# nadult/Snail

Measured on AMD Instinct MI355X. Metric: Mrays/sec (primary), higher is better.
Workload: dtype f32; 1 GPU; BASELINE config 1: atrium (263124 tris, sponza.obj stand-in) 1920x1080 primary rays, hit records (t,u,v,triId); reflections=False, arith=host_sse, arith_tables=host CPU, packets=16x16 px = 1 wavefront, bvh_nodes=161677, bvh_depth=21, frames_in_flight=16, frames_per_launch=4, launches_in_flight=4, settle_frames=356, order_refresh=16, ranks=1, packet_order=heaviest first (node visits of an earlier frame), parallelism=single-gpu

## Files before the change

### include/snail_hip_debug.h

```cpp
#ifndef SNAIL_HIP_DEBUG_H
#define SNAIL_HIP_DEBUG_H
#include "snail_hip.h"
#ifdef __cplusplus
extern "C" {
#endif

int snail_debug_delay_dev(float microseconds, void *stream);

int snail_debug_clock_dev(float microseconds, uint64_t *d_out2, void *stream);

int snail_debug_recip_check(uint64_t out2[2]);

int snail_debug_hostsse_device_check(int fn, int threads, uint64_t *badChunks, uint32_t *firstBadChunk);

int snail_debug_dispatch_rate(int blocks, int threads, int reps, float *ms_per_launch);

int snail_debug_anyorder(SnailScene *, const float cam[13], int resx, int resy, int frames, int flags, float *ms_total);

int snail_debug_occupancy(int out[4]);

int snail_debug_rel_flag_count(SnailScene *, const float org[3], int *count);

int snail_debug_rel_axis_flag_count(SnailScene *, const float org[3], int out[6]);

#ifdef __cplusplus
}
#endif
#endif
```

### snail_amd/_lib.py

```python
from __future__ import annotations

import ctypes as C
import os

HERE = os.path.dirname(os.path.abspath(__file__))
LIB_PATH = os.environ.get("SNAIL_LIB_PATH") or os.path.join(HERE, "libsnailhip.so")


class SnailError(RuntimeError):
    pass


_lib = None

_VP, _I, _F13 = C.c_void_p, C.c_int, C.c_void_p
SIGNATURES = {
    "snail_last_error": (C.c_char_p, []),
    "snail_device_count": (_I, []),
    "snail_tris_from_verts": (_I, [_VP, _I, _VP]),
    "snail_bvh_build": (_I, [_VP, _I, _VP, _VP, _VP, _VP]),
    "snail_scene_create": (_VP, [_VP, _I, _VP, _I, _I, _I]),
    "snail_scene_destroy": (None, [_VP]),
    "snail_scene_info": (_I, [_VP, _VP, _VP, _VP, _VP]),
    "snail_scene_flags": (_I, [_VP, _VP, _VP]),
# ... 97 lines not shown
    "snail_texture_build": (_I, [_VP, _I, _I, _VP, C.c_int64, _VP]),
    "snail_materials_create": (_VP, [_VP, _VP, _I, _VP, _I, _VP, _I, _VP, _I]),
    "snail_materials_destroy": (None, [_VP]),
    "snail_materials_shade_packets_dev": (_I, [_VP, _F13, _I, _I, _VP, _I, _VP, _VP, _VP, _VP, _VP, _VP]),
    "snail_render_materials_dev": (_I, [_VP, _F13, _I, _I, _VP, _I, _VP, _I, _VP, _I, _VP, _VP]),
    "snail_render_materials_packets_dev": (_I, [_VP, _F13, _I, _I, _VP, _I, _VP, _I, _VP, _I, _VP, _VP, _VP]),
    "snail_render_materials_image": (_I, [_VP, _F13, _I, _I, _VP, _I, _VP, _I, _VP, _I, _VP]),
}

MATERIALS_BOUNCE_SIGNATURES = {
    "snail_materials_mirror_packets_dev": (_I, [_VP, _F13, _I, _I, _VP, _I, _VP, _VP, _VP, _VP, _VP, _VP, _VP, _VP, _VP, _VP]),
    "snail_materials_shade_rays_dev": (_I, [_VP, _I, _VP, _VP, _VP, _VP, _VP, _VP, _VP, _VP]),
    "snail_materials_bounce_dev": (_I, [_VP, _F13, _I, _I, _VP, _I, _VP, _I, _VP, _I, _VP, _VP]),
    "snail_materials_bounce_packets_dev": (_I, [_VP, _F13, _I, _I, _VP, _I, _VP, _I, _VP, _I, _VP, _VP, _VP]),
    "snail_materials_bounce_image": (_I, [_VP, _F13, _I, _I, _VP, _I, _VP, _I, _VP, _I, _VP]),
}

MATERIALS_TILES_SIGNATURES = {
    "snail_materials_frame_packets_dev": (_I, [_VP, _F13, _I, _I, _VP, _I, _VP, _I, _VP, _I, _VP, _VP, _VP, _VP]),
    "snail_materials_render_tiles": (_I, [_VP, _F13, _I, _I, _VP, _VP, _I, _VP, _I, _VP, _I, _VP, _VP, _VP]),
    "snail_materials_render_frame": (_I, [_VP, _F13, _I, _I, _VP, _I, _VP, _I, _VP, _I, _VP]),
}

MATERIALS_TRANSPARENCY_SIGNATURES = {
    "snail_materials_create_transparent": (_VP, [_VP, _VP, _I, _VP, _I, _VP, _I, _VP, _VP, _I]),
    "snail_materials_can_select_transparent": (_I, [_VP]),
    "snail_materials_shade_packets_transp_dev": (_I, [_VP, _F13, _I, _I, _VP, _I, _VP, _VP, _VP, _VP, _VP, _VP, _VP, _VP]),
    "snail_materials_shade_rays_transp_dev": (_I, [_VP, _I, _VP, _VP, _VP, _VP, _VP, _VP, _VP, _VP, _VP, _VP]),
    "snail_materials_continue_packets_dev": (_I, [_VP, _F13, _I, _I, _VP, _I, _VP, _VP, _VP, _VP, _VP, _VP, _VP, _VP, _VP, _VP, _VP, _VP, _VP, _VP]),
    "snail_materials_transparent_dev": (_I, [_VP, _F13, _I, _I, _VP, _I, _VP, _I, _VP, _I, _I, _VP, _VP, _VP]),
    "snail_materials_transparent_packets_dev": (_I, [_VP, _F13, _I, _I, _VP, _I, _VP, _I, _VP, _I, _VP, _I, _VP, _VP, _VP]),
    "snail_materials_transparent_image": (_I, [_VP, _F13, _I, _I, _VP, _I, _VP, _I, _VP, _I, _I, _VP, _VP]),
}

MATERIALS_TREE_SIGNATURES = {
    "snail_materials_mirror_rays_dev": (_I, [_VP, _I, _VP, _VP, _VP, _VP, _VP, _VP, _VP, _VP, _VP, _VP, _VP, _VP, _VP, _VP, _VP]),
    "snail_materials_tree_frame_packets_dev": (_I, [_VP, _F13, _I, _I, _VP, _I, _VP, _I, _VP, _I, _VP, _VP, _I, _VP, _VP, _VP]),
    "snail_materials_tree_render_tiles": (_I, [_VP, _F13, _I, _I, _VP, _VP, _I, _VP, _I, _VP, _I, _VP, _VP, _I, _VP, _VP]),
    "snail_materials_tree_render_frame": (_I, [_VP, _F13, _I, _I, _VP, _I, _VP, _I, _VP, _I, _I, _VP, _VP]),
    "snail_materials_set_level_budget": (_I, [_VP, C.c_uint64]),
    "snail_materials_level_bytes": (C.c_int64, [_I, _I, _I]),
}

MATERIALS_HEAT_SIGNATURES = {
    "snail_materials_packet_stats_dev": (_I, [_VP, _F13, _I, _I, _VP, _I, _VP, _I, _I, _I, _VP, _VP, _VP, _VP]),
    "snail_materials_heat_packets_dev": (_I, [_VP, _F13, _I, _I, _VP, _I, _VP, _I, _I, _VP, _VP, _VP, _I, _VP, _VP, _VP]),
    "snail_materials_render_heat_tiles": (_I, [_VP, _F13, _I, _I, _VP, _VP, _I, _VP, _I, _I, _VP, _VP, _I, _VP, _VP]),
    "snail_materials_render_heat_frame": (_I, [_VP, _F13, _I, _I, _VP, _I, _I, _VP, _I, _I, _VP, _VP]),
}

MATERIALS_DYNAMIC_SIGNATURES = {
    "snail_materials_create_dev": (_VP, [_VP, _VP, _VP, _VP, _I, _VP, _VP, _VP, _VP, _I, _VP, _I, _VP, _VP, _I, _VP]),
    "snail_materials_rebuild_dev": (_I, [_VP, _VP, _VP, _VP, _VP, _VP]),
    "snail_materials_update_dev": (_I, [_VP, _VP, _VP, _VP, _VP, _VP]),
}

INSTANCES_MATERIALS_SIGNATURES = {
    "snail_instances_materials_create": (_VP, [_VP, _VP, _I, _VP, _I, _VP, _I]),
    "snail_instances_materials_destroy": (None, [_VP]),
    "snail_instances_materials_shade_packets_dev": (_I, [_VP, _F13, _I, _I, _VP, _I, _VP, _VP, _VP, _VP, _VP, _VP, _VP]),
    "snail_instances_render_materials_dev": (_I, [_VP, _F13, _I, _I, _VP, _I, _VP, _I, _VP, _I, _VP, _VP]),
    "snail_instances_render_materials_packets_dev": (_I, [_VP, _F13, _I, _I, _VP, _I, _VP, _I, _VP, _I, _VP, _VP, _VP]),
    "snail_instances_render_materials_image": (_I, [_VP, _F13, _I, _I, _VP, _I, _VP, _I, _VP, _I, _VP]),
}

INSTANCES_MATERIALS_BOUNCE_SIGNATURES = {
    "snail_instances_materials_mirror_packets_dev": (_I, [_VP, _F13, _I, _I, _VP, _I, _VP, _VP, _VP, _VP, _VP, _VP, _VP, _VP, _VP, _VP, _VP, _VP]),
    "snail_instances_materials_shade_rays_dev": (_I, [_VP, _I, _VP, _VP, _VP, _VP, _VP, _VP, _VP, _VP]),
    "snail_instances_materials_bounce_dev": (_I, [_VP, _F13, _I, _I, _VP, _I, _VP, _I, _VP, _I, _VP, _VP]),
    "snail_instances_materials_bounce_packets_dev": (_I, [_VP, _F13, _I, _I, _VP, _I, _VP, _I, _VP, _I, _VP, _VP, _VP]),
    "snail_instances_materials_bounce_image": (_I, [_VP, _F13, _I, _I, _VP, _I, _VP, _I, _VP, _I, _VP]),
}

DEBUG_SIGNATURES = {
    "snail_debug_delay_dev": (_I, [C.c_float, _VP]),
    "snail_debug_clock_dev": (_I, [C.c_float, _VP, _VP]),
    "snail_debug_recip_check": (_I, [_VP]),
    "snail_debug_dispatch_rate": (_I, [_I, _I, _I, _VP]),
    "snail_debug_hostsse_device_check": (_I, [_I, _I, _VP, _VP]),
    "snail_debug_occupancy": (_I, [_VP]),
    "snail_debug_anyorder": (_I, [_VP, _F13, _I, _I, _I, _I, _VP]),
    "snail_debug_rel_flag_count": (_I, [_VP, _VP, _VP]),
    "snail_debug_rel_axis_flag_count": (_I, [_VP, _VP, _VP]),
}
DEBUG_LIB_PATH = os.path.join(HERE, "libsnailhip_debug.so")
_dbg = None


def debug_lib():
    global _dbg
    if _dbg is None:
        if not os.path.exists(DEBUG_LIB_PATH):
            raise SnailError("workbench library %s is missing: `make -C snail_amd/csrc debug`" % DEBUG_LIB_PATH)
        L = C.CDLL(DEBUG_LIB_PATH)
        for table in (SIGNATURES, INSTANCES_SIGNATURES, INSTANCES_SHADE_SIGNATURES, INSTANCES_TILES_SIGNATURES, INSTANCES_BUILD_SIGNATURES, BVH_FAST_SIGNATURES, HEATMAP_SIGNATURES, MATERIALS_SIGNATURES, MATERIALS_BOUNCE_SIGNATURES, MATERIALS_TILES_SIGNATURES, MATERIALS_TRANSPARENCY_SIGNATURES, MATERIALS_TREE_SIGNATURES, MATERIALS_HEAT_SIGNATURES, MATERIALS_DYNAMIC_SIGNATURES, INSTANCES_MATERIALS_SIGNATURES, INSTANCES_MATERIALS_BOUNCE_SIGNATURES, DEBUG_SIGNATURES):
            for name, (res, args) in table.items():
                fn = getattr(L, name)
                fn.restype = res
                fn.argtypes = args
        _dbg = L
    return _dbg


def lib():
    global _lib
    if _lib is None:
        if not os.path.exists(LIB_PATH):
            raise SnailError(
                "HIP extension %s is missing: run `python -c 'import __graft_entry__ as g; g.build()'` "
                "(or `make -C snail_amd/csrc`). There is no CPU fallback." % LIB_PATH)
        try:
            L = C.CDLL(LIB_PATH)
        except OSError as e:
            raise SnailError("cannot load %s: %s" % (LIB_PATH, e)) from e
        for table in (SIGNATURES, INSTANCES_SIGNATURES, INSTANCES_SHADE_SIGNATURES, INSTANCES_TILES_SIGNATURES, INSTANCES_BUILD_SIGNATURES, BVH_FAST_SIGNATURES, HEATMAP_SIGNATURES, MATERIALS_SIGNATURES, MATERIALS_BOUNCE_SIGNATURES, MATERIALS_TILES_SIGNATURES, MATERIALS_TRANSPARENCY_SIGNATURES, MATERIALS_TREE_SIGNATURES, MATERIALS_HEAT_SIGNATURES, MATERIALS_DYNAMIC_SIGNATURES, INSTANCES_MATERIALS_SIGNATURES, INSTANCES_MATERIALS_BOUNCE_SIGNATURES):
            for name, (res, args) in table.items():
                fn = getattr(L, name)
                fn.restype = res
                fn.argtypes = args
        for name, (res, args) in DEBUG_SIGNATURES.items():
            fn = getattr(L, name, None)
            if fn is not None:
                fn.restype = res
                fn.argtypes = args
        _lib = L
    return _lib


def check(rc: int, what: str) -> None:
    if rc != 0:
        msg = lib().snail_last_error()
        raise SnailError("%s failed (status %d): %s" % (what, rc, msg.decode() if msg else "?"))


def ptr(a):
    if a is None:
        return None
    if hasattr(a, "data_ptr"):
        return C.c_void_p(a.data_ptr())
    return a.ctypes.data_as(C.c_void_p)
```

### snail_amd/csrc/bvh_fast.inc

```
namespace devf {

using devb::BuildHdr;
using devb::TNode;
static_assert(SNAIL_MAX_DEPTH == devb::kMaxDepth, "BuildHdr::qCount and the small kernel's stack are sized for DBVH::maxDepth == BVH::maxDepth");

struct FastArgs : devb::SplitArgs {
	const float *verts;
	uint4 *nodes, *pf, *tris;
	unsigned trisOff;
	int needSane;
	int *cur;
	int *perm, *info;
};

__global__ void k_fast_init(FastArgs A) {
	const int i = blockIdx.x * blockDim.x + threadIdx.x;
	if(i < A.n) A.startCnt[i] = 0;
	if(i == 0) devb::hdrInit(*A.hdr);
}

__global__ void k_fast_boxes(FastArgs A) {
	const int i = blockIdx.x * blockDim.x + threadIdx.x;
	if(i >= A.n) return;
	float p[9], rec[16];
// ... 65 lines not shown
	bool curOnDevice = false;
	int depthLimit = SNAIL_MAX_DEPTH;
	hipEvent_t ready = nullptr;
	bool hasReady = false;
	unsigned long long rebuilds = 0;
	struct Use { hipStream_t stream; hipEvent_t ev; };
	std::vector<Use> uses;
};

namespace {

void fastFree(SnailSceneFast *f) {
	if(!f) return;
	if(f->base) (void)hipFree(f->base);
	if(f->dCur) (void)hipFree(f->dCur);
	if(f->ready) (void)hipEventDestroy(f->ready);
	for(auto &u : f->uses) (void)hipEventDestroy(u.ev);
	delete f;
}

int fastSceneBegin(SnailScene *s, hipStream_t stream) {
	SnailSceneFast *f = s->fast;
	if(f->hasReady) HIP_TRY(hipStreamWaitEvent(stream, f->ready, 0));
	return 0;
}
void fastSceneEnd(SnailScene *s, hipStream_t stream) {
	SnailSceneFast *f = s->fast;
	for(auto &u : f->uses)
		if(u.stream == stream) { (void)hipEventRecord(u.ev, stream); return; }
	SnailSceneFast::Use u;
	u.stream = stream;
	if(hipEventCreateWithFlags(&u.ev, hipEventDisableTiming) != hipSuccess) return;
	(void)hipEventRecord(u.ev, stream);
	f->uses.push_back(u);
}

int fastEnqueue(SnailScene *s, const float *dVerts, int32_t *dPerm, int32_t *dInfo, int needSane, hipStream_t st) {
	SnailSceneFast *f = s->fast;
	const int n = s->nTris;
	devf::FastArgs A;
	memset((void *)&A, 0, sizeof(A));
	buildCarve(f->base, n, A);
	A.n = n; A.maxDepth = f->depthLimit;
	A.verts = dVerts;
	A.nodes = s->dNodes; A.tris = s->dTris; A.pf = s->pfOKButNesting ? (uint4 *)s->dPF : nullptr; A.trisOff = (unsigned)s->trisOff;
	A.needSane = needSane; A.cur = f->dCur; A.perm = dPerm; A.info = dInfo;
	const devb::SplitArgs &SA = A;
	typedef devb::SplitBvh P;
	const int perN = (n + 255) / 256;
	hipLaunchKernelGGL(devf::k_fast_init, dim3(perN), dim3(256), 0, st, A);
	hipLaunchKernelGGL(devf::k_fast_boxes, dim3(perN), dim3(256), 0, st, A);
	hipLaunchKernelGGL(devb::k_build_root<P>, dim3(1), dim3(64), 0, st, SA);
	if(n > devb::kSmall) {
		const int most = n / (devb::kSmall + 1) + 1;
		const int wide = 28;
		for(int level = 0; level < wide; level++) {
			const int grid = std::min(level < 11 ? (1 << level) : 2048, most);
			hipLaunchKernelGGL(devb::k_build_big<P>, dim3(grid), dim3(256), 0, st, SA, level, level + 1);
		}
		hipLaunchKernelGGL(devb::k_build_big<P>, dim3(1), dim3(256), 0, st, SA, wide, (int)devb::kLevels);
	}
	if(n >= P::minSplit) hipLaunchKernelGGL(devb::k_build_small<P>, dim3(std::min(n / 2 + 1, 8192)), dim3(64), 0, st, SA);
	hipLaunchKernelGGL(devb::k_build_scan, dim3(1), dim3(1024), 0, st, SA);
	hipLaunchKernelGGL(devf::k_fast_commit, dim3((unsigned)std::min((2 * (long long)n + 255) / 256, 4096LL)), dim3(256), 0, st, A);
	HIP_TRY(hipGetLastError());
	if(!f->ready) HIP_TRY(hipEventCreateWithFlags(&f->ready, hipEventDisableTiming));
	HIP_TRY(hipEventRecord(f->ready, st));
	f->hasReady = true;
	f->curOnDevice = true;
	f->rebuilds++;
	return 0;
}

int fastWaitUsers(SnailScene *s, hipStream_t st) {
	SnailSceneFast *f = s->fast;
	for(auto &u : f->uses) HIP_TRY(hipStreamWaitEvent(st, u.ev, 0));
	if(f->hasReady) HIP_TRY(hipStreamWaitEvent(st, f->ready, 0));
	return 0;
}

int fastRebuildLocked(SnailScene *s, const float *dVerts, int32_t *dPerm, int32_t *dInfo, hipStream_t st) {
	if(int rc = fastWaitUsers(s, st)) return rc;
	for(auto &e : s->rel) e.valid = false;
	return fastEnqueue(s, dVerts, dPerm, dInfo, s->fastOK, st);
}

int fastCurrent(const SnailScene *cs, int cur[4]) {
	SnailScene *s = const_cast<SnailScene *>(cs);
	SnailSceneFast *f = s->fast;
	DeviceGuard guard(s->device);
	std::lock_guard<std::mutex> lock(s->mu);
	if(f->curOnDevice) {
		if(f->hasReady) HIP_TRY(hipEventSynchronize(f->ready));
		HIP_TRY(hipMemcpy(f->cur, f->dCur, sizeof(f->cur), hipMemcpyDeviceToHost));
		f->curOnDevice = false;
	}
	memcpy(cur, f->cur, sizeof(f->cur));
	return 0;
}

}

extern "C" {

SnailScene *snail_scene_create_fast_dev(const float *d_verts9, int nTris, int device, int32_t *d_perm, int32_t *d_info, void *stream) {
	const char *fn = "snail_scene_create_fast_dev";
	if(!d_verts9 || nTris <= 0 || nTris > (1 << 29)) { snail_set_error("%s: bad arguments", fn); return nullptr; }
	DeviceGuard guard(device);
	if(!guard.ok) { snail_set_error("%s: hipSetDevice(%d) failed", fn, device); return nullptr; }
	hipStream_t st = (hipStream_t)stream;
	SnailScene *s = new SnailScene();
	s->fast = new SnailSceneFast();
	SnailSceneFast *f = s->fast;
	const int cap = 2 * nTris - 1;
	s->device = device; s->nNodes = cap; s->nTris = nTris;
	const size_t trisOff = pfTrisOffset(cap), pfBytes = trisOff + (size_t)nTris * 64;
	const bool fits = pfFits((size_t)cap + 1, (size_t)nTris);
	s->trisOff = (int)(fits ? trisOff : 0);
	s->pfOKButNesting = fits ? 1 : 0;
	hipError_t e;
	if((e = hipMalloc((void **)&s->dNodes, (size_t)cap * 32)) != hipSuccess || (e = hipMalloc((void **)&s->dPF, fits ? pfBytes : (size_t)nTris * 64)) != hipSuccess ||
	   (e = hipMalloc((void **)&f->base, buildScratchBytes(nTris))) != hipSuccess || (e = hipMalloc((void **)&f->dCur, 4 * sizeof(int))) != hipSuccess ||
	   (fits && (e = hipMemset(s->dPF, 0, ((size_t)cap + 1) * 32)) != hipSuccess) || (e = hipMemset(f->dCur, 0, 4 * sizeof(int))) != hipSuccess) {
		snail_set_error("%s: %s", fn, hipGetErrorString(e));
		snail_scene_destroy(s);
		return nullptr;
	}
	s->dTris = (uint4 *)(s->dPF + s->trisOff);
	hipLaunchKernelGGL(dev::lbvh::k_fill_empty, dim3((unsigned)((cap + 255) / 256)), dim3(256), 0, 0, (float *)s->dNodes, cap);
	int cur[4] = {0, 0, 0, 0}, status[8] = {0};
	if((e = hipDeviceSynchronize()) != hipSuccess || fastEnqueue(s, d_verts9, d_perm, d_info, 0, st) != 0 || (e = hipStreamSynchronize(st)) != hipSuccess ||
	   (e = hipMemcpy(status, f->base, sizeof(status), hipMemcpyDeviceToHost)) != hipSuccess || fastCurrent(s, cur) != 0) {
		if(e != hipSuccess) snail_set_error("%s: %s", fn, hipGetErrorString(e));
		snail_scene_destroy(s);
		return nullptr;
	}
	if(status[0] != 0) {
		if(status[0] == 1) snail_set_error("%s: a vertex is not finite", fn);
		else snail_set_error("%s: the tree is deeper than BVH::maxDepth = %d", fn, SNAIL_MAX_DEPTH);
		snail_scene_destroy(s);
		return nullptr;
	}
	s->depth = cur[1]; s->fastOK = cur[2]; s->nestedOK = 1; s->pfOK = s->pfOKButNesting;
	f->depthLimit = s->depth > 62 ? SNAIL_MAX_DEPTH : 62;
	return s;
}

int snail_scene_rebuild_fast_dev(SnailScene *s, const float *d_verts9, int nTris, int32_t *d_perm, int32_t *d_info, void *stream) {
	const char *fn = "snail_scene_rebuild_fast_dev";
	if(int rc = checkScene(s, fn)) return rc;
	if(!s->fast) { snail_set_error("%s: the handle was not made by snail_scene_create_fast_dev", fn); return 1; }
	if(!d_verts9 || nTris != s->nTris) { snail_set_error("%s: %d triangles, the handle holds %d (or null vertices)", fn, nTris, s->nTris); return 1; }
	hipStream_t st = (hipStream_t)stream;
	DeviceGuard guard(s->device);
	SNAIL_LOCK(s);
	return fastRebuildLocked(s, d_verts9, d_perm, d_info, st);
}

}
```

### snail_amd/csrc/snail_dev.inc

```
namespace SNAIL_DEV_NS {

typedef unsigned long long u64;
typedef unsigned u32x4 __attribute__((ext_vector_type(4)));
typedef const __attribute__((address_space(4))) u32x4 *scalar_ptr;

struct Node {
	float bmin[3], bmax[3];
	unsigned sub;
	int aux;
};

__device__ __forceinline__ float asf(unsigned u) { return __uint_as_float(u); }
__device__ __forceinline__ float asf(int u) { return __int_as_float(u); }

typedef const __attribute__((address_space(4))) char *scalar_bytes;
__device__ __forceinline__ Node loadNode(const uint4 *nodes, int idx) {
	const unsigned off = (unsigned)idx << 5;
	scalar_ptr p = (scalar_ptr)((scalar_bytes)(unsigned long long)nodes + off);
	u32x4 a = p[0], b = p[1];
	Node n;
	n.bmin[0] = asf(a.x); n.bmin[1] = asf(a.y); n.bmin[2] = asf(a.z);
	n.bmax[0] = asf(a.w); n.bmax[1] = asf(b.x); n.bmax[2] = asf(b.y);
	n.sub = b.z; n.aux = (int)b.w;
	return n;
// ... 257 lines not shown
		outMax[c] = noneU ? 0.0f : (x01 > x23 ? x01 : x23);
	}
}

__device__ __forceinline__ bool boxTestInterval(const Node &n, const Interval &i) {
	float lmin = 0.0f, lmax = 0.0f;
#pragma unroll
	for(int k = 0; k < 3; k++) {
		float l1 = i.minIDir[k] * (n.bmin[k] - i.maxOrg[k]);
		float l2 = i.maxIDir[k] * (n.bmin[k] - i.maxOrg[k]);
		float l3 = i.minIDir[k] * (n.bmax[k] - i.minOrg[k]);
		float l4 = i.maxIDir[k] * (n.bmax[k] - i.minOrg[k]);
		float lo = Min<M_EXACT>(Min<M_EXACT>(l1, l2), Min<M_EXACT>(l3, l4));
		float hi = Max<M_EXACT>(Max<M_EXACT>(l1, l2), Max<M_EXACT>(l3, l4));
		if(k == 0) { lmin = lo; lmax = hi; }
		else { lmin = Max<M_EXACT>(lmin, lo); lmax = Min<M_EXACT>(lmax, hi); }
	}
	return lmax >= 0.0f && lmin <= lmax;
}

struct TriTerms {
	float t0v[3], t1v[3], tmul;
};
__device__ __forceinline__ TriTerms triTerms(const Tri &t, float ox, float oy, float oz) {
	TriTerms r;
	float tv[3] = {ox - t.a[0], oy - t.a[1], oz - t.a[2]};
	r.t0v[0] = (t.ba[1] * tv[2] - t.ba[2] * tv[1]) * t.it0;
	r.t0v[1] = (t.ba[2] * tv[0] - t.ba[0] * tv[2]) * t.it0;
	r.t0v[2] = (t.ba[0] * tv[1] - t.ba[1] * tv[0]) * t.it0;
	r.t1v[0] = (tv[1] * t.ca[2] - tv[2] * t.ca[1]) * t.it0;
	r.t1v[1] = (tv[2] * t.ca[0] - tv[0] * t.ca[2]) * t.it0;
	r.t1v[2] = (tv[0] * t.ca[1] - tv[1] * t.ca[0]) * t.it0;
	r.tmul = -(tv[0] * t.n[0] + tv[1] * t.n[1] + tv[2] * t.n[2]);
	return r;
}

__device__ __forceinline__ float selLanes(float a, float b, u64 lanesOfB) {
	float r;
	asm("v_cndmask_b32 %0, %1, %2, %3" : "=v"(r) : "v"(a), "v"(b), "s"(lanesOfB));
	return r;
}
__device__ __forceinline__ float xbar(int byteAddr, float x) { return __int_as_float(__builtin_amdgcn_ds_bpermute(byteAddr, __float_as_int(x))); }
template <int CTRL> __device__ __forceinline__ float quadRot(float v) {
	return __int_as_float(__builtin_amdgcn_update_dpp(0, __float_as_int(v), CTRL, 0xf, 0xf, false));
}
struct QuadTerms {
	float n, t0v, t1v, tmul;
};
template <int M>
__device__ __forceinline__ u64 cullQuad(const uint4 *__restrict__ tris, int count , int firstTri, int lane, const float (&org)[3][4],
										const Interval &iv, QuadTerms &T) {
	const int c = lane & 3;
	const bool active = lane < 4 * count;
	T.n = T.t0v = T.t1v = T.tmul = 0.0f;
	bool pass = false;
	const float oc = selLanes(selLanes(org[0][0], org[1][0], 0x2222222222222222ull), org[2][0], 0x4444444444444444ull);
	const float dmn = selLanes(selLanes(iv.minDir[0], iv.minDir[1], 0x2222222222222222ull), iv.minDir[2], 0x4444444444444444ull);
	const float dmx = selLanes(selLanes(iv.maxDir[0], iv.maxDir[1], 0x2222222222222222ull), iv.maxDir[2], 0x4444444444444444ull);
	if(active) {
		const float *rec = (const float *)(tris + (size_t)(firstTri + (lane >> 2)) * 4);
		const float *rc = rec + (c == 3 ? 0 : c);
		const float ac = rc[0], bac = rc[3], cac = rc[6], nc = rc[12];
		const float t0 = rec[9], it0 = rec[10];
		const float tv = oc - ac;
		const float tv1 = quadRot<0xC9>(tv), tv2 = quadRot<0xD2>(tv);
		const float ba1 = quadRot<0xC9>(bac), ba2 = quadRot<0xD2>(bac), ca1 = quadRot<0xC9>(cac), ca2 = quadRot<0xD2>(cac);
		const float c1 = ba1 * tv2 - ba2 * tv1;
		const float c2 = tv1 * ca2 - tv2 * ca1;
		T.n = nc; T.t0v = c1 * it0; T.t1v = c2 * it0;
		const float p = tv * nc;
		T.tmul = -((p + quadRot<0xC9>(p)) + quadRot<0xD2>(p));
		float m;
		if(M == M_EXACT) m = (nc < 0.0f ? dmn : dmx) * nc;
		else m = vmax(dmn * nc, dmx * nc);
		const float det = (m + quadRot<0xC9>(m)) + quadRot<0xD2>(m);
		const float c1a = dmn * c1, c1b = dmx * c1, c2a = dmn * c2, c2b = dmx * c2;
		const float u0p = Min<M>(c1a, c1b), u1p = Max<M>(c1a, c1b), v0p = Min<M>(c2a, c2b), v1p = Max<M>(c2a, c2b);
		const float u0 = (u0p + quadRot<0xC9>(u0p)) + quadRot<0xD2>(u0p), u1 = (u1p + quadRot<0xC9>(u1p)) + quadRot<0xD2>(u1p);
		const float v0 = (v0p + quadRot<0xC9>(v0p)) + quadRot<0xD2>(v0p), v1 = (v1p + quadRot<0xC9>(v1p)) + quadRot<0xD2>(v1p);
		pass = (c == 0) & ((det < 0.0f) | ((Min<M>(u1, v1) >= 0.0f) & (u0 + v0 <= det * t0)));
	}
	return __builtin_amdgcn_ballot_w64(pass);
}
__device__ __forceinline__ void setId(int &d, int v) { d = v; }
__device__ __forceinline__ void setId(float &d, int v) { d = __int_as_float(v); }
template <int R> struct NarrowRays {
	float d[3][R], dist[R];
	int tid[R];
};
template <int R> __device__ __forceinline__ void narrowGather(const float (&q)[4], int srcAddr, float (&out)[R]) {
	const float a0 = xbar(srcAddr, q[0]), a1 = xbar(srcAddr, q[1]), a2 = xbar(srcAddr, q[2]), a3 = xbar(srcAddr, q[3]);
	if(R == 1) out[0] = selLanes(selLanes(a0, a1, 0xaaaaaaaaaaaaaaaaull), selLanes(a2, a3, 0xaaaaaaaaaaaaaaaaull), 0xccccccccccccccccull);
	else { out[0] = selLanes(a0, a2, 0xaaaaaaaaaaaaaaaaull); out[R - 1] = selLanes(a1, a3, 0xaaaaaaaaaaaaaaaaull); }
}
template <int R, int M, class TID>
__device__ __forceinline__ void leafSharedNarrow(const uint4 *__restrict__ tris, int count, int firstTri, int lane, int first, int last,
												 const float (&org)[3][4], Quad &Q, TID (&tid)[4], const Interval &iv, Counters &st) {
	constexpr int LPQ = 4 / R;
	const int width = last - first + 1;
	const bool inRange = lane >= first && lane <= last;
	const bool live = lane < width * LPQ;
	st.leaves++;
	st.fetched += (unsigned)count;
	QuadTerms qt = {};
	u64 keep = cullQuad<M>(tris, count, firstTri, lane, org, iv, qt);
	if(keep == 0) return;
	NarrowRays<R> N;
	const int srcAddr = (first + lane / LPQ) * 4;
#pragma unroll
	for(int c = 0; c < 3; c++) narrowGather<R>(Q.d[c], srcAddr, N.d[c]);
	narrowGather<R>(Q.dist, srcAddr, N.dist);
#pragma unroll
	for(int i = 0; i < R; i++) N.tid[i] = -1;
	do {
		const int kb = __builtin_ctzll(keep);
		keep &= keep - 1;
		const float nx = xbar(kb * 4, qt.n), ny = xbar(kb * 4 + 4, qt.n), nz = xbar(kb * 4 + 8, qt.n);
		const float ax = xbar(kb * 4, qt.t0v), ay = xbar(kb * 4 + 4, qt.t0v), az = xbar(kb * 4 + 8, qt.t0v);
		const float bx = xbar(kb * 4, qt.t1v), by = xbar(kb * 4 + 4, qt.t1v), bz = xbar(kb * 4 + 8, qt.t1v);
		const float tmul = xbar(kb * 4, qt.tmul);
		const int idx = firstTri + (kb >> 2);
#if SNAIL_ARITH_SSE
		if(R > 1) {
			if(live) {
				float det[R];
				bool test[R], any = false;
#pragma unroll
				for(int i = 0; i < R; i++) {
					const float dt = N.d[0][i] * nx + N.d[1][i] * ny + N.d[2][i] * nz;
					const float v = N.d[0][i] * ax + N.d[1][i] * ay + N.d[2][i] * az;
					const float u = N.d[0][i] * bx + N.d[1][i] * by + N.d[2][i] * bz;
					const float duv = dt - u - v;
					const float uvmin = Min3<M>(u, v, duv), uvmax = Max3<M>(u, v, duv);
					test[i] = (uvmax <= 0.0f) | (uvmin >= 0.0f);
					det[i] = test[i] ? dt : 1.0f;
					any |= test[i];
				}
				if(any) {
					float idet[R];
					InvN<R>(det, idet);
#pragma unroll
					for(int i = 0; i < R; i++) {
						const float dd = idet[i] * tmul;
						if(test[i] && dd < N.dist[i] && dd > 0.0f) { N.dist[i] = dd; N.tid[i] = idx; }
					}
				}
			}
		} else
#endif
		if(live)
#pragma unroll
			for(int i = 0; i < R; i++) {
				const float det = N.d[0][i] * nx + N.d[1][i] * ny + N.d[2][i] * nz;
				const float v = N.d[0][i] * ax + N.d[1][i] * ay + N.d[2][i] * az;
				const float u = N.d[0][i] * bx + N.d[1][i] * by + N.d[2][i] * bz;
				const float duv = det - u - v;
				const float uvmin = Min3<M>(u, v, duv), uvmax = Max3<M>(u, v, duv);
				if((uvmax <= 0.0f) | (uvmin >= 0.0f)) {
					const float dd = Inv(det) * tmul;
					if(dd < N.dist[i] && dd > 0.0f) { N.dist[i] = dd; N.tid[i] = idx; }
				}
			}
		st.intersects += width;
	} while(keep);
	const int q = lane - first;
#pragma unroll
	for(int l = 0; l < 4; l++) {
		const int src = (q * LPQ + l / R) * 4;
		const float nd = xbar(src, N.dist[l % R]);
		const int nt = __builtin_amdgcn_ds_bpermute(src, N.tid[l % R]);
		if(inRange && nt >= 0) { Q.dist[l] = nd; setId(tid[l], nt); }
	}
}

template <int R, int M>
__device__ __forceinline__ void leafSharedNarrowShadow(const uint4 *__restrict__ tris, int count, int firstTri, int lane, int first, int last,
													   const float (&org)[3][4], Quad &Q, const Interval &iv, Counters &st) {
	constexpr int LPQ = 4 / R;
	const float inf = __builtin_inff();
	const int width = last - first + 1;
	const bool inRange = lane >= first && lane <= last;
	const bool live = lane < width * LPQ;
	st.leaves++;
	st.fetched += (unsigned)count;
	QuadTerms qt = {};
	u64 keep = cullQuad<M>(tris, count, firstTri, lane, org, iv, qt);
	if(keep == 0) return;
	float nd[3][R], ndist[R];
	const int srcAddr = (first + lane / LPQ) * 4;
#pragma unroll
	for(int c = 0; c < 3; c++) narrowGather<R>(Q.d[c], srcAddr, nd[c]);
	narrowGather<R>(Q.dist, srcAddr, ndist);
	do {
		const int kb = __builtin_ctzll(keep);
		keep &= keep - 1;
		const float nx = xbar(kb * 4, qt.n), ny = xbar(kb * 4 + 4, qt.n), nz = xbar(kb * 4 + 8, qt.n);
		const float ax = xbar(kb * 4, qt.t0v), ay = xbar(kb * 4 + 4, qt.t0v), az = xbar(kb * 4 + 8, qt.t0v);
		const float bx = xbar(kb * 4, qt.t1v), by = xbar(kb * 4 + 4, qt.t1v), bz = xbar(kb * 4 + 8, qt.t1v);
		const float tmul = xbar(kb * 4, qt.tmul);
#pragma unroll
		for(int i = 0; i < R; i++) {
			const float det = nd[0][i] * nx + nd[1][i] * ny + nd[2][i] * nz;
			const float v = nd[0][i] * ax + nd[1][i] * ay + nd[2][i] * az;
			const float u = nd[0][i] * bx + nd[1][i] * by + nd[2][i] * bz;
			bool test = (Min<M>(u, v) >= 0.0f) & (u + v <= det);
			test = test & (tmul > 0.0f) & (tmul < ndist[i] * det);
			if(live && test) ndist[i] = -inf;
		}
		st.intersects += width;
	} while(keep);
	const int q = lane - first;
#pragma unroll
	for(int l = 0; l < 4; l++) {
		const float d = xbar((q * LPQ + l / R) * 4, ndist[l % R]);
		if(inRange) Q.dist[l] = d;
	}
}

template <bool MASK, bool SHADOW, int M, bool BARY, class TID>
__device__ __forceinline__ bool leafShared(const uint4 *__restrict__ tris, int count, int firstTri, int size, int lane, int first, int last,
										   const float (&org)[3][4], Quad &Q, unsigned mask4, TID (&tid)[4], float (&bu)[4], float (&bv)[4],
										   const Interval &iv, Counters &st) {
	const float inf = __builtin_inff();
	const bool inRange = lane >= first && lane <= last;
	const int width = last - first + 1;
	if(!SHADOW && !MASK && !BARY) {
		const int widthU = __builtin_amdgcn_readfirstlane(width);
		const int countU = __builtin_amdgcn_readfirstlane(count);
		if(widthU <= 32 && countU <= 16) {
			const int firstU = __builtin_amdgcn_readfirstlane(first);
			if(widthU <= 16) leafSharedNarrow<1, M>(tris, countU, firstTri, lane, firstU, firstU + widthU - 1, org, Q, tid, iv, st);
			else leafSharedNarrow<2, M>(tris, countU, firstTri, lane, firstU, firstU + widthU - 1, org, Q, tid, iv, st);
			return false;
		}
	}
	if(SHADOW && !MASK && !BARY) {
		const int widthU = __builtin_amdgcn_readfirstlane(width);
		const int countU = __builtin_amdgcn_readfirstlane(count);
		if(widthU <= 32 && widthU < size && countU <= 16) {
			const int firstU = __builtin_amdgcn_readfirstlane(first);
			if(widthU <= 16) leafSharedNarrowShadow<1, M>(tris, countU, firstTri, lane, firstU, firstU + widthU - 1, org, Q, iv, st);
			else leafSharedNarrowShadow<2, M>(tris, countU, firstTri, lane, firstU, firstU + widthU - 1, org, Q, iv, st);
			return false;
		}
	}
	const u64 curRange = rangeMask(first, last);
	st.leaves++;
	constexpr bool LANE_MASK = !SHADOW;
	auto collide = [&](const float nx, const float ny, const float nz, const float ax, const float ay, const float az, const float bx, const float by, const float bz,
					   const float tmul, const int idx) -> bool {
		bool all4 = true;
#if SNAIL_ARITH_SSE
		if(!SHADOW && !BARY) {
			if(!LANE_MASK || inRange) {
				float det[4];
				bool test[4], any = false;
#pragma unroll
				for(int l = 0; l < 4; l++) {
					const float dt = Q.d[0][l] * nx + Q.d[1][l] * ny + Q.d[2][l] * nz;
					const float v = Q.d[0][l] * ax + Q.d[1][l] * ay + Q.d[2][l] * az;
					const float u = Q.d[0][l] * bx + Q.d[1][l] * by + Q.d[2][l] * bz;
					const float duv = dt - u - v;
					const float uvmin = Min3<M>(u, v, duv), uvmax = Max3<M>(u, v, duv);
					test[l] = ((uvmax <= 0.0f) | (uvmin >= 0.0f)) & inRange;
					if(MASK) test[l] = test[l] & (((mask4 >> l) & 1u) != 0);
					det[l] = test[l] ? dt : 1.0f;
					any |= test[l];
				}
				if(any) {
					float idet[4];
					InvN<4>(det, idet);
#pragma unroll
					for(int l = 0; l < 4; l++) {
						const float dd = idet[l] * tmul;
						if(test[l] && dd < Q.dist[l] && dd > 0.0f) { Q.dist[l] = dd; setId(tid[l], idx); }
					}
				}
			}
			st.intersects += width;
			return false;
		}
#endif
		if(!LANE_MASK || inRange)
#pragma unroll
		for(int l = 0; l < 4; l++) {
			const float det = Q.d[0][l] * nx + Q.d[1][l] * ny + Q.d[2][l] * nz;
			const float v = Q.d[0][l] * ax + Q.d[1][l] * ay + Q.d[2][l] * az;
			const float u = Q.d[0][l] * bx + Q.d[1][l] * by + Q.d[2][l] * bz;
			if(SHADOW) {
				bool test = (Min<M>(u, v) >= 0.0f) & (u + v <= det);
				test = test & (tmul > 0.0f) & (tmul < Q.dist[l] * det);
				all4 = all4 & test;
				if(inRange && test) Q.dist[l] = -inf;
			} else {
				const float duv = det - u - v;
				const float uvmin = Min3<M>(u, v, duv), uvmax = Max3<M>(u, v, duv);
				bool test = ((uvmax <= 0.0f) | (uvmin >= 0.0f)) & inRange;
				if(MASK) test = test & (((mask4 >> l) & 1u) != 0);
				if(test) {
					const float idet = Inv(det);
					const float dd = idet * tmul;
					if(dd < Q.dist[l] && dd > 0.0f) {
						Q.dist[l] = dd; setId(tid[l], idx);
						if(BARY) { bu[l] = u * idet; bv[l] = v * idet; }
					}
// ... 224 lines not shown
				for(int l = 0; l < 4; l++) {
					float lmin = 0.0f, lmax = 0.0f;
#pragma unroll
					for(int k = 0; k < 3; k++) {
						float l1 = Q.id[k][l] * (SHARED ? tmn[k] : n.bmin[k] - org[k][l]);
						float l2 = Q.id[k][l] * (SHARED ? tmx[k] : n.bmax[k] - org[k][l]);
						float lo = Min<M_EXACT>(l1, l2), hi = Max<M_EXACT>(l1, l2);
						if(k == 0) { lmin = lo; lmax = hi; }
						else if(SHADOW) { lmin = Max<M_EXACT>(lo, lmin); lmax = Min<M_EXACT>(hi, lmax); }
						else { lmin = Max<M_EXACT>(lmin, lo); lmax = Min<M_EXACT>(lmax, hi); }
					}
					bool pass = SHADOW ? (lmax >= 0.0f && lmin <= Min<M_EXACT>(lmax, Q.dist[l])) : !(lmax < 0.0f || lmin > Min<M_EXACT>(lmax, Q.dist[l]));
					anyPass |= pass;
				}
			}
			passMask = __builtin_amdgcn_ballot_w64(anyPass);
		} else passMask = fastPass(n);
		const u64 alive = passMask & __builtin_amdgcn_ballot_w64((unsigned)(lane - first) <= (unsigned)(last - first));
		if(alive != 0) {
			first = __builtin_ctzll(alive);
			last = 63 - __builtin_clzll(alive);
			if(!isLeaf) {
				const int fl = first | (last << 8);
				if(!DEEP || sp < 64) writeLane2(stkNode, farIdx, stkFL, fl, sp);
				else writeLane2(stkNode2, farIdx, stkFL2, fl, sp - 64);
				sp++;
				n = nn;
				continue;
			}
		const int count = n.aux, firstTri = (int)(n.sub & 0x7fffffffu);
		if(SHARED) {
			if(leafShared<MASK, SHADOW, M, BARY>(tris, count, firstTri, size, lane, first, last, org, Q, mask4, tid, bu, bv, iv, st)) return;
		} else {
			leafPerRay<MASK, M, BARY>(tris, count, firstTri, lane, first, last, org, Q, mask4, tid, bu, bv, st);
		}
		}
		if(sp == 0) break;
		sp--;
		int cur, fl;
		if(!DEEP || sp < 64) { cur = __builtin_amdgcn_readlane(stkNode, sp); fl = __builtin_amdgcn_readlane(stkFL, sp); }
		else { cur = __builtin_amdgcn_readlane(stkNode2, sp - 64); fl = __builtin_amdgcn_readlane(stkFL2, sp - 64); }
		first = fl & 0xff; last = fl >> 8;
		n = loadNode(nodes, cur);
	}
}

#define SNAIL_SLAB_COH(L, NX, FX, NY, FY, NZ, FZ)                                                                                           \
	"v_mul_f32 %[t0], %[ix" L "], %[pnx]\n v_mul_f32 %[t1], %[iy" L "], %[pny]\n v_mul_f32 %[t2], %[iz" L "], %[pnz]\n"                    \
	"v_mul_f32 %[t3], %[ix" L "], %[pfx]\n v_mul_f32 %[t4], %[iy" L "], %[pfy]\n v_mul_f32 %[t5], %[iz" L "], %[pfz]\n"                    \
	"v_max3_f32 %[t0], %[t0], %[t1], %[t2]\n v_min3_f32 %[t3], %[t3], %[t4], %[t5]\n"
#define SNAIL_SLAB_FAST(L, NX, FX, NY, FY, NZ, FZ)                                                                                          \
	"v_mul_f32 %[t0], %[ix" L "], %[pnx]\n v_mul_f32 %[t3], %[ix" L "], %[pfx]\n v_min_f32 %[u0], %[t0], %[t3]\n v_max_f32 %[t3], %[t0], %[t3]\n" \
	"v_mul_f32 %[t1], %[iy" L "], %[pny]\n v_mul_f32 %[t4], %[iy" L "], %[pfy]\n v_min_f32 %[t0], %[t1], %[t4]\n v_max_f32 %[t4], %[t1], %[t4]\n" \
	"v_mul_f32 %[t2], %[iz" L "], %[pnz]\n v_mul_f32 %[t5], %[iz" L "], %[pfz]\n v_min_f32 %[t1], %[t2], %[t5]\n v_max_f32 %[t5], %[t2], %[t5]\n" \
	"v_max3_f32 %[t0], %[u0], %[t0], %[t1]\n v_min3_f32 %[t3], %[t3], %[t4], %[t5]\n"
#define SNAIL_SLAB_COH_R(L, NX, FX, NY, FY, NZ, FZ)                                                                                         \
	"v_mul_f32 %[t0], " NX ", %[ix" L "]\n v_mul_f32 %[t1], " NY ", %[iy" L "]\n v_mul_f32 %[t2], " NZ ", %[iz" L "]\n"                    \
	"v_mul_f32 %[t3], " FX ", %[ix" L "]\n v_mul_f32 %[t4], " FY ", %[iy" L "]\n v_mul_f32 %[t5], " FZ ", %[iz" L "]\n"                    \
	"v_max3_f32 %[t0], %[t0], %[t1], %[t2]\n v_min3_f32 %[t3], %[t3], %[t4], %[t5]\n"
#define SNAIL_SLAB_FAST_R(L, NX, FX, NY, FY, NZ, FZ)                                                                                        \
	"v_mul_f32 %[t0], " NX ", %[ix" L "]\n v_mul_f32 %[t3], " FX ", %[ix" L "]\n v_min_f32 %[u0], %[t0], %[t3]\n v_max_f32 %[t3], %[t0], %[t3]\n" \
	"v_mul_f32 %[t1], " NY ", %[iy" L "]\n v_mul_f32 %[t4], " FY ", %[iy" L "]\n v_min_f32 %[t0], %[t1], %[t4]\n v_max_f32 %[t4], %[t1], %[t4]\n" \
	"v_mul_f32 %[t2], " NZ ", %[iz" L "]\n v_mul_f32 %[t5], " FZ ", %[iz" L "]\n v_min_f32 %[t1], %[t2], %[t5]\n v_max_f32 %[t5], %[t2], %[t5]\n" \
	"v_max3_f32 %[t0], %[u0], %[t0], %[t1]\n v_min3_f32 %[t3], %[t3], %[t4], %[t5]\n"
#define SNAIL_SLABO_COH(L, NX, FX, NY, FY, NZ, FZ)                                                                                          \
	"v_sub_f32 %[t0], " NX ", %[ox" L "]\n v_sub_f32 %[t1], " NY ", %[oy" L "]\n v_sub_f32 %[t2], " NZ ", %[oz" L "]\n"                    \
	"v_sub_f32 %[t3], " FX ", %[ox" L "]\n v_sub_f32 %[t4], " FY ", %[oy" L "]\n v_sub_f32 %[t5], " FZ ", %[oz" L "]\n"                    \
	"v_mul_f32 %[t0], %[ix" L "], %[t0]\n v_mul_f32 %[t1], %[iy" L "], %[t1]\n v_mul_f32 %[t2], %[iz" L "], %[t2]\n"                       \
	"v_mul_f32 %[t3], %[ix" L "], %[t3]\n v_mul_f32 %[t4], %[iy" L "], %[t4]\n v_mul_f32 %[t5], %[iz" L "], %[t5]\n"                       \
	"v_max3_f32 %[t0], %[t0], %[t1], %[t2]\n v_min3_f32 %[t3], %[t3], %[t4], %[t5]\n"
#define SNAIL_SLABO_FAST(L, NX, FX, NY, FY, NZ, FZ)                                                                                         \
	"v_sub_f32 %[t0], " NX ", %[ox" L "]\n v_sub_f32 %[t3], " FX ", %[ox" L "]\n v_mul_f32 %[t0], %[ix" L "], %[t0]\n v_mul_f32 %[t3], %[ix" L "], %[t3]\n" \
	"v_min_f32 %[u0], %[t0], %[t3]\n v_max_f32 %[t3], %[t0], %[t3]\n"                                                                      \
	"v_sub_f32 %[t1], " NY ", %[oy" L "]\n v_sub_f32 %[t4], " FY ", %[oy" L "]\n v_mul_f32 %[t1], %[iy" L "], %[t1]\n v_mul_f32 %[t4], %[iy" L "], %[t4]\n" \
	"v_min_f32 %[t0], %[t1], %[t4]\n v_max_f32 %[t4], %[t1], %[t4]\n"                                                                      \
	"v_sub_f32 %[t2], " NZ ", %[oz" L "]\n v_sub_f32 %[t5], " FZ ", %[oz" L "]\n v_mul_f32 %[t2], %[iz" L "], %[t2]\n v_mul_f32 %[t5], %[iz" L "], %[t5]\n" \
	"v_min_f32 %[t1], %[t2], %[t5]\n v_max_f32 %[t5], %[t2], %[t5]\n"                                                                      \
	"v_max3_f32 %[t0], %[u0], %[t0], %[t1]\n v_min3_f32 %[t3], %[t3], %[t4], %[t5]\n"
#define SNAIL_PRE_SHARED(NX, FX, NY, FY, NZ, FZ)                                                                                            \
	" v_sub_f32 %[pnx], " NX ", %[ox]\n v_sub_f32 %[pny], " NY ", %[oy]\n v_sub_f32 %[pnz], " NZ ", %[oz]\n"                               \
	" v_sub_f32 %[pfx], " FX ", %[ox]\n v_sub_f32 %[pfy], " FY ", %[oy]\n v_sub_f32 %[pfz], " FZ ", %[oz]\n"
#define SNAIL_PRE_NONE(NX, FX, NY, FY, NZ, FZ) ""
#define SNAIL_ORG_SHARED() [ox] "v"(org[0][0]), [oy] "v"(org[1][0]), [oz] "v"(org[2][0])
#define SNAIL_ORG_PERRAY()                                                                                                                 \
	[ox0] "v"(org[0][0]), [ox1] "v"(org[0][1]), [ox2] "v"(org[0][2]), [ox3] "v"(org[0][3]), [oy0] "v"(org[1][0]), [oy1] "v"(org[1][1]),     \
		[oy2] "v"(org[1][2]), [oy3] "v"(org[1][3]), [oz0] "v"(org[2][0]), [oz1] "v"(org[2][1]), [oz2] "v"(org[2][2]), [oz3] "v"(org[2][3])
#define SNAIL_TAIL_POS(L, S) "v_max_f32 %[t0], 0, %[t0]\n v_min_f32 %[t3], %[t3], %[d" L "]\n v_sub_f32 %[" S "], %[t3], %[t0]\n"
#define SNAIL_TAIL_ANY(L, S) "v_min_f32 %[t4], %[t3], %[d" L "]\n v_sub_f32 %[t4], %[t4], %[t0]\n v_min_f32 %[" S "], %[t4], %[t3]\n"
#define SNAIL_TAIL_POSF(L, S) "v_min_f32 %[t3], %[t3], %[d" L "]\n v_sub_f32 %[" S "], %[t3], %[t0]\n"
#define SNAIL_POP_2W                                                                                                                       \
	" v_readlane_b32 %[cur], %[stkN], %[sp]\n v_readlane_b32 %[fl], %[stkF], %[sp]\n"                                                      \
	" s_and_b32 %[first], %[fl], 0xff\n s_lshr_b32 %[last], %[fl], 8\n"
#define SNAIL_PUSH_2W                                                                                                                      \
	" s_lshl_b32 %[off], %[last], 8\n s_or_b32 %[off], %[off], %[first]\n"                                                                 \
	" s_mov_b32 m0, %[sp]\n v_writelane_b32 %[stkN], %[fl], m0\n v_writelane_b32 %[stkF], %[off], m0\n"
#define SNAIL_COUNT " s_add_u32 %[cnt], %[cnt], 1\n"
#define SNAIL_DRAIN_SMEM " s_waitcnt lgkmcnt(0)\n"
#define SNAIL_DESCEND_ASM(PRE, ORGOPS, SLAB, TAIL, CNTPOP, CNTVISIT, NX, FX, NY, FY, NZ, FZ)                                                 \
	asm volatile(SNAIL_DRAIN_SMEM                                                                                                          \
				 "L_pop_%=:\n"                                                                                                             \
				 " s_cmp_eq_u32 %[sp], 0\n s_cbranch_scc1 L_done_%=\n"                                                                     \
				 " s_sub_u32 %[sp], %[sp], 1\n" CNTPOP                                                                                     \
				 SNAIL_POP_2W                                                                                                              \
				 " s_lshl_b32 %[off], %[cur], 5\n s_load_dwordx8 s[84:91], %[base], %[off]\n"                                              \
				 " s_sub_u32 %[width], %[last], %[first]\n"                                                                                \
				 " s_bfm_b64 exec, %[width], %[first]\n s_bitset1_b64 exec, %[last]\n"                                                     \
				 " s_waitcnt lgkmcnt(0)\n"                                                                                                 \
				 "L_visit_%=:\n" CNTVISIT                                                                                                  \
				 PRE(NX, FX, NY, FY, NZ, FZ)                                                                                               \
				 SLAB("0", NX, FX, NY, FY, NZ, FZ) TAIL("0", "s0") SLAB("1", NX, FX, NY, FY, NZ, FZ) TAIL("1", "s1")                       \
				 SLAB("2", NX, FX, NY, FY, NZ, FZ) TAIL("2", "s2") SLAB("3", NX, FX, NY, FY, NZ, FZ) TAIL("3", "s3")                       \
				 " v_max_f32 %[s2], %[s2], %[s3]\n v_max3_f32 %[s0], %[s0], %[s1], %[s2]\n"                                                \
				 " v_cmp_le_f32 vcc, 0, %[s0]\n"                                                                                           \
				 " s_and_b64 %[alive], vcc, exec\n s_cbranch_scc0 L_pop_%=\n"                                                              \
				 " s_ff1_i32_b64 %[first], %[alive]\n s_flbit_i32_b64 %[last], %[alive]\n s_xor_b32 %[last], %[last], 63\n"                \
				 " s_sub_u32 %[width], %[last], %[first]\n"                                                                                \
				 " s_bfm_b64 exec, %[width], %[first]\n s_bitset1_b64 exec, %[last]\n"                                                     \
				 " s_cmp_lt_i32 s90, 0\n s_cbranch_scc1 L_leaf_%=\n"                                                                       \
				 " s_lshr_b32 %[cur], %[sign16], s91\n s_xor_b32 %[cur], %[cur], s91\n s_bfe_u32 %[cur], %[cur], 0x10010\n"                \
				 " s_add_u32 %[fl], s90, 1\n s_sub_u32 %[fl], %[fl], %[cur]\n"                                                             \
				 " s_add_u32 %[cur], s90, %[cur]\n s_lshl_b32 %[off], %[cur], 5\n"                                                         \
				 " s_load_dwordx8 s[84:91], %[base], %[off]\n"                                                                             \
				 SNAIL_PUSH_2W                                                                                                             \
				 " s_add_u32 %[sp], %[sp], 1\n"                                                                                            \
				 " s_waitcnt lgkmcnt(0)\n s_branch L_visit_%=\n"                                                                           \
				 "L_leaf_%=:\n s_mov_b32 %[leafSub], s90\n s_mov_b32 %[leafAux], s91\n s_branch L_end_%=\n"                                \
				 "L_done_%=:\n s_mov_b32 %[leafSub], 0\n s_mov_b32 %[leafAux], 0\n"                                                        \
				 "L_end_%=:\n s_mov_b64 exec, -1\n"                                                                                        \
				 : [sp] "+s"(sp), [first] "+s"(first), [last] "+s"(last), [cnt] "+s"(cnt), [stkN] "+v"(stkN), [stkF] "+v"(stkF),           \
				   [leafSub] "=&s"(leafSub), [leafAux] "=&s"(leafAux), [cur] "=&s"(sCur), [fl] "=&s"(sFl), [off] "=&s"(sOff),              \
				   [width] "=&s"(sWidth), [rng] "=&s"(sRng), [alive] "=&s"(sAlive), [pnx] "=&v"(vt[0]), [pny] "=&v"(vt[1]),                \
				   [pnz] "=&v"(vt[2]), [pfx] "=&v"(vt[3]), [pfy] "=&v"(vt[4]), [pfz] "=&v"(vt[5]), [t0] "=&v"(vt[6]), [t1] "=&v"(vt[7]),   \
				   [t2] "=&v"(vt[8]), [t3] "=&v"(vt[9]), [t4] "=&v"(vt[10]), [t5] "=&v"(vt[11]), [s0] "=&v"(vt[12]), [s1] "=&v"(vt[13]),   \
				   [s2] "=&v"(vt[14]), [s3] "=&v"(vt[15]), [u0] "=&v"(vt[16])                                                              \
				 : [base] "s"(nodeBase), [sign16] "s"(sign16), [lane] "v"(lane), ORGOPS(), [ix0] "v"(Q.id[0][0]), [ix1] "v"(Q.id[0][1]), [ix2] "v"(Q.id[0][2]), [ix3] "v"(Q.id[0][3]),        \
				   [iy0] "v"(Q.id[1][0]), [iy1] "v"(Q.id[1][1]), [iy2] "v"(Q.id[1][2]), [iy3] "v"(Q.id[1][3]), [iz0] "v"(Q.id[2][0]),      \
				   [iz1] "v"(Q.id[2][1]), [iz2] "v"(Q.id[2][2]), [iz3] "v"(Q.id[2][3]), [d0] "v"(Q.dist[0]), [d1] "v"(Q.dist[1]),          \
				   [d2] "v"(Q.dist[2]), [d3] "v"(Q.dist[3])                                                                                \
				 : "s84", "s85", "s86", "s87", "s88", "s89", "s90", "s91", "vcc", "scc", "m0");                                            \
	              \
	asm volatile("" ::"s"(sp), "s"(first), "s"(last), "s"(cnt), "v"(stkN), "v"(stkF), "s"(leafSub), "s"(leafAux), "s"(sCur), "s"(sFl), "s"(sOff),    \
				 "s"(sWidth), "s"(sRng), "s"(sAlive), "v"(vt[0]), "v"(vt[1]), "v"(vt[2]), "v"(vt[3]), "v"(vt[4]), "v"(vt[5]), "v"(vt[6]), "v"(vt[7]), \
				 "v"(vt[8]), "v"(vt[9]), "v"(vt[10]), "v"(vt[11]), "v"(vt[12]), "v"(vt[13]), "v"(vt[14]), "v"(vt[15]), "v"(vt[16]))
#define SNAIL_REL_INSIDE_BIT 31
#define SNAIL_MOV_REC(D0, D1, D2, D3, S0, S1, S2, S3)                                                                                       \
	" s_mov_b64 " D0 ", " S0 "\n s_mov_b64 " D1 ", " S1 "\n s_mov_b64 " D2 ", " S2 "\n s_mov_b64 " D3 ", " S3 "\n"
#define SNAIL_A_FROM_T SNAIL_MOV_REC("s[84:85]", "s[86:87]", "s[88:89]", "s[90:91]", "s[68:69]", "s[70:71]", "s[72:73]", "s[74:75]")
#define SNAIL_PF_LEAFREQ_TRI(OTHERSET) " s_bitset0_b32 %[cur], 31\n s_load_dwordx8 " OTHERSET ", %[base], %[cur]\n"
#define SNAIL_PF_LEAFREQ_SLOT0(OTHERSET) " s_max_i32 %[cur], %[cur], 0\n s_load_dwordx8 " OTHERSET ", %[base], %[cur]\n"

#define SNAIL_PF2_NEARFAR(SUB, AUX, FARX, OTHERSET, LEAFREQ)                                                                                          \
				 " s_and_b32 %[cur], " AUX ", %[sign16]\n s_cselect_b32 %[cur], 32, 0\n"                                                       \
				 " s_xor_b32 %[cur], " SUB ", %[cur]\n s_xor_b32 " FARX ", %[cur], 32\n"                                                       \
				 LEAFREQ(OTHERSET)
#define SNAIL_PF2_TAIL(X, SUB)  \
				 " v_max_f32 %[s2], %[s2], %[s3]\n v_max3_f32 %[s0], %[s0], %[s1], %[s2]\n"                                                \
				 " v_cmpx_le_f32 vcc, 0, %[s0]\n"                                                                                           \
				 " s_cbranch_execz L_fail_%=\n"                                                                                            \
				 " s_cbranch_scc1 L_leaf" X "_%=\n"
#define SNAIL_PF2_ISLEAF(SUB) " s_cmp_lt_i32 " SUB ", 0\n"
#define SNAIL_PF2_ALIVE " s_sub_u32 %[cur], %[last], %[first]\n s_bfm_b64 %[alive], %[cur], %[first]\n s_bitset1_b64 %[alive], %[last]\n"
#define SNAIL_PF2_FIRSTLAST " s_ff1_i32_b64 %[first], exec\n s_flbit_i32_b64 %[last], exec\n s_xor_b32 %[last], %[last], 63\n"
static_assert(SNAIL_REL_INSIDE_BIT == 31, "SNAIL_OIN_TEST_SNAIL_TAIL_POS names the bit in its text");
#define SNAIL_OIN_TEST_SNAIL_TAIL_POS(AUX, CP, OMASK) " s_bitcmp1_b32 " AUX ", 31\n s_cbranch_scc1 L_oin" CP "_%=\n"
#define SNAIL_OIN_TEST_SNAIL_TAIL_ANY(AUX, CP, OMASK) ""
#define SNAIL_OIN_TEST_SNAIL_TAIL_POSF(AUX, CP, OMASK) " s_and_b32 vcc_lo, " AUX ", " OMASK "\n s_cbranch_scc0 L_slow" CP "_%=\n"
// ... 81 lines not shown
				 " v_readlane_b32 %[topw], %[stkN], %[off]\n"                                                                              \
				 " s_and_b32 %[cur], %[topw], 0xfffff\n s_lshl_b32 %[off], %[cur], 5\n"                                                    \
				 " s_load_dwordx8 s[68:75], %[base], %[off]\n"                                                                             \
				 " s_bfe_u32 %[first], %[topw], 0x60014\n s_lshr_b32 %[last], %[topw], 26\n" SNAIL_PF2_ALIVE                               \
				 "L_pop_%=:\n"                             \
				 " s_sub_u32 m0, m0, 1\n" CNTPOP                                                                                     \
				 " s_mov_b64 exec, %[alive]\n"                                                                                             \
				 " s_waitcnt lgkmcnt(0)\n" SNAIL_A_FROM_T                                                                                  \
				                   \
				 " s_sub_u32 %[off], m0, 1\n s_max_i32 %[off], %[off], 0\n"   \
				 " v_readlane_b32 %[topw], %[stkN], %[off]\n"                                                                              \
				 SNAIL_OIN_TEST_of(TAIL)("s91", "Aq", OMASK)                                                                                 \
				 SNAIL_PF2_POPBODY(PRE, SLAB, TAIL, CNTVISIT, LEAFREQ, NXA, FXA, NYA, FYA, NZA, FZA)                                         \
				                                                                    \
				 SNAIL_PF2_PENDING("B", "s[84:91]", "s82", "s83", "%[width]", "%[fl]", PRE, SLAB, TAIL, CNTVISIT, LEAFREQ, OMASK, NXB, FXB, NYB, FYB, NZB, FZB)            \
				                                                                    \
				 SNAIL_PF2_PENDING("A", "s[76:83]", "s90", "s91", "%[fl]", "%[width]", PRE, SLAB, TAIL, CNTVISIT, LEAFREQ, OMASK, NXA, FXA, NYA, FYA, NZA, FZA)            \
				 " s_branch L_visitBp_%=\n"                                                                                                \
				 SNAIL_PF2_LEAF("A", "s90", "s91") SNAIL_PF2_LEAF("B", "s82", "s83")                                                       \
				 SNAIL_OIN_COPIES_of(TAIL)(CNTVISIT, LEAFREQ)                                                                               \
				 SNAIL_POSENTRY_COPIES_of(TAIL)(PRE, SLAB, CNTVISIT, LEAFREQ, NXA, FXA, NYA, FYA, NZA, FZA, NXB, FXB, NYB, FYB, NZB, FZB)    \
				 "L_fail_%=:\n"                                                                                                            \
				 " s_cmp_eq_u32 m0, 0\n s_cbranch_scc0 L_pop_%=\n"                                                                      \
				 "L_done_%=:\n s_mov_b32 %[leafSub], 0\n s_mov_b32 %[leafAux], 0\n s_waitcnt lgkmcnt(0)\n"                                  \
				 "L_end_%=:\n s_mov_b64 exec, -1\n s_mov_b32 %[sp], m0\n"                                                                                        \
				 : [sp] "+s"(sp), [first] "+s"(first), [last] "+s"(last), [cnt] "+s"(cnt), [stkN] "+v"(stkN), [stkF] "+v"(stkF),           \
				   [leafSub] "=&s"(leafSub), [leafAux] "=&s"(leafAux), [cur] "=&s"(sCur), [fl] "=&s"(sFl), [off] "=&s"(sOff),              \
				   [width] "=&s"(sWidth), [topw] "=&s"(sTopw), [alive] "=&s"(sAlive), PREVARS() [t0] "=&v"(vt[6]), [t1] "=&v"(vt[7]),   \
				   [t2] "=&v"(vt[8]), [t3] "=&v"(vt[9]), [t4] "=&v"(vt[10]), [t5] "=&v"(vt[11]), [s0] "=&v"(vt[12]), [s1] "=&v"(vt[13]),   \
				   [s2] "=&v"(vt[14]), [s3] "=&v"(vt[15]), [u0] "=&v"(vt[16])                                                              \
				 : [base] "s"(nodeBase), [sign16] "s"(sign16), [lane] "v"(lane), ORGOPS(), [ix0] "v"(Q.id[0][0]), [ix1] "v"(Q.id[0][1]), [ix2] "v"(Q.id[0][2]), [ix3] "v"(Q.id[0][3]),        \
				   [iy0] "v"(Q.id[1][0]), [iy1] "v"(Q.id[1][1]), [iy2] "v"(Q.id[1][2]), [iy3] "v"(Q.id[1][3]), [iz0] "v"(Q.id[2][0]),      \
				   [iz1] "v"(Q.id[2][1]), [iz2] "v"(Q.id[2][2]), [iz3] "v"(Q.id[2][3]), [d0] "v"(Q.dist[0]), [d1] "v"(Q.dist[1]),          \
				   [d2] "v"(Q.dist[2]), [d3] "v"(Q.dist[3])                                                                                \
				 : "s68", "s69", "s70", "s71", "s72", "s73", "s74", "s75", "s76", "s77", "s78", "s79", "s80", "s81", "s82", "s83", "s84", "s85", "s86", "s87", \
				   "s88", "s89", "s90", "s91", "vcc", "scc", "m0" EXTRACLOB);                                                                        \
	asm volatile("" ::"s"(sp), "s"(first), "s"(last), "s"(cnt), "v"(stkN), "v"(stkF), "s"(leafSub), "s"(leafAux), "s"(sCur), "s"(sFl), "s"(sOff),    \
				 "s"(sWidth), "s"(sTopw), "s"(sAlive), "v"(vt[6]), "v"(vt[7]), \
				 "v"(vt[8]), "v"(vt[9]), "v"(vt[10]), "v"(vt[11]), "v"(vt[12]), "v"(vt[13]), "v"(vt[14]), "v"(vt[15]), "v"(vt[16]))
#define SNAIL_PREVARS_SHARED() [pnx] "=&v"(vt[0]), [pny] "=&v"(vt[1]), [pnz] "=&v"(vt[2]), [pfx] "=&v"(vt[3]), [pfy] "=&v"(vt[4]), [pfz] "=&v"(vt[5]),
#define SNAIL_PREVARS_NONE() [pnx] "=&v"(vt[0]), [pny] "=&v"(vt[1]), [pnz] "=&v"(vt[2]), [pfx] "=&v"(vt[3]), [pfy] "=&v"(vt[4]), [pfz] "=&v"(vt[5]),
#define SNAIL_PREVARS_SNAIL_PRE_SHARED SNAIL_PREVARS_SHARED
#define SNAIL_PREVARS_SNAIL_PRE_NONE SNAIL_PREVARS_NONE
#define SNAIL_PREVARS_SNAIL_PRE_SEL SNAIL_PREVARS_NONE
#define SNAIL_PREVARS_EMPTY()
#define SNAIL_PRE_NONE_X(NX, FX, NY, FY, NZ, FZ) ""
#define SNAIL_PREVARS_SNAIL_PRE_NONE_X SNAIL_PREVARS_EMPTY
#define SNAIL_PREVARS_of(PRE) SNAIL_PREVARS_##PRE
#define SNAIL_DESCEND_PF2M(OMASK, PRE, ORGOPS, SLAB, TAIL, CNTPOP, CNTVISIT, LEAFREQ, NXA, FXA, NYA, FYA, NZA, FZA, NXB, FXB, NYB, FYB, NZB, FZB)                 \
	SNAIL_DESCEND_PF2X(, OMASK, SNAIL_PREVARS_of(PRE), PRE, ORGOPS, SLAB, TAIL, CNTPOP, CNTVISIT, LEAFREQ, NXA, FXA, NYA, FYA, NZA, FZA, NXB, FXB, NYB, FYB, NZB, FZB)
#define SNAIL_PRE_SEL(NX, FX, NY, FY, NZ, FZ)                                                                                               \
				 " s_bitcmp1_b32 %[sign16], 8\n s_cselect_b32 s62, " FX ", " NX "\n s_cselect_b32 s65, " NX ", " FX "\n"                       \
				 " s_bitcmp1_b32 %[sign16], 9\n s_cselect_b32 s63, " FY ", " NY "\n s_cselect_b32 s66, " NY ", " FY "\n"                       \
				 " s_bitcmp1_b32 %[sign16], 10\n s_cselect_b32 s64, " FZ ", " NZ "\n s_cselect_b32 s67, " NZ ", " FZ "\n"
#define SNAIL_SLABO_SEL(L, NX, FX, NY, FY, NZ, FZ) SNAIL_SLABO_COH(L, "s62", "s65", "s63", "s66", "s64", "s67")
#define SNAIL_SEL_CLOB , "s62", "s63", "s64", "s65", "s66", "s67"
#define SNAIL_DESCEND_PF2_SEL(ORGOPS, SLAB, TAIL, CNTPOP, CNTVISIT, LEAFREQ)                                                                \
	SNAIL_DESCEND_PF2X(SNAIL_SEL_CLOB, "0", SNAIL_PREVARS_NONE, SNAIL_PRE_SEL, ORGOPS, SLAB, TAIL, CNTPOP, CNTVISIT, LEAFREQ, "s84", "s87", "s85", "s88", "s86", "s89", "s76", "s79", "s77", "s80", "s78", "s81")
#define SNAIL_DESCEND_PF2_PLAIN(PRE, ORGOPS, SLAB, TAIL, CNTPOP, CNTVISIT, LEAFREQ) SNAIL_DESCEND_PF2M("0", PRE, ORGOPS, SLAB, TAIL, CNTPOP, CNTVISIT, LEAFREQ, "s84", "s87", "s85", "s88", "s86", "s89", "s76", "s79", "s77", "s80", "s78", "s81")
#define SNAIL_DESCEND_PF2_OCT(PRE, ORGOPS, SLAB, TAIL, CNTPOP, CNTVISIT, LEAFREQ, OCT)                                                                                                    \
	switch(OCT) {                                                                                                                          \
	case 0: SNAIL_DESCEND_PF2M("0x0e000000", PRE, ORGOPS, SLAB, TAIL, CNTPOP, CNTVISIT, LEAFREQ, "s84", "s87", "s85", "s88", "s86", "s89", "s76", "s79", "s77", "s80", "s78", "s81"); break;            \
	case 1: SNAIL_DESCEND_PF2M("0x1c000000", PRE, ORGOPS, SLAB, TAIL, CNTPOP, CNTVISIT, LEAFREQ, "s87", "s84", "s85", "s88", "s86", "s89", "s79", "s76", "s77", "s80", "s78", "s81"); break;            \
	case 2: SNAIL_DESCEND_PF2M("0x2a000000", PRE, ORGOPS, SLAB, TAIL, CNTPOP, CNTVISIT, LEAFREQ, "s84", "s87", "s88", "s85", "s86", "s89", "s76", "s79", "s80", "s77", "s78", "s81"); break;            \
	case 3: SNAIL_DESCEND_PF2M("0x38000000", PRE, ORGOPS, SLAB, TAIL, CNTPOP, CNTVISIT, LEAFREQ, "s87", "s84", "s88", "s85", "s86", "s89", "s79", "s76", "s80", "s77", "s78", "s81"); break;            \
	case 4: SNAIL_DESCEND_PF2M("0x46000000", PRE, ORGOPS, SLAB, TAIL, CNTPOP, CNTVISIT, LEAFREQ, "s84", "s87", "s85", "s88", "s89", "s86", "s76", "s79", "s77", "s80", "s81", "s78"); break;            \
	case 5: SNAIL_DESCEND_PF2M("0x54000000", PRE, ORGOPS, SLAB, TAIL, CNTPOP, CNTVISIT, LEAFREQ, "s87", "s84", "s85", "s88", "s89", "s86", "s79", "s76", "s77", "s80", "s81", "s78"); break;            \
	case 6: SNAIL_DESCEND_PF2M("0x62000000", PRE, ORGOPS, SLAB, TAIL, CNTPOP, CNTVISIT, LEAFREQ, "s84", "s87", "s88", "s85", "s89", "s86", "s76", "s79", "s80", "s77", "s81", "s78"); break;            \
	default: SNAIL_DESCEND_PF2M("0x70000000", PRE, ORGOPS, SLAB, TAIL, CNTPOP, CNTVISIT, LEAFREQ, "s87", "s84", "s88", "s85", "s89", "s86", "s79", "s76", "s80", "s77", "s81", "s78"); break;           \
	}

#define SNAIL_DESCEND_OCT(PRE, ORGOPS, SLAB, TAIL, CNTPOP, CNTVISIT, OCT)                                                                     \
	switch(OCT) {                                                                                                                          \
	case 0: SNAIL_DESCEND_ASM(PRE, ORGOPS, SLAB, TAIL, CNTPOP, CNTVISIT, "s84", "s87", "s85", "s88", "s86", "s89"); break;                              \
	case 1: SNAIL_DESCEND_ASM(PRE, ORGOPS, SLAB, TAIL, CNTPOP, CNTVISIT, "s87", "s84", "s85", "s88", "s86", "s89"); break;                              \
	case 2: SNAIL_DESCEND_ASM(PRE, ORGOPS, SLAB, TAIL, CNTPOP, CNTVISIT, "s84", "s87", "s88", "s85", "s86", "s89"); break;                              \
	case 3: SNAIL_DESCEND_ASM(PRE, ORGOPS, SLAB, TAIL, CNTPOP, CNTVISIT, "s87", "s84", "s88", "s85", "s86", "s89"); break;                              \
	case 4: SNAIL_DESCEND_ASM(PRE, ORGOPS, SLAB, TAIL, CNTPOP, CNTVISIT, "s84", "s87", "s85", "s88", "s89", "s86"); break;                              \
	case 5: SNAIL_DESCEND_ASM(PRE, ORGOPS, SLAB, TAIL, CNTPOP, CNTVISIT, "s87", "s84", "s85", "s88", "s89", "s86"); break;                              \
	case 6: SNAIL_DESCEND_ASM(PRE, ORGOPS, SLAB, TAIL, CNTPOP, CNTVISIT, "s84", "s87", "s88", "s85", "s89", "s86"); break;                              \
	default: SNAIL_DESCEND_ASM(PRE, ORGOPS, SLAB, TAIL, CNTPOP, CNTVISIT, "s87", "s84", "s88", "s85", "s89", "s86"); break;                             \
	}

template <bool SHADOW, bool COH, bool PACK, bool MASK, bool BARY, bool POSDIST, bool REL = true >
__device__ __forceinline__ void walkSharedAsm(const uint4 *__restrict__ nodes , const uint4 *__restrict__ tris, int size, int lane,
											  const float (&org)[3][4], Quad &Q, unsigned mask4, int (&tid)[4], float (&bu)[4], float (&bv)[4], float *lds,
											  Counters &st, const int oct) {
	Interval iv;
	{
		unsigned act4 = lane < size ? 15u : 0u;
		if(SHADOW) {
			act4 = 0;
			if(lane < size)
#pragma unroll
				for(int l = 0; l < 4; l++) act4 |= (Q.dist[l] >= 0.0f ? 1u : 0u) << l;
		} else if(MASK) act4 = lane < size ? (mask4 & 15u) : 0u;
		computeMinMax<false, (MASK || SHADOW)>(Q.d, act4, size, lane, lds, iv.minDir, iv.maxDir);
	}
#pragma unroll
	for(int k = 0; k < 3; k++) { iv.minIDir[k] = iv.maxIDir[k] = 0.0f; iv.minOrg[k] = iv.maxOrg[k] = org[k][0]; }
	const int signBits = __builtin_amdgcn_readfirstlane((Q.d[0][0] < 0.0f ? 1 : 0) | (Q.d[1][0] < 0.0f ? 2 : 0) | (Q.d[2][0] < 0.0f ? 4 : 0));
	float tidBits[4];
#pragma unroll
	for(int l = 0; l < 4; l++) tidBits[l] = __int_as_float(tid[l]);
	const int sign16 = PACK ? signBits : signBits << 16;
	const u64 nodeBase = (u64)nodes;
	float stkN = __int_as_float(PACK ? (int)((unsigned)(size - 1) << 26) | 1 : 0), stkF = __int_as_float((size - 1) << 8);
	int sp = 1, first = 0, last = size - 1, cnt = 0;
	for(;;) {
		int leafSub, leafAux, sCur, sFl, sOff, sWidth;
		u64 sRng, sAlive;
		float vt[17];
		if(PACK) {
			int sTopw;
			if(COH) {
				if(SHADOW && REL) { SNAIL_DESCEND_PF2_OCT(SNAIL_PRE_NONE_X, SNAIL_ORG_SHARED, SNAIL_SLAB_COH_R, SNAIL_TAIL_ANY, "", SNAIL_COUNT, SNAIL_PF_LEAFREQ_SLOT0, oct) }
				else if(SHADOW) { SNAIL_DESCEND_PF2_OCT(SNAIL_PRE_SHARED, SNAIL_ORG_SHARED, SNAIL_SLAB_COH, SNAIL_TAIL_ANY, "", SNAIL_COUNT, SNAIL_PF_LEAFREQ_TRI, oct) }
				else if(POSDIST) { SNAIL_DESCEND_PF2_OCT(SNAIL_PRE_NONE_X, SNAIL_ORG_SHARED, SNAIL_SLAB_COH_R, SNAIL_TAIL_POSF, SNAIL_COUNT, "", SNAIL_PF_LEAFREQ_SLOT0, oct) }
				else { SNAIL_DESCEND_PF2_OCT(SNAIL_PRE_SHARED, SNAIL_ORG_SHARED, SNAIL_SLAB_COH, SNAIL_TAIL_ANY, SNAIL_COUNT, "", SNAIL_PF_LEAFREQ_TRI, oct) }
			} else {
				if(SHADOW && REL) { SNAIL_DESCEND_PF2_PLAIN(SNAIL_PRE_NONE_X, SNAIL_ORG_SHARED, SNAIL_SLAB_FAST_R, SNAIL_TAIL_ANY, "", SNAIL_COUNT, SNAIL_PF_LEAFREQ_SLOT0); }
				else if(SHADOW) { SNAIL_DESCEND_PF2_PLAIN(SNAIL_PRE_SHARED, SNAIL_ORG_SHARED, SNAIL_SLAB_FAST, SNAIL_TAIL_ANY, "", SNAIL_COUNT, SNAIL_PF_LEAFREQ_TRI); }
				else if(POSDIST) { SNAIL_DESCEND_PF2_PLAIN(SNAIL_PRE_NONE_X, SNAIL_ORG_SHARED, SNAIL_SLAB_FAST_R, SNAIL_TAIL_POS, SNAIL_COUNT, "", SNAIL_PF_LEAFREQ_SLOT0); }
				else { SNAIL_DESCEND_PF2_PLAIN(SNAIL_PRE_SHARED, SNAIL_ORG_SHARED, SNAIL_SLAB_FAST, SNAIL_TAIL_ANY, SNAIL_COUNT, "", SNAIL_PF_LEAFREQ_TRI); }
			}
		} else if(COH) {
			if(SHADOW) { SNAIL_DESCEND_OCT(SNAIL_PRE_SHARED, SNAIL_ORG_SHARED, SNAIL_SLAB_COH, SNAIL_TAIL_ANY, "", SNAIL_COUNT, oct) }
			else if(POSDIST) { SNAIL_DESCEND_OCT(SNAIL_PRE_SHARED, SNAIL_ORG_SHARED, SNAIL_SLAB_COH, SNAIL_TAIL_POS, SNAIL_COUNT, "", oct) }
			else { SNAIL_DESCEND_OCT(SNAIL_PRE_SHARED, SNAIL_ORG_SHARED, SNAIL_SLAB_COH, SNAIL_TAIL_ANY, SNAIL_COUNT, "", oct) }
		} else {
			if(SHADOW) { SNAIL_DESCEND_ASM(SNAIL_PRE_SHARED, SNAIL_ORG_SHARED, SNAIL_SLAB_FAST, SNAIL_TAIL_ANY, "", SNAIL_COUNT, "s84", "s87", "s85", "s88", "s86", "s89"); }
			else if(POSDIST) { SNAIL_DESCEND_ASM(SNAIL_PRE_SHARED, SNAIL_ORG_SHARED, SNAIL_SLAB_FAST, SNAIL_TAIL_POS, SNAIL_COUNT, "", "s84", "s87", "s85", "s88", "s86", "s89"); }
			else { SNAIL_DESCEND_ASM(SNAIL_PRE_SHARED, SNAIL_ORG_SHARED, SNAIL_SLAB_FAST, SNAIL_TAIL_ANY, SNAIL_COUNT, "", "s84", "s87", "s85", "s88", "s86", "s89"); }
		}
		if(leafSub == 0) break;
		if(leafShared<MASK, SHADOW, COH ? M_COH : M_FAST, BARY>(tris, leafAux, (int)((unsigned)leafSub & 0x7fffffffu), size, lane, first, last, org, Q, mask4,
																 tidBits, bu, bv, iv, st))
			break;
	}
#pragma unroll
	for(int l = 0; l < 4; l++) tid[l] = __float_as_int(tidBits[l]);
	st.iters += SHADOW ? (unsigned)cnt : 2u * (unsigned)cnt - 1u;
}

template <bool MASK, bool COH, bool BARY, bool PACK>
__device__ __forceinline__ void walkPerRayAsm(const uint4 *__restrict__ nodes , const uint4 *__restrict__ tris, int size, int lane, const float (&org)[3][4],
											  Quad &Q, unsigned mask4, int (&tid)[4], float (&bu)[4], float (&bv)[4], Counters &st, const int oct) {
	const int signBits = __builtin_amdgcn_readfirstlane((Q.d[0][0] < 0.0f ? 1 : 0) | (Q.d[1][0] < 0.0f ? 2 : 0) | (Q.d[2][0] < 0.0f ? 4 : 0));
	const int sign16 = PACK ? (COH ? signBits | __builtin_amdgcn_readfirstlane(oct) << 8 : signBits) : signBits << 16;
	const u64 nodeBase = (u64)nodes;
	float stkN = __int_as_float(PACK ? (int)((unsigned)(size - 1) << 26) | 1 : 0), stkF = __int_as_float((size - 1) << 8);
	int sp = 1, first = 0, last = size - 1, cnt = 0;
	for(;;) {
		int leafSub, leafAux, sCur, sFl, sOff, sWidth;
		u64 sRng, sAlive;
		float vt[17];
		if(PACK) {
			int sTopw;
			if(COH) { SNAIL_DESCEND_PF2_SEL(SNAIL_ORG_PERRAY, SNAIL_SLABO_SEL, SNAIL_TAIL_ANY, SNAIL_COUNT, "", SNAIL_PF_LEAFREQ_TRI); }
			else { SNAIL_DESCEND_PF2_PLAIN(SNAIL_PRE_NONE, SNAIL_ORG_PERRAY, SNAIL_SLABO_FAST, SNAIL_TAIL_ANY, SNAIL_COUNT, "", SNAIL_PF_LEAFREQ_TRI); }
		} else if(COH) { SNAIL_DESCEND_OCT(SNAIL_PRE_NONE, SNAIL_ORG_PERRAY, SNAIL_SLABO_COH, SNAIL_TAIL_ANY, SNAIL_COUNT, "", oct) }
		else { SNAIL_DESCEND_ASM(SNAIL_PRE_NONE, SNAIL_ORG_PERRAY, SNAIL_SLABO_FAST, SNAIL_TAIL_ANY, SNAIL_COUNT, "", "s84", "s87", "s85", "s88", "s86", "s89"); }
		if(leafSub == 0) break;
		leafPerRay<MASK, COH ? M_COH : M_FAST, BARY>(tris, leafAux, (int)((unsigned)leafSub & 0x7fffffffu), lane, first, last, org, Q, mask4, tid, bu, bv, st);
	}
	st.iters += 2u * (unsigned)cnt - 1u;
}

__device__ __forceinline__ void finalBarycentrics(const uint4 *__restrict__ tris, const float (&org)[3][4], const Quad &Q, const int (&tid)[4],
												  float (&bu)[4], float (&bv)[4]) {
#if SNAIL_ARITH_SSE
	float det[4], uu[4], vv[4], idet[4];
#pragma unroll
	for(int l = 0; l < 4; l++) {
		det[l] = 1.0f; uu[l] = 0.0f; vv[l] = 0.0f;
		if(Q.dist[l] < __builtin_inff()) {
			const Tri t = loadTriVector(tris, tid[l]);
			const TriTerms tt = triTerms(t, org[0][0], org[1][0], org[2][0]);
			det[l] = Q.d[0][l] * t.n[0] + Q.d[1][l] * t.n[1] + Q.d[2][l] * t.n[2];
			vv[l] = Q.d[0][l] * tt.t0v[0] + Q.d[1][l] * tt.t0v[1] + Q.d[2][l] * tt.t0v[2];
			uu[l] = Q.d[0][l] * tt.t1v[0] + Q.d[1][l] * tt.t1v[1] + Q.d[2][l] * tt.t1v[2];
		}
	}
	InvN<4>(det, idet);
#pragma unroll
	for(int l = 0; l < 4; l++) {
		const bool hit = Q.dist[l] < __builtin_inff();
		bu[l] = hit ? uu[l] * idet[l] : 0.0f; bv[l] = hit ? vv[l] * idet[l] : 0.0f;
	}
#else
#pragma unroll
	for(int l = 0; l < 4; l++) {
		bu[l] = 0.0f; bv[l] = 0.0f;
		if(Q.dist[l] < __builtin_inff()) {
			const Tri t = loadTriVector(tris, tid[l]);
			const TriTerms tt = triTerms(t, org[0][0], org[1][0], org[2][0]);
			const float det = Q.d[0][l] * t.n[0] + Q.d[1][l] * t.n[1] + Q.d[2][l] * t.n[2];
			const float v = Q.d[0][l] * tt.t0v[0] + Q.d[1][l] * tt.t0v[1] + Q.d[2][l] * tt.t0v[2];
			const float u = Q.d[0][l] * tt.t1v[0] + Q.d[1][l] * tt.t1v[1] + Q.d[2][l] * tt.t1v[2];
			const float idet = Inv(det);
			bu[l] = u * idet; bv[l] = v * idet;
		}
	}
#endif
}

__device__ __forceinline__ int classify(bool fastOK, bool laneFinite, bool live, const float (&id)[3][4], const float (&dist)[4], int &oct) {
	oct = 0;
	if(!(fastOK && __all(laneFinite || !live))) return M_EXACT;
	bool coh = true;
#pragma unroll
	for(int k = 0; k < 3; k++) {
		bool anyNeg = false, anyPos = false;
#pragma unroll
		for(int l = 0; l < 4; l++) {
			const bool matters = dist[l] > -__builtin_inff();
			anyNeg |= matters && __float_as_int(id[k][l]) < 0;
			anyPos |= matters && __float_as_int(id[k][l]) >= 0;
		}
		const bool n = __any(anyNeg && live), p = __any(anyPos && live);
		coh = coh && !(n && p);
		oct |= n ? (1 << k) : 0;
	}
	return coh ? M_COH : M_FAST;
}

__device__ __forceinline__ bool originSaneDev(const float (&o)[3]) {
	return __builtin_fabsf(o[0]) <= 1.0e9f && __builtin_fabsf(o[1]) <= 1.0e9f && __builtin_fabsf(o[2]) <= 1.0e9f;
}
__device__ __forceinline__ bool finite4(const float (&v)[3][4]) {
	bool f = true;
#pragma unroll
	for(int c = 0; c < 3; c++)
#pragma unroll
		for(int l = 0; l < 4; l++) f = f && (__builtin_fabsf(v[c][l]) < __builtin_inff());
	return f;
}

__device__ __forceinline__ void flushStats(u64 *stats, const Counters &st, unsigned rays, int lane) {
	if(stats && lane == 0) {
		atomicAdd(&stats[0], (u64)st.intersects);
		atomicAdd(&stats[1], (u64)st.iters);
		atomicAdd(&stats[2], (u64)rays);
		atomicAdd(&stats[3], (u64)st.skips);
	}
}
__device__ __forceinline__ void bookPacket(unsigned *pstats, size_t packet, const Counters &st, unsigned rays, int lane) {
	if(pstats && lane == 0) {
		unsigned *w = pstats + packet * 4;
		atomicAdd(&w[0], st.intersects);
		atomicAdd(&w[1], st.iters);
		atomicAdd(&w[2], rays);
		atomicAdd(&w[3], st.skips);
	}
}

__device__ __forceinline__ int convChannelW(float c) {
	float v = c * 255.0f;
	v = v > 0.0f ? v : 0.0f;
	v = v < 255.0f ? v : 255.0f;
	return (int)v;
}

template <class ARGS>
__device__ __forceinline__ void bookPacketLate(size_t packet, const Counters &st, unsigned rays, int lane) {
	const ARGS __attribute__((address_space(4))) *E = (const ARGS __attribute__((address_space(4))) *)__builtin_amdgcn_kernarg_segment_ptr();
	asm volatile("" : "+s"(E));
	bookPacket(E->pstats, packet, st, rays, lane);
}

struct GenConst {
	float tright[3], tup[3], txyz[3][4], org[3];
};

struct FrameOut {
	float *t, *u, *v;
	int *id;
	unsigned char *bgr;
};
struct PrimaryArgs {
	const unsigned *hostTab;
	const uint4 *nodes, *tris;
	const uint4 *pf;
	int nFrames;
	GenConst g[SNAIL_MAX_BATCH];
	FrameOut out[SNAIL_MAX_BATCH];
	const uint4 *rel[SNAIL_MAX_BATCH];
	int resx, resy, x0, y0, w, h;
	const int2 *packetXY;
	int nPackets, pw, ph;
	int nBlocks;
	int pack;
	int packetMajor;
	int fastOK;
	u64 *stats;
	unsigned *cost;
	const int *order;
	int *slotCost;
	int nSlots;
	int *defer;
	int *nextOrder;
	int nextOrderFlags;
	unsigned *pstats;
};

typedef const PrimaryArgs __attribute__((address_space(4))) *PrimaryArgsK;
typedef const FrameOut __attribute__((address_space(4))) *FrameOutK;
__device__ __forceinline__ PrimaryArgsK lateArgs() {
	PrimaryArgsK p = (PrimaryArgsK)__builtin_amdgcn_kernarg_segment_ptr();
	asm volatile("" : "+s"(p));
	return p;
}

#define LDS_FLOATS_PER_WAVE (64 * 12 + 64)

__device__ __forceinline__ int interleave16(int b) {
	const int xcd = b & 7, j = b >> 3;
	return (((j >> 4) << 3) + xcd) * 16 + (j & 15);
}

template <bool DEEP, bool EXACTPASS, bool DIAG = false, bool PSTATS = false>
__device__ __forceinline__ void primaryPacket(const PrimaryArgs &A, const int li, const int fi, float *lds) {
	const int lane = threadIdx.x & 63;
	const GenConst &G = A.g[fi];

	int px, py, pidx;
	if(A.packetXY) {
		pidx = li;
		if((unsigned)pidx >= (unsigned)A.nPackets) return;
		int2 xy = A.packetXY[pidx];
		px = __builtin_amdgcn_readfirstlane(xy.x);
		py = __builtin_amdgcn_readfirstlane(xy.y);
	} else {
		const int nrx = (A.pw + 3) >> 2;
		const int region = li >> 4, k = li & 15;
		const int rx = region % nrx, ry = region / nrx;
		const int cx = rx * 4 + (k & 3), cy = ry * 4 + (k >> 2);
		if(cx >= A.pw || cy >= A.ph) {
			if(A.slotCost && fi == 0 && lane == 0 && (unsigned)li < (unsigned)A.nSlots) A.slotCost[li] = 0;
			return;
		}
		px = A.x0 + cx * 16;
		py = A.y0 + cy * 16;
		pidx = cy * A.pw + cx;
	}

	const u64 tStart = DIAG ? __builtin_amdgcn_s_memtime() : 0;
	Quad Q;
	const int ty = lane >> 2, k4 = lane & 3;
#if SNAIL_ARITH_SSE
	{
		float p[3][4], pp[4], rs[4], dn[12], idn[12];
#pragma unroll
		for(int l = 0; l < 4; l++) {
			const float xoff = (float)(px + (l >= 2 ? 2 : 0));
			const float yoff = (float)(py - (l >= 2 ? 1 : 0));
			const float tposx = (float)(4 * k4) + xoff;
			const float tposy = (float)ty + yoff;
#pragma unroll
			for(int c = 0; c < 3; c++) p[c][l] = G.tright[c] * tposx + (G.tup[c] * tposy + G.txyz[c][l]);
			pp[l] = p[0][l] * p[0][l] + p[1][l] * p[1][l] + p[2][l] * p[2][l];
		}
		RSqrtN<4>(pp, rs);
#pragma unroll
		for(int l = 0; l < 4; l++)
#pragma unroll
			for(int c = 0; c < 3; c++) { Q.d[c][l] = p[c][l] * rs[l]; dn[c * 4 + l] = Q.d[c][l] + 0.00000001f; }
		InvN<12>(dn, idn);
#pragma unroll
		for(int l = 0; l < 4; l++) {
#pragma unroll
			for(int c = 0; c < 3; c++) Q.id[c][l] = idn[c * 4 + l];
			Q.dist[l] = __builtin_inff();
		}
	}
#else
#pragma unroll
	for(int l = 0; l < 4; l++) {
		const float xoff = (float)(px + (l >= 2 ? 2 : 0));
		const float yoff = (float)(py - (l >= 2 ? 1 : 0));
		const float tposx = (float)(4 * k4) + xoff;
		const float tposy = (float)ty + yoff;
		const float p0 = G.tright[0] * tposx + (G.tup[0] * tposy + G.txyz[0][l]);
		const float p1 = G.tright[1] * tposx + (G.tup[1] * tposy + G.txyz[1][l]);
		const float p2 = G.tright[2] * tposx + (G.tup[2] * tposy + G.txyz[2][l]);
		const float rs = RSqrt(p0 * p0 + p1 * p1 + p2 * p2);
		Q.d[0][l] = p0 * rs; Q.d[1][l] = p1 * rs; Q.d[2][l] = p2 * rs;
#pragma unroll
		for(int c = 0; c < 3; c++) Q.id[c][l] = Inv(Q.d[c][l] + 0.00000001f);
		Q.dist[l] = __builtin_inff();
	}
#endif
	int tid[4] = {0, 0, 0, 0};
	float bu[4] = {0, 0, 0, 0}, bv[4] = {0, 0, 0, 0};
	float org[3][4];
#pragma unroll
	for(int c = 0; c < 3; c++)
#pragma unroll
		for(int l = 0; l < 4; l++) org[c][l] = G.org[c];

	Counters st = {0, 0, 0, 0, 0};
	int oct;
	const int mode = classify(A.fastOK != 0, finite4(Q.id) && finite4(Q.d), true, Q.id, Q.dist, oct);
	if(EXACTPASS) walk<true, false, false, M_EXACT, false, DEEP, true>(A.nodes, A.tris, 64, lane, org, Q, 15u, tid, bu, bv, lds, st);
	else if(mode == M_EXACT) {
		if(lane == 0) A.defer[2 + atomicAdd(&A.defer[0], 1)] = fi * A.nSlots + li;
		return;
	} else if(DEEP) {
		if(mode == M_COH) walk<true, false, false, M_COH, false, DEEP, true>(A.nodes, A.tris, 64, lane, org, Q, 15u, tid, bu, bv, lds, st, oct);
		else walk<true, false, false, M_FAST, false, DEEP, true>(A.nodes, A.tris, 64, lane, org, Q, 15u, tid, bu, bv, lds, st);
	} else if(A.pack && !DIAG) {
		const uint4 *pn = A.rel[fi];
		if(mode == M_COH) walkSharedAsm<false, true, true, false, false, true>(pn, A.tris, 64, lane, org, Q, 15u, tid, bu, bv, lds, st, oct);
		else walkSharedAsm<false, false, true, false, false, true>(pn, A.tris, 64, lane, org, Q, 15u, tid, bu, bv, lds, st, 0);
	} else if(mode == M_COH) walkSharedAsm<false, true, false, false, false, true>(A.nodes, A.tris, 64, lane, org, Q, 15u, tid, bu, bv, lds, st, oct);
	else walkSharedAsm<false, false, false, false, false, true>(A.nodes, A.tris, 64, lane, org, Q, 15u, tid, bu, bv, lds, st, 0);
	const PrimaryArgsK E = lateArgs();
	const FrameOutK F = &E->out[fi];
	if(F->u || F->v) finalBarycentrics(E->tris, org, Q, tid, bu, bv);

	flushStats(E->stats, st, 256u, lane);
	if(PSTATS && fi == 0) bookPacket(E->pstats, (size_t)pidx, st, 256u, lane);
	if(E->slotCost && fi == 0 && lane == 0) E->slotCost[li] = (int)st.iters;
	if(DIAG && E->cost && lane == 0) {
		const u64 tEnd = __builtin_amdgcn_s_memtime();
		unsigned *c = E->cost + (size_t)pidx * 8;
		c[0] = st.iters; c[1] = st.intersects; c[2] = (unsigned)(tEnd - tStart); c[3] = (unsigned)(tStart >> 6);
		c[4] = st.fetched; c[5] = st.leaves; c[6] = 0; c[7] = 0;
	}

	if(F->bgr) {
		unsigned bytes[12];
#pragma unroll
		for(int l = 0; l < 4; l++) {
			const float dist = InvDiv(Q.dist[l]);
			bytes[l * 3 + 0] = (unsigned)convChannelW(dist * 2.0f); bytes[l * 3 + 1] = (unsigned)convChannelW(dist * 250.0f); bytes[l * 3 + 2] = (unsigned)convChannelW(dist * 20.0f);
		}
		unsigned *o = (unsigned *)(F->bgr + ((size_t)pidx * 256 + (size_t)lane * 4) * 3);
#pragma unroll
		for(int k = 0; k < 3; k++) o[k] = bytes[4 * k] | (bytes[4 * k + 1] << 8) | (bytes[4 * k + 2] << 16) | (bytes[4 * k + 3] << 24);
	}
	if(E->packetXY || E->packetMajor) {
		const size_t o = (size_t)pidx * 256 + (size_t)lane * 4;
		if(F->t) *(float4 *)(F->t + o) = make_float4(Q.dist[0], Q.dist[1], Q.dist[2], Q.dist[3]);
		if(F->u) *(float4 *)(F->u + o) = make_float4(bu[0], bu[1], bu[2], bu[3]);
		if(F->v) *(float4 *)(F->v + o) = make_float4(bv[0], bv[1], bv[2], bv[3]);
		if(F->id) *(int4 *)(F->id + o) = make_int4(tid[0], tid[1], tid[2], tid[3]);
	} else {
		const int yy = py + ty, xx = px + k4 * 4;
		const int xlim = min(E->resx, E->x0 + E->w), ylim = min(E->resy, E->y0 + E->h);
		if(yy < ylim) {
			const size_t o = (size_t)yy * E->resx + xx;
			if(xx + 3 < xlim && (E->resx & 3) == 0) {
				if(F->t) *(float4 *)(F->t + o) = make_float4(Q.dist[0], Q.dist[1], Q.dist[2], Q.dist[3]);
				if(F->u) *(float4 *)(F->u + o) = make_float4(bu[0], bu[1], bu[2], bu[3]);
				if(F->v) *(float4 *)(F->v + o) = make_float4(bv[0], bv[1], bv[2], bv[3]);
				if(F->id) *(int4 *)(F->id + o) = make_int4(tid[0], tid[1], tid[2], tid[3]);
			} else {
#pragma unroll
				for(int l = 0; l < 4; l++)
					if(xx + l < xlim) {
						if(F->t) F->t[o + l] = Q.dist[l];
						if(F->u) F->u[o + l] = bu[l];
						if(F->v) F->v[o + l] = bv[l];
						if(F->id) F->id[o + l] = tid[l];
					}
			}
		}
	}
}

#ifndef SNAIL_PRIMARY_WAVES
#define SNAIL_PRIMARY_WAVES 6
#endif
template <bool DEEP, bool PSTATS = false>
__global__ __launch_bounds__(64) __attribute__((amdgpu_waves_per_eu(SNAIL_PRIMARY_WAVES))) void k_primary(PrimaryArgs A) {
	__shared__ float lds[LDS_FLOATS_PER_WAVE];
	int b = (int)blockIdx.x;
	int fi = 0;
	if(A.nFrames > 1) {
		const int t = b >> 3;
		fi = t % A.nFrames;
		b = ((t / A.nFrames) << 3) | (b & 7);
	}
	int li = interleave16(b);
	if(A.order) {
		if(b >= A.nSlots) return;
		li = __builtin_amdgcn_readfirstlane(A.order[b]);
		if((unsigned)li >= (unsigned)A.nSlots) return;
	}
	primaryPacket<DEEP, false, false, PSTATS>(A, li, fi, lds);
}
template <bool DEEP>
__global__ __launch_bounds__(64) __attribute__((amdgpu_waves_per_eu(SNAIL_PRIMARY_WAVES))) void k_primary_diag(PrimaryArgs A) {
	__shared__ float lds[LDS_FLOATS_PER_WAVE];
	primaryPacket<DEEP, false, true>(A, interleave16((int)blockIdx.x), 0, lds);
}

#if SNAIL_ARITH_SSE && defined(SNAIL_DEBUG_API)
__global__ __launch_bounds__(256) void k_hostsse_sums(const unsigned *tables , int fn, unsigned firstChunk, u64 *sums) {
	const unsigned x0 = (firstChunk + blockIdx.x) << 16;
	u64 s = 0;
	for(unsigned k = 0; k < 256u; k++) {
		const unsigned x = x0 + k * 256u + threadIdx.x;
		s += hostSseMix(x, fn == 0 ? __float_as_uint(rcpHost(__uint_as_float(x))) : __float_as_uint(rsqrtHost(__uint_as_float(x))));
	}
	atomicAdd(&sums[blockIdx.x], s);
}
#endif

#define ORDER_THREADS_LDS 256
#define ORDER_LDS_MAX_SLOTS 49152
#ifndef SNAIL_ORDER_ADAPTIVE
#define SNAIL_ORDER_ADAPTIVE 3
#endif
__device__ __forceinline__ void orderSortBlock(const int *__restrict__ cost , int n, int *__restrict__ order, int flags ) {
	__builtin_amdgcn_s_setprio(3);
	constexpr int T = ORDER_THREADS_LDS, BPT = 4096 / T;
	extern __shared__ unsigned stash32[];
	unsigned short *stash = (unsigned short *)stash32;
	__shared__ int bins[4096];
	__shared__ int waveSum[T / 64];
	__shared__ int maxCost;
	const int tid = (int)threadIdx.x, lane = tid & 63, wv = tid >> 6;
	if(tid == 0) maxCost = 0;
#pragma unroll
	for(int k = 0; k < BPT; k++) bins[k * T + tid] = 0;
	const int nFull = n >> 2;
	const int4 *cost4 = (const int4 *)cost;
	int m = 0;
	for(int j0 = 0; j0 < nFull; j0 += 4 * T) {
		int4 v[4];
#pragma unroll
		for(int k = 0; k < 4; k++) { const int idx = j0 + k * T + tid; v[k] = idx < nFull ? cost4[idx] : make_int4(0, 0, 0, 0); }
#pragma unroll
		for(int k = 0; k < 4; k++) {
			const int idx = j0 + k * T + tid;
			const int a = min(max(v[k].x, 0), 65535), b = min(max(v[k].y, 0), 65535), c = min(max(v[k].z, 0), 65535), d = min(max(v[k].w, 0), 65535);
			m = max(max(m, max(a, b)), max(c, d));
			if(idx < nFull) { stash32[idx * 2] = (unsigned)a | ((unsigned)b << 16); stash32[idx * 2 + 1] = (unsigned)c | ((unsigned)d << 16); }
		}
	}
	for(int i = nFull * 4 + tid; i < n; i += T) { const int a = min(max(cost[i], 0), 65535); m = max(m, a); stash[i] = (unsigned short)a; }
#pragma unroll
	for(int d = 32; d >= 1; d >>= 1) m = max(m, __shfl_xor(m, d));
	__syncthreads();
	if(lane == 0) atomicMax(&maxCost, m);
	__syncthreads();
	int shift = 0;
	while((maxCost >> shift) > 4095) shift++;
	int mySum = 0;
	for(int i = tid; i < n; i += T) { const int c16 = (int)stash[i]; mySum += c16; atomicAdd(&bins[4095 - min(c16 >> shift, 4095)], 1); }
	__shared__ unsigned sumCost;
	__shared__ int p99Class;
#pragma unroll
	for(int d = 32; d >= 1; d >>= 1) mySum += __shfl_xor(mySum, d);
	if(tid == 0) { sumCost = 0; p99Class = 4095; }
	__syncthreads();
	if(lane == 0) atomicAdd(&sumCost, (unsigned)mySum);
	int sum = 0;
#pragma unroll
	for(int k = 0; k < BPT; k++) sum += bins[tid * BPT + k];
	int incl = sum;
#pragma unroll
	for(int d = 1; d < 64; d <<= 1) { const int o = __shfl_up(incl, d); if(lane >= d) incl += o; }
	if(lane == 63) waveSum[wv] = incl;
	__syncthreads();
	int run = incl - sum;
	for(int w = 0; w < wv; w++) run += waveSum[w];
	__shared__ int cutClass, heavyCount;
	const int p99Want = max(n / 100, 1);
	if(tid == 0) { cutClass = 4096; heavyCount = n; }
	__syncthreads();
#pragma unroll
// ... 977 lines not shown
	while((unsigned)(__builtin_amdgcn_s_memrealtime() - r0) < ticks) __builtin_amdgcn_s_sleep(1);
	const u64 c1 = __builtin_amdgcn_s_memtime(), r1 = __builtin_amdgcn_s_memrealtime();
	if(threadIdx.x == 0) { out[0] = c1 - c0; out[1] = r1 - r0; }
}

__global__ __launch_bounds__(256) void k_recip_check(unsigned base, unsigned long long *out) {
	const unsigned bits = base + blockIdx.x * 256u + threadIdx.x;
	const float x = __uint_as_float(bits);
	const float ref = 1.0f / x, got = recipExact(x);
	const bool same = (ref != ref) ? (got != got) : __float_as_uint(ref) == __float_as_uint(got);
	const bool inside = ((bits & 0x7f800000u) - 0x00800000u) < 0x7e000000u;
	const u64 bad = __builtin_amdgcn_ballot_w64(!same), in = __builtin_amdgcn_ballot_w64(inside);
	if((threadIdx.x & 63) == 0) {
		if(bad) atomicAdd(&out[0], (unsigned long long)__builtin_popcountll(bad));
		if(in) atomicAdd(&out[1], (unsigned long long)__builtin_popcountll(in));
	}
}

__global__ void k_nop(int *sink) { if(sink && threadIdx.x == 0 && blockIdx.x == 0x7fffffff) *sink = 1; }
#endif

__host__ __device__ inline void pfEncode(const unsigned (&in)[8], unsigned (&out)[8], unsigned trisOff) {
	for(int k = 0; k < 6; k++) out[k] = in[k];
	if(in[6] & 0x80000000u) { out[6] = 0x80000000u | (trisOff + ((in[6] & 0x7fffffffu) << 6)); out[7] = in[7]; }
	else { out[6] = (in[6] + 1u + (in[7] >> 16)) << 5; out[7] = 1u << (in[7] & 3u); }
}
__global__ __launch_bounds__(256) void k_pf_encode(const uint4 *__restrict__ nodes, int nNodes, unsigned trisOff, uint4 *__restrict__ pf) {
	const int i = (int)(blockIdx.x * 256 + threadIdx.x);
	if(i >= nNodes) return;
	const uint4 a = nodes[(size_t)i * 2], b = nodes[(size_t)i * 2 + 1];
	const unsigned in[8] = {a.x, a.y, a.z, a.w, b.x, b.y, b.z, b.w};
	unsigned out[8];
	pfEncode(in, out, trisOff);
	pf[(size_t)(i + 1) * 2] = make_uint4(out[0], out[1], out[2], out[3]);
	pf[(size_t)(i + 1) * 2 + 1] = make_uint4(out[4], out[5], out[6], out[7]);
}

__host__ __device__ inline bool relOriginInside(const unsigned (&w)[6]) {
	bool in = true;
	for(int k = 0; k < 3; k++) {
		const float n = __builtin_bit_cast(float, w[k]), f = __builtin_bit_cast(float, w[3 + k]);
		in = in && n <= 0.0f && f >= 0.0f;
	}
	return in;
}
__host__ __device__ inline unsigned relAux(const unsigned (&rel)[6], unsigned sub, unsigned aux) {
	const bool leaf = (sub & 0x80000000u) != 0;
	if(!leaf && !(aux & 7u)) return aux;
	unsigned bits = 0;
	for(int c = 0; c < 3; c++) {
		if(__builtin_bit_cast(float, rel[c]) > 0.0f) bits |= 1u << (SNAIL_REL_NEARPOS_BIT + c);
		if(__builtin_bit_cast(float, rel[3 + c]) < 0.0f) bits |= 1u << (SNAIL_REL_FARNEG_BIT + c);
	}
	return !leaf && relOriginInside(rel) ? aux | (1u << SNAIL_REL_INSIDE_BIT) : aux | bits;
}
__global__ __launch_bounds__(256) void k_rel_nodes(const uint4 *__restrict__ pf, int nSlots, float ox, float oy, float oz, uint4 *__restrict__ rel) {
	const int i = (int)(blockIdx.x * 256 + threadIdx.x);
	if(i >= nSlots) return;
	const uint4 a = pf[(size_t)i * 2], b = pf[(size_t)i * 2 + 1];
	const float o[3] = {ox, oy, oz};
	const unsigned in[6] = {a.x, a.y, a.z, a.w, b.x, b.y};
	unsigned out[6];
	for(int k = 0; k < 6; k++) out[k] = __float_as_uint(__uint_as_float(in[k]) - o[k % 3]);
	rel[(size_t)i * 2] = make_uint4(out[0], out[1], out[2], out[3]);
	rel[(size_t)i * 2 + 1] = make_uint4(out[4], out[5], b.z, relAux(out, b.z, b.w));
}

struct RelFillArgs {
	int n;
	float org[SNAIL_MAX_BATCH][3];
	uint4 *dst[SNAIL_MAX_BATCH];
};
__global__ __launch_bounds__(256) void k_rel_nodes_multi(const uint4 *__restrict__ pf, int nSlots, RelFillArgs A) {
	const int i = (int)(blockIdx.x * 256 + threadIdx.x);
	if(i >= nSlots) return;
	const uint4 a = pf[(size_t)i * 2], b = pf[(size_t)i * 2 + 1];
	const unsigned in[6] = {a.x, a.y, a.z, a.w, b.x, b.y};
	for(int f = 0; f < A.n; f++) {
		unsigned out[6];
		for(int k = 0; k < 6; k++) out[k] = __float_as_uint(__uint_as_float(in[k]) - A.org[f][k % 3]);
		A.dst[f][(size_t)i * 2] = make_uint4(out[0], out[1], out[2], out[3]);
		A.dst[f][(size_t)i * 2 + 1] = make_uint4(out[4], out[5], b.z, relAux(out, b.z, b.w));
	}
}
#ifdef SNAIL_DEBUG_API
__global__ __launch_bounds__(256) void k_rel_flag_count(const uint4 *__restrict__ rel, int nSlots, unsigned long long *__restrict__ out) {
	const int i = (int)(blockIdx.x * 256 + threadIdx.x);
	const bool flagged = i < nSlots && !(rel[(size_t)i * 2 + 1].z & 0x80000000u) && ((rel[(size_t)i * 2 + 1].w >> SNAIL_REL_INSIDE_BIT) & 1u);
	const u64 m = __builtin_amdgcn_ballot_w64(flagged);
	if((threadIdx.x & 63) == 0 && m) atomicAdd(out, (unsigned long long)__builtin_popcountll(m));
}
__global__ __launch_bounds__(256) void k_rel_axis_flag_count(const uint4 *__restrict__ rel, int nSlots, unsigned long long *__restrict__ out) {
	const int i = (int)(blockIdx.x * 256 + threadIdx.x);
	const unsigned w = i < nSlots ? rel[(size_t)i * 2 + 1].w : 0u;
	for(int k = 0; k < 3; k++) {
		const u64 lo = __builtin_amdgcn_ballot_w64((w >> (SNAIL_REL_NEARPOS_BIT + 2 * k)) & 1u), hi = __builtin_amdgcn_ballot_w64((w >> (SNAIL_REL_NEARPOS_BIT + 2 * k + 1)) & 1u);
		if((threadIdx.x & 63) == 0 && (lo | hi)) atomicAdd(out + k, (unsigned long long)__builtin_popcountll(lo) | (unsigned long long)__builtin_popcountll(hi) << 32);
	}
}
#endif

struct AccountArgs {
	const uint4 *nodes, *tris;
	GenConst g;
	int x0, y0, pw, ph;
	u64 *out;
};
__global__ __launch_bounds__(256) void k_account(AccountArgs A) {
	const int lane = threadIdx.x & 63;
	const int p = (int)blockIdx.x * 4 + (int)(threadIdx.x >> 6);
	if(p >= A.pw * A.ph) return;
	const int px = A.x0 + (p % A.pw) * 16, py = A.y0 + (p / A.pw) * 16;
	const int ty = lane >> 2, k4 = lane & 3;
	const float inf = __builtin_inff();
	unsigned vn = 0, vt = 0, hits = 0;
	for(int l = 0; l < 4; l++) {
		const float xoff = (float)(px + (l >= 2 ? 2 : 0)), yoff = (float)(py - (l >= 2 ? 1 : 0));
		const float tposx = (float)(4 * k4) + xoff, tposy = (float)ty + yoff;
		float pp[3], d[3], id[3];
		for(int c = 0; c < 3; c++) pp[c] = A.g.tright[c] * tposx + (A.g.tup[c] * tposy + A.g.txyz[c][l]);
		const float rs = 1.0f / __builtin_sqrtf(pp[0] * pp[0] + pp[1] * pp[1] + pp[2] * pp[2]);
		for(int c = 0; c < 3; c++) { d[c] = pp[c] * rs; id[c] = 1.0f / (d[c] + 0.00000001f); }
		const int sg[3] = {d[0] < 0.0f, d[1] < 0.0f, d[2] < 0.0f};
		int stack[SNAIL_MAX_DEPTH + 2], sp = 0;
		stack[sp++] = 0;
		float dist = inf;
		while(sp) {
			int cur = stack[--sp];
			for(;;) {
				const uint4 *np = A.nodes + (size_t)cur * 2;
				const uint4 a = np[0], b = np[1];
				const float bmin[3] = {asf(a.x), asf(a.y), asf(a.z)}, bmax[3] = {asf(a.w), asf(b.x), asf(b.y)};
				vn++;
				float lmin = 0.0f, lmax = 0.0f;
				for(int k = 0; k < 3; k++) {
					float l1 = id[k] * (bmin[k] - A.g.org[k]), l2 = id[k] * (bmax[k] - A.g.org[k]);
					float lo = Min<M_EXACT>(l1, l2), hi = Max<M_EXACT>(l1, l2);
					if(k == 0) { lmin = lo; lmax = hi; }
					else { lmin = Max<M_EXACT>(lmin, lo); lmax = Min<M_EXACT>(lmax, hi); }
				}
				if(lmax < 0.0f || lmin > Min<M_EXACT>(lmax, dist)) break;
				if(b.z & 0x80000000u) {
					const int count = (int)b.w, firstTri = (int)(b.z & 0x7fffffffu);
					for(int k = 0; k < count; k++) {
						const Tri t = loadTriVector(A.tris, firstTri + k);
						vt++;
						float tv[3] = {A.g.org[0] - t.a[0], A.g.org[1] - t.a[1], A.g.org[2] - t.a[2]};
						float t0v[3] = {(t.ba[1] * tv[2] - t.ba[2] * tv[1]) * t.it0, (t.ba[2] * tv[0] - t.ba[0] * tv[2]) * t.it0,
										(t.ba[0] * tv[1] - t.ba[1] * tv[0]) * t.it0};
						float t1v[3] = {(tv[1] * t.ca[2] - tv[2] * t.ca[1]) * t.it0, (tv[2] * t.ca[0] - tv[0] * t.ca[2]) * t.it0,
										(tv[0] * t.ca[1] - tv[1] * t.ca[0]) * t.it0};
						const float tmul = -(tv[0] * t.n[0] + tv[1] * t.n[1] + tv[2] * t.n[2]);
						const float det = d[0] * t.n[0] + d[1] * t.n[1] + d[2] * t.n[2];
						const float v = d[0] * t0v[0] + d[1] * t0v[1] + d[2] * t0v[2];
						const float u = d[0] * t1v[0] + d[1] * t1v[1] + d[2] * t1v[2];
						const float duv = det - u - v;
						const float uvmin = Min<M_EXACT>(u, Min<M_EXACT>(v, duv)), uvmax = Max<M_EXACT>(u, Max<M_EXACT>(v, duv));
						if(!(uvmax <= 0.0f || uvmin >= 0.0f)) continue;
						const float t2 = (1.0f / det) * tmul;
						if(t2 < dist && t2 > 0.0f) dist = t2;
					}
					break;
				}
				const int child = (int)b.z, axis = (int)(b.w & 0xffff), fn = (int)((b.w >> 16) & 0xffff) ^ sg[axis];
				stack[sp++] = child + (fn ^ 1);
				cur = child + fn;
// ... 14 lines not shown
```

### snail_amd/csrc/snail_hip.hip

```cpp
#include <hip/hip_runtime.h>
#include <hip/hip_ext.h>

#include <cmath>
#include <cstdarg>
#include <cstdio>
#include <algorithm>
#include <cstring>
#include <memory>
#include <mutex>
#include <utility>
#include <vector>

#include "../../include/snail_hip.h"
#include "../../include/snail_instances.h"
#include "../../include/snail_bvh_fast.h"
#include "host_sse.h"
#ifdef SNAIL_DEBUG_API
#include "../../include/snail_hip_debug.h"
#endif

static thread_local char g_err[1024] = "";

void snail_set_error(const char *fmt, ...) {
	va_list ap;
	va_start(ap, fmt);
	vsnprintf(g_err, sizeof(g_err), fmt, ap);
	va_end(ap);
}

#define HIP_TRY(expr)                                                                                     \
	do {                                                                                                  \
		hipError_t e_ = (expr);                                                                           \
		if(e_ != hipSuccess) {                                                                            \
			snail_set_error("%s failed: %s (%s:%d)", #expr, hipGetErrorString(e_), __FILE__, __LINE__);  \
			return 100 + (int)e_;                                                                         \
		}                                                                                                 \
	} while(0)

#define SNAIL_DEV_NS dev
#define SNAIL_ARITH_SSE 0
#include "snail_dev.inc"
#include "instances.inc"
#include "instances_shade.inc"
#include "materials.inc"
#include "instances_materials.inc"
#include "instances_materials_bounce.inc"
#include "materials_transparency.inc"
#include "materials_tree.inc"
#undef SNAIL_DEV_NS
#undef SNAIL_ARITH_SSE
#define SNAIL_DEV_NS dev_sse
#define SNAIL_ARITH_SSE 1
#include "snail_dev.inc"
#include "instances.inc"
#include "instances_shade.inc"
#include "materials.inc"
#include "instances_materials.inc"
#include "instances_materials_bounce.inc"
#include "materials_transparency.inc"
#include "materials_tree.inc"
#undef SNAIL_DEV_NS
#undef SNAIL_ARITH_SSE
#include "heatmap.inc"
#include "build_common.inc"
#include "instances_build.inc"
#include "materials_dynamic.inc"

#define SNAIL_LAUNCH(SSE, ARGS_T, GRID, BLOCK, LDS, STREAM, A, ...)                                                                          \
	do {                                                                                                                                   \
		if(SSE) {                                                                                                                          \
			dev_sse::ARGS_T a_;                                                                                                            \
			static_assert(sizeof(a_) == sizeof(A), "argument records of the two arithmetics differ");                                      \
			memcpy((void *)&a_, (const void *)&(A), sizeof(a_));                                                                           \
			hipLaunchKernelGGL((dev_sse::__VA_ARGS__), GRID, BLOCK, LDS, STREAM, a_);                                                      \
		} else hipLaunchKernelGGL((dev::__VA_ARGS__), GRID, BLOCK, LDS, STREAM, A);                                                        \
	} while(0)

namespace { struct TileJob; void freeTileJobs(SnailScene *); }
struct SnailSceneFast;
namespace { int fastSceneBegin(SnailScene *, hipStream_t); void fastSceneEnd(SnailScene *, hipStream_t); void fastFree(SnailSceneFast *); int fastCurrent(const SnailScene *, int cur[4]); }
struct SnailScene {
	int device = 0;
	int arith = SNAIL_ARITH_IEEE;
	unsigned *dTab = nullptr;
	unsigned tabGen = 0;
	TileJob *tileJob = nullptr, *frameJob = nullptr;
	SnailSceneFast *fast = nullptr;
	int nNodes = 0, nTris = 0, depth = 0;
	uint4 *dNodes = nullptr, *dTris = nullptr;
	char *dPF = nullptr;
	int trisOff = 0;
	struct RelNodes {
		float org[3] = {0, 0, 0};
		uint4 *d = nullptr;
		bool valid = false;
		unsigned long long stamp = 0;
		hipEvent_t filled = nullptr;
		enum { kStreams = 8 };
		hipStream_t usedOn[kStreams] = {};
		hipEvent_t used[kStreams] = {};
		int nUsed = 0;
	};
	enum { kRelSlots = 40 };
	RelNodes rel[kRelSlots];
	unsigned long long relClock = 0;
	int pfOK = 0;
	int fastOK = 0;
	int nestedOK = 1;
	int pfOKButNesting = 0;
	int lastBlocks = 0, lastThreads = 0;
#ifndef SNAIL_DEFER_SLOTS
#define SNAIL_DEFER_SLOTS 8
#endif
	enum { kDeferSlots = SNAIL_DEFER_SLOTS };
	int *dDefer[kDeferSlots] = {};
	hipEvent_t deferDone[kDeferSlots] = {};
	bool deferUsed[kDeferSlots] = {};
	int deferCap = 0;
	unsigned launchCount = 0;
	struct ShadeScratch {
		size_t packets = 0;
		bool refl = false;
		float *hitT = nullptr; int *hitId = nullptr;
		float *rOrg = nullptr, *rDir = nullptr, *rIDir = nullptr, *rDist = nullptr, *rCol = nullptr;
		int *rObj = nullptr;
		unsigned char *rMask = nullptr;
		int *defer = nullptr;
		float *sDist = nullptr;
		unsigned *pstats = nullptr;
		int *heatXY = nullptr;
		hipEvent_t done = nullptr;
		bool used = false;
	} shade[kDeferSlots];
	unsigned shadeCount = 0;
	struct RayDefer { int *p = nullptr; size_t cap = 0; hipEvent_t done = nullptr; bool used = false; } rayDefer[kDeferSlots];
	unsigned rayCount = 0;
	std::mutex mu;
	std::mutex renderMu;
	struct HostCall {
		hipStream_t stream = nullptr;
		unsigned long long *dStats = nullptr;
		char *arena = nullptr;
		size_t cap = 0, used = 0;
	};
	std::vector<HostCall *> hostFree;
};

namespace {

struct DeviceGuard {
	int prev = -1;
	bool ok = true;
	explicit DeviceGuard(int dev) {
		if(hipGetDevice(&prev) != hipSuccess) prev = -1;
		if(prev != dev) ok = hipSetDevice(dev) == hipSuccess;
	}
	~DeviceGuard() {
		int cur = -1;
		if(prev >= 0 && hipGetDevice(&cur) == hipSuccess && cur != prev) (void)hipSetDevice(prev);
	}
};

struct HostCallScope {
	SnailScene *s;
	SnailScene::HostCall *c = nullptr;
	int rc = 0;
	bool finished = false;
	HostCallScope(SnailScene *scene, const char *fn) : s(scene) {
		{
			std::lock_guard<std::mutex> lock(s->mu);
			if(!s->hostFree.empty()) { c = s->hostFree.back(); s->hostFree.pop_back(); }
		}
		if(!c) {
			c = new SnailScene::HostCall();
			hipError_t e = hipStreamCreateWithFlags(&c->stream, hipStreamNonBlocking);
			if(e == hipSuccess) e = hipMalloc((void **)&c->dStats, 4 * sizeof(unsigned long long));
			if(e != hipSuccess) {
				snail_set_error("%s: per-call stream / counters: %s", fn, hipGetErrorString(e));
				if(c->stream) (void)hipStreamDestroy(c->stream);
				delete c; c = nullptr; rc = 100 + (int)e;
			}
		}
		if(c) c->used = 0;
	}
	~HostCallScope() {
		if(!c) return;
		if(!finished) (void)hipStreamSynchronize(c->stream);
		std::lock_guard<std::mutex> lock(s->mu);
// ... 60 lines not shown
	if(*dTab && *tabGen == gen) return 0;
	if(!*dTab) HIP_TRY(hipMalloc((void **)dTab, snap.size() * sizeof(unsigned)));
	HIP_TRY(hipDeviceSynchronize());
	HIP_TRY(hipMemcpy(*dTab, snap.data(), snap.size() * sizeof(unsigned), hipMemcpyHostToDevice));
	*tabGen = gen;
	return 0;
}
int hostSseDeviceTables(const char *fn, const unsigned **out, bool capturing = false) {
	static std::mutex mu;
	static unsigned *tab[64] = {};
	static unsigned gen[64] = {};
	int devId = 0;
	HIP_TRY(hipGetDevice(&devId));
	if(devId < 0 || devId >= 64) { snail_set_error("%s: device index %d", fn, devId); return 1; }
	std::lock_guard<std::mutex> lock(mu);
	if(capturing) {
		unsigned now = 0;
		const char *why = "";
		if(hostSseSnapshot(nullptr, &now, &why)) { snail_set_error("%s: SNAIL_ARITH_HOST_SSE is not available on this host: %s", fn, why); return 2; }
		if(!tab[devId] || gen[devId] != now) {
			snail_set_error("%s: this device's copy of the rcpps / rsqrtps tables is missing or stale and the stream is being captured: call snail_arith_prepare_device() before the capture", fn);
			return 3;
		}
	} else if(int rc = hostSseFill(fn, &tab[devId], &gen[devId])) return rc;
	*out = tab[devId];
	return 0;
}

bool originSane(const float *o) {
	for(int c = 0; c < 3; c++)
		if(!(std::fabs(o[c]) <= 1.0e9f)) return false;
	return true;
}

#ifdef SNAIL_DEBUG_API
int debugEnvInt(const char *name) { const char *v = getenv(name); return v ? atoi(v) : 0; }
#else
constexpr int debugEnvInt(const char *) { return 0; }
#endif

bool useDeep(const SnailScene *s) {
	static const bool force = debugEnvInt("SNAIL_DEBUG_FORCE_DEEP") != 0;
	return force || s->depth > 62;
}

int stackPack(const SnailScene *s) {
	static const bool off = debugEnvInt("SNAIL_DEBUG_NO_PACK") != 0;
	static const bool assumeNested = debugEnvInt("SNAIL_DEBUG_ASSUME_NESTED") != 0;
	return !off && (s->pfOK || (assumeNested && s->pfOKButNesting)) ? 1 : 0;
}

struct RelPending {
	dev::RelFillArgs fill;
	int entry[SNAIL_MAX_BATCH];
};
int relFor(SnailScene *s, const float org[3], hipStream_t stream, const uint4 **out, int *which, RelPending *pend = nullptr) {
	SnailScene::RelNodes *hit = nullptr, *victim = nullptr;
	for(auto &e : s->rel) {
		if(e.valid && memcmp(e.org, org, 12) == 0) { hit = &e; break; }
		if(!victim || (!e.valid && victim->valid) || (e.valid == victim->valid && e.stamp < victim->stamp)) victim = &e;
	}
	if(hit) {
		HIP_TRY(hipStreamWaitEvent(stream, hit->filled, 0));
		hit->stamp = ++s->relClock;
		*out = hit->d; *which = (int)(hit - s->rel);
		return 0;
	}
	SnailScene::RelNodes &e = *victim;
	const int nSlots = s->nNodes + 1;
	if(!e.d) HIP_TRY(hipMalloc((void **)&e.d, (size_t)nSlots * 32));
	if(!e.filled) HIP_TRY(hipEventCreateWithFlags(&e.filled, hipEventDisableTiming));
	HIP_TRY(hipStreamWaitEvent(stream, e.filled, 0));
	for(int k = 0; k < e.nUsed; k++) HIP_TRY(hipStreamWaitEvent(stream, e.used[k], 0));
	e.nUsed = 0;
	if(pend && pend->fill.n < SNAIL_MAX_BATCH) {
		const int k = pend->fill.n++;
		memcpy(pend->fill.org[k], org, 12); pend->fill.dst[k] = e.d; pend->entry[k] = (int)(&e - s->rel);
	} else {
		hipLaunchKernelGGL(dev::k_rel_nodes, dim3((unsigned)((nSlots + 255) / 256)), dim3(256), 0, stream, (const uint4 *)s->dPF, nSlots, org[0], org[1], org[2], e.d);
		HIP_TRY(hipGetLastError());
		HIP_TRY(hipEventRecord(e.filled, stream));
	}
	memcpy(e.org, org, 12); e.valid = true; e.stamp = ++s->relClock;
	*out = e.d; *which = (int)(&e - s->rel);
	return 0;
}
void relDrop(SnailScene *s, RelPending &pend) {
	for(int k = 0; k < pend.fill.n; k++) s->rel[pend.entry[k]].valid = false;
	pend.fill.n = 0;
}
int relFlush(SnailScene *s, RelPending &pend, hipStream_t stream) {
	if(pend.fill.n == 0) return 0;
	const int nSlots = s->nNodes + 1;
	hipLaunchKernelGGL(dev::k_rel_nodes_multi, dim3((unsigned)((nSlots + 255) / 256)), dim3(256), 0, stream, (const uint4 *)s->dPF, nSlots, pend.fill);
	hipError_t e = hipGetLastError();
	for(int k = 0; k < pend.fill.n && e == hipSuccess; k++) e = hipEventRecord(s->rel[pend.entry[k]].filled, stream);
	if(e != hipSuccess) {
		relDrop(s, pend);
		snail_set_error("origin-relative node records: %s", hipGetErrorString(e));
		return 100 + (int)e;
	}
	pend.fill.n = 0;
	return 0;
}
int relUsed(SnailScene *s, int which, hipStream_t stream) {
	SnailScene::RelNodes &e = s->rel[which];
	int k = 0;
	while(k < e.nUsed && e.usedOn[k] != stream) k++;
	if(k == e.nUsed) {
		if(e.nUsed == SnailScene::RelNodes::kStreams) {
			HIP_TRY(hipStreamWaitEvent(stream, e.used[0], 0));
			k = 0;
		} else e.nUsed++;
		e.usedOn[k] = stream;
		if(!e.used[k]) HIP_TRY(hipEventCreateWithFlags(&e.used[k], hipEventDisableTiming));
	}
	HIP_TRY(hipEventRecord(e.used[k], stream));
	return 0;
}

struct SceneUse {
	SnailScene *s; hipStream_t st; int rc = 0;
	SceneUse(SnailScene *scene, hipStream_t stream) : s(scene), st(stream) { if(s->fast) rc = fastSceneBegin(s, st); }
	~SceneUse() { if(s->fast) fastSceneEnd(s, st); }
	SceneUse(const SceneUse &) = delete;
	SceneUse &operator=(const SceneUse &) = delete;
};

int checkScene(const SnailScene *s, const char *fn) {
	if(!s || !s->dNodes || !s->dPF || !s->dTris) { snail_set_error("%s: invalid scene handle", fn); return 1; }
	return 0;
}

#define SNAIL_LOCK(s) std::lock_guard<std::mutex> snailLock_((s)->mu)

struct FrameSet {
	int n = 0;
	const float *cam[SNAIL_MAX_BATCH] = {};
	dev::FrameOut out[SNAIL_MAX_BATCH] = {};
};

enum { SORT_IN_LAUNCH_MAX = 20480 };
struct ExactPass {
	dim3 grid, block;
	size_t lds = 0;
	int *nextOrder = nullptr;
	int orderFlags = 0;
	bool sortAfter = false;
};
ExactPass exactPassFor(int exactBlocks, const int32_t *dSlotCost, int nSlots, int32_t *dNextOrder, int orderFlags) {
	ExactPass e;
	e.orderFlags = orderFlags;
	e.grid = dim3((unsigned)exactBlocks); e.block = dim3(64);
	if(!dNextOrder || !dSlotCost || nSlots <= 0) return e;
	if(nSlots <= SORT_IN_LAUNCH_MAX && ((uintptr_t)dSlotCost & 15) == 0) {
		e.grid = dim3((unsigned)exactBlocks + 1); e.block = dim3(ORDER_THREADS_LDS);
		e.lds = (size_t)((nSlots + 3) / 4 * 4) * 2;
		e.nextOrder = (int *)dNextOrder;
	} else e.sortAfter = true;
	return e;
}

int launchPrimaryFrames(SnailScene *s, const FrameSet &FS, int resx, int resy, int x0, int y0, int w, int h, const int32_t *dPacketXY, int nPackets, uint64_t *dStats,
						hipStream_t stream, unsigned *dCost = nullptr, bool packetMajor = false, const int32_t *dOrder = nullptr, int32_t *dSlotCost = nullptr,
						int32_t *dNextOrder = nullptr, int orderFlags = 0, uint32_t *dPacketStats = nullptr) {
	if(resx <= 0 || resy <= 0) { snail_set_error("snail_trace_primary: bad resolution %dx%d", resx, resy); return 1; }
	if(dNextOrder && !dSlotCost) { snail_set_error("snail_trace_primary: the next dispatch order is derived from d_slot_cost, which is null"); return 1; }
	if(FS.n < 1 || FS.n > SNAIL_MAX_BATCH) { snail_set_error("snail_trace_primary: 1..%d frames per launch (got %d)", SNAIL_MAX_BATCH, FS.n); return 1; }
	SceneUse use(s, stream);
	if(use.rc) return use.rc;
	dev::PrimaryArgs A;
	memset(&A, 0, sizeof(A));
	A.hostTab = s->arith == SNAIL_ARITH_HOST_SSE ? s->dTab : nullptr;
	A.nodes = s->dNodes; A.tris = s->dTris; A.pf = (const uint4 *)s->dPF;
	A.nFrames = FS.n;
	A.fastOK = s->fastOK;
	for(int k = 0; k < FS.n; k++) {
		A.g[k] = makeGen(FS.cam[k], resx, resy);
		A.out[k] = FS.out[k];
		A.fastOK = A.fastOK && originSane(FS.cam[k]);
	}
	A.resx = resx; A.resy = resy;
	A.stats = (dev::u64 *)dStats;
	A.cost = dCost;
	A.pstats = dPacketStats;
	A.packetMajor = packetMajor ? 1 : 0;
	A.pack = stackPack(s);
	int relWhich[SNAIL_MAX_BATCH];
	for(int k = 0; k < FS.n; k++) { relWhich[k] = -1; A.rel[k] = nullptr; }
	int blocks;
	if(dPacketXY) {
		if(nPackets <= 0) return 0;
		A.packetXY = (const int2 *)dPacketXY;
		A.nPackets = nPackets;
		blocks = ((nPackets + 127) / 128) * 128;
	} else {
		if((x0 & 15) || (y0 & 15) || w <= 0 || h <= 0 || x0 < 0 || y0 < 0) {
			snail_set_error("snail_trace_primary: rect origin must be a non-negative multiple of 16 and the size positive (got %d,%d %dx%d)", x0, y0, w, h);
			return 1;
		}
		A.x0 = x0; A.y0 = y0; A.w = w; A.h = h;
		A.pw = (w + 15) / 16; A.ph = (h + 15) / 16;
		A.nPackets = A.pw * A.ph;
		const int nRegions = ((A.pw + 3) / 4) * ((A.ph + 3) / 4);
		blocks = ((nRegions + 7) / 8) * 8 * 16;
	}
	A.nBlocks = blocks;
	A.nSlots = dPacketXY ? nPackets : blocks;
	A.order = dOrder; A.slotCost = dSlotCost;
	if(A.pack && !useDeep(s)) {
		RelPending pend;
		pend.fill.n = 0;
		for(int k = 0; k < FS.n; k++)
			if(int rc = relFor(s, FS.cam[k], stream, &A.rel[k], &relWhich[k], &pend)) { relDrop(s, pend); return rc; }
		if(int rc = relFlush(s, pend, stream)) return rc;
	}
	const int gridBlocks = blocks * FS.n;
	s->lastBlocks = gridBlocks; s->lastThreads = 64;
	if(gridBlocks + 2 > s->deferCap) {
		HIP_TRY(hipDeviceSynchronize());
		for(int k = 0; k < SnailScene::kDeferSlots; k++) {
			if(s->dDefer[k]) (void)hipFree(s->dDefer[k]);
			s->dDefer[k] = nullptr;
			HIP_TRY(hipMalloc((void **)&s->dDefer[k], (size_t)(gridBlocks + 2) * sizeof(int)));
			HIP_TRY(hipMemset(s->dDefer[k], 0, 2 * sizeof(int)));
		}
		HIP_TRY(hipDeviceSynchronize());
		s->deferCap = gridBlocks + 2;
	}
	const int slot = (int)(s->launchCount++ % SnailScene::kDeferSlots);
	A.defer = s->dDefer[slot];
	if(!s->deferDone[slot]) HIP_TRY(hipEventCreateWithFlags(&s->deferDone[slot], hipEventDisableTiming));
	if(s->deferUsed[slot]) HIP_TRY(hipStreamWaitEvent(stream, s->deferDone[slot], 0));
	static const int dynLds = debugEnvInt("SNAIL_DEBUG_DYNLDS");
	const int exactBlocks = A.fastOK ? (blocks < 8 ? blocks : 8) : (blocks < 2048 ? blocks : 2048);
	const dim3 grid(gridBlocks), block(64);
	const ExactPass EP = exactPassFor(exactBlocks, dSlotCost, A.nSlots, dCost ? nullptr : dNextOrder, orderFlags);
	A.nextOrder = EP.nextOrder; A.nextOrderFlags = EP.orderFlags;
	const bool sse = s->arith == SNAIL_ARITH_HOST_SSE;
	if(dCost) {
		if(useDeep(s)) SNAIL_LAUNCH(sse, PrimaryArgs, dim3(blocks), dim3(64), 0, stream, A, k_primary_diag<true>);
		else SNAIL_LAUNCH(sse, PrimaryArgs, dim3(blocks), dim3(64), 0, stream, A, k_primary_diag<false>);
	} else if(A.pstats) {
		if(useDeep(s)) SNAIL_LAUNCH(sse, PrimaryArgs, grid, block, dynLds, stream, A, k_primary<true, true>);
		else SNAIL_LAUNCH(sse, PrimaryArgs, grid, block, dynLds, stream, A, k_primary<false, true>);
	} else if(useDeep(s)) SNAIL_LAUNCH(sse, PrimaryArgs, grid, block, dynLds, stream, A, k_primary<true>);
	else SNAIL_LAUNCH(sse, PrimaryArgs, grid, block, dynLds, stream, A, k_primary<false>);
	static const bool noExact = debugEnvInt("SNAIL_DEBUG_NO_EXACT_PASS") != 0;
	if(noExact && s->arith == SNAIL_ARITH_IEEE && !EP.nextOrder && !EP.sortAfter) { }
	else if(A.pstats) {
		if(useDeep(s)) SNAIL_LAUNCH(sse, PrimaryArgs, EP.grid, EP.block, EP.lds, stream, A, k_primary_exact<true, true>);
		else SNAIL_LAUNCH(sse, PrimaryArgs, EP.grid, EP.block, EP.lds, stream, A, k_primary_exact<false, true>);
	} else if(useDeep(s)) SNAIL_LAUNCH(sse, PrimaryArgs, EP.grid, EP.block, EP.lds, stream, A, k_primary_exact<true>);
	else SNAIL_LAUNCH(sse, PrimaryArgs, EP.grid, EP.block, EP.lds, stream, A, k_primary_exact<false>);
	HIP_TRY(hipGetLastError());
	if(EP.sortAfter) { if(int rc = snail_order_from_cost_hint_dev(dSlotCost, A.nSlots, dNextOrder, EP.orderFlags, stream)) return rc; }
	HIP_TRY(hipEventRecord(s->deferDone[slot], stream));
	s->deferUsed[slot] = true;
	for(int k = 0; k < FS.n; k++)
		if(relWhich[k] >= 0) { if(int rc = relUsed(s, relWhich[k], stream)) return rc; }
	return 0;
}

int launchPrimary(SnailScene *s, const float cam[13], int resx, int resy, int x0, int y0, int w, int h, const int32_t *dPacketXY,
				  int nPackets, float *t, float *u, float *v, int32_t *id, uint64_t *dStats, hipStream_t stream, unsigned *dCost = nullptr,
				  bool packetMajor = false, uint8_t *dBgr = nullptr, const int32_t *dOrder = nullptr, int32_t *dSlotCost = nullptr, int32_t *dNextOrder = nullptr, int orderFlags = 0,
				  uint32_t *dPacketStats = nullptr) {
	FrameSet FS;
	FS.n = 1; FS.cam[0] = cam;
	FS.out[0].t = t; FS.out[0].u = u; FS.out[0].v = v; FS.out[0].id = (int *)id; FS.out[0].bgr = dBgr;
	return launchPrimaryFrames(s, FS, resx, resy, x0, y0, w, h, dPacketXY, nPackets, dStats, stream, dCost, packetMajor, dOrder, dSlotCost, dNextOrder, orderFlags, dPacketStats);
}

int shadeScratch(SnailScene *s, SnailScene::ShadeScratch &W, size_t packets, size_t blocks, bool refl) {
	if(W.hitT && W.packets >= packets && (W.refl || !refl)) return 0;
	HIP_TRY(hipDeviceSynchronize());
	if(W.hitT) (void)hipFree(W.hitT);
	const hipEvent_t keep = W.done;
	W = SnailScene::ShadeScratch();
	W.done = keep;
	const size_t rays = packets * 256, quads = packets * 64;
	const size_t deferInts = blocks * SNAIL_MAX_LIGHTS + 16;
	size_t bytes = rays * 8 + deferInts * 4 + rays * 4 * SNAIL_MAX_LIGHTS + packets * 32;
	if(refl) bytes += quads * 12 * 4 * 3 + rays * 4 * 2 + rays * 12 + quads;
	char *base = nullptr;
	HIP_TRY(hipMalloc((void **)&base, bytes));
	W.packets = packets; W.refl = refl;
	W.hitT = (float *)base; base += rays * 4;
	W.hitId = (int *)base; base += rays * 4;
	W.defer = (int *)base; base += deferInts * 4;
	HIP_TRY(hipMemset(W.defer, 0, 16 * sizeof(int)));
	HIP_TRY(hipDeviceSynchronize());
	W.sDist = (float *)base; base += rays * 4 * SNAIL_MAX_LIGHTS;
	W.pstats = (unsigned *)base; base += packets * 16;
	W.heatXY = (int *)base; base += packets * 16;
	if(refl) {
		W.rOrg = (float *)base; base += quads * 48;
		W.rDir = (float *)base; base += quads * 48;
		W.rIDir = (float *)base; base += quads * 48;
		W.rDist = (float *)base; base += rays * 4;
		W.rObj = (int *)base; base += rays * 4;
		W.rCol = (float *)base; base += rays * 12;
		W.rMask = (unsigned char *)base;
	}
	return 0;
}

template <bool SHARED, bool MASK>
void launchRaysKernels(const SnailScene *s, const dev::RaysArgs &A, int blocks, const ExactPass &EP, hipStream_t stream) {
	const bool deep = useDeep(s), bary = A.bary != nullptr, sse = s->arith == SNAIL_ARITH_HOST_SSE;
#define SNAIL_RAYS_LAUNCH(D, B)                                                                                                            \
	do {                                                                                                                                   \
		SNAIL_LAUNCH(sse, RaysArgs, dim3(blocks), dim3(64), 0, stream, A, k_rays<SHARED, MASK, D, B>);                                      \
		SNAIL_LAUNCH(sse, RaysArgs, EP.grid, EP.block, EP.lds, stream, A, k_rays_exact<SHARED, MASK, D, B>);                                \
	} while(0)
	if(deep && bary) SNAIL_RAYS_LAUNCH(true, true);
	else if(deep) SNAIL_RAYS_LAUNCH(true, false);
	else if(bary) SNAIL_RAYS_LAUNCH(false, true);
	else SNAIL_RAYS_LAUNCH(false, false);
#undef SNAIL_RAYS_LAUNCH
}

int launchRays(SnailScene *s, bool shadow, int nPackets, int size, int sharedOrigin, const float *origin, const float *dir,
					  const float *idir, const uint8_t *mask, float *distance, int32_t *object, float *bary, uint64_t *dStats, hipStream_t stream,
					  const int32_t *dOrder = nullptr, int32_t *dSlotCost = nullptr, int nSlots = 0, int32_t *dNextOrder = nullptr, int orderFlags = 0,
					  uint32_t *dPacketStats = nullptr) {
	if(nPackets <= 0) return 0;
	if(size < 1 || size > SNAIL_PACKET_QUADS) { snail_set_error("packet size %d outside 1..%d quads", size, SNAIL_PACKET_QUADS); return 1; }
	if(!origin || !dir || !idir || !distance || (!shadow && !object)) { snail_set_error("null ray array"); return 1; }
	SceneUse use(s, stream);
	if(use.rc) return use.rc;
	dev::RaysArgs A;
	memset(&A, 0, sizeof(A));
	A.hostTab = s->arith == SNAIL_ARITH_HOST_SSE ? s->dTab : nullptr;
	A.nodes = s->dNodes; A.tris = s->dTris; A.pf = (const uint4 *)s->dPF;
	A.nPackets = nPackets; A.size = size; A.fastOK = s->fastOK; A.pack = stackPack(s);
	A.origin = origin; A.dir = dir; A.idir = idir; A.mask = mask;
	A.distance = distance; A.object = object; A.bary = bary;
	A.stats = (dev::u64 *)dStats;
	A.pstats = shadow ? nullptr : dPacketStats;
	int blocks = ((nPackets + 127) / 128) * 128;
	if(!shadow && (dOrder || dSlotCost) && nSlots >= nPackets) {
		A.order = dOrder; A.slotCost = dSlotCost; A.nSlots = nSlots;
// ... 179 lines not shown
		for(int i = 0; i < nNodes; i++) {
			unsigned in[8], out[8];
			for(int k = 0; k < 8; k++) in[k] = nw[(size_t)i * 8 + k];
			dev::pfEncode(in, out, (unsigned)trisOff);
			for(int k = 0; k < 8; k++) pf[((size_t)i + 1) * 8 + k] = out[k];
		}
	}
	hipError_t e;
	if((e = hipMalloc((void **)&s->dNodes, (size_t)nNodes * 32)) != hipSuccess || (e = hipMalloc((void **)&s->dPF, fits ? pfBytes : (size_t)nTris * 64)) != hipSuccess ||
	   (e = hipMemcpy(s->dNodes, nodes32, (size_t)nNodes * 32, hipMemcpyHostToDevice)) != hipSuccess ||
	   (e = hipMemcpy(s->dPF + s->trisOff, tris64, (size_t)nTris * 64, hipMemcpyHostToDevice)) != hipSuccess ||
	   (!pf.empty() && (e = hipMemcpy(s->dPF, pf.data(), pf.size() * 4, hipMemcpyHostToDevice)) != hipSuccess)) {
		snail_set_error("snail_scene_create: %s", hipGetErrorString(e));
		snail_scene_destroy(s);
		return nullptr;
	}
	s->dTris = (uint4 *)(s->dPF + s->trisOff);
	return s;
}

SnailScene *snail_scene_create_lbvh(const float *tri_verts, int nTris, int device, int maxLeafTris, int32_t *perm, float *build_ms) {
	if(!tri_verts || nTris <= 0 || maxLeafTris < 1 || maxLeafTris > 64) { snail_set_error("snail_scene_create_lbvh: bad arguments (1 <= maxLeafTris <= 64)"); return nullptr; }
	DeviceGuard guard(device);
	if(!guard.ok) { snail_set_error("snail_scene_create_lbvh: hipSetDevice(%d) failed", device); return nullptr; }
	uint4 *dNodes = nullptr, *dTris = nullptr;
	int depth = 0, fastOK = 0;
	if(buildLbvhDevice(tri_verts, nTris, maxLeafTris, &dNodes, &dTris, perm, &depth, &fastOK, build_ms)) return nullptr;
	if(depth > SNAIL_MAX_DEPTH) {
		(void)hipFree(dNodes); (void)hipFree(dTris);
		snail_set_error("snail_scene_create_lbvh: depth %d exceeds BVH::maxDepth %d", depth, SNAIL_MAX_DEPTH);
		return nullptr;
	}
	SnailScene *s = new SnailScene();
	s->device = device; s->nNodes = 2 * nTris - 1; s->nTris = nTris; s->depth = depth; s->fastOK = fastOK;
	s->dNodes = dNodes;
	const size_t trisOff = pfTrisOffset(s->nNodes), pfBytes = trisOff + (size_t)nTris * 64;
	const bool fits = pfFits((size_t)s->nNodes + 1, (size_t)nTris);
	s->trisOff = (int)(fits ? trisOff : 0);
	s->nestedOK = 1; s->pfOKButNesting = s->pfOK = fits ? 1 : 0;
	hipError_t e;
	if((e = hipMalloc((void **)&s->dPF, fits ? pfBytes : (size_t)nTris * 64)) != hipSuccess ||
	   (e = hipMemcpy(s->dPF + s->trisOff, dTris, (size_t)nTris * 64, hipMemcpyDeviceToDevice)) != hipSuccess) {
		(void)hipFree(dTris);
		snail_set_error("snail_scene_create_lbvh: %s", hipGetErrorString(e));
		snail_scene_destroy(s);
		return nullptr;
	}
	(void)hipFree(dTris);
	s->dTris = (uint4 *)(s->dPF + s->trisOff);
	if(fits) {
		(void)hipMemset(s->dPF, 0, 32);
		hipLaunchKernelGGL(dev::k_pf_encode, dim3((unsigned)((s->nNodes + 255) / 256)), dim3(256), 0, 0, s->dNodes, s->nNodes, (unsigned)trisOff, (uint4 *)s->dPF);
		if((e = hipDeviceSynchronize()) != hipSuccess) {
			snail_set_error("snail_scene_create_lbvh: %s", hipGetErrorString(e));
			snail_scene_destroy(s);
			return nullptr;
		}
	}
	return s;
}

int snail_scene_download(const SnailScene *s, void *nodes32, void *tris64) {
	if(int rc = checkScene(s, "snail_scene_download")) return rc;
	DeviceGuard guard(s->device);
	int nNodes = s->nNodes;
	if(s->fast) {
		int cur[4];
		if(int rc = fastCurrent(s, cur)) return rc;
		nNodes = cur[0];
	}
	if(nodes32) HIP_TRY(hipMemcpy(nodes32, s->dNodes, (size_t)nNodes * 32, hipMemcpyDeviceToHost));
	if(tris64) HIP_TRY(hipMemcpy(tris64, s->dTris, (size_t)s->nTris * 64, hipMemcpyDeviceToHost));
	return 0;
}

void snail_scene_destroy(SnailScene *s) {
	if(!s) return;
	DeviceGuard guard(s->device);
	freeTileJobs(s);
	if(s->dNodes) (void)hipFree(s->dNodes);
	if(s->dPF) (void)hipFree(s->dPF);
	if(s->dTab) (void)hipFree(s->dTab);
	fastFree(s->fast);
	for(auto &e : s->rel) {
		if(e.d) (void)hipFree(e.d);
		if(e.filled) (void)hipEventDestroy(e.filled);
		for(hipEvent_t ev : e.used) if(ev) (void)hipEventDestroy(ev);
	}
	for(SnailScene::HostCall *c : s->hostFree) {
		if(c->arena) (void)hipFree(c->arena);
		if(c->dStats) (void)hipFree(c->dStats);
		if(c->stream) (void)hipStreamDestroy(c->stream);
		delete c;
	}
	for(int k = 0; k < SnailScene::kDeferSlots; k++) if(s->dDefer[k]) (void)hipFree(s->dDefer[k]);
	for(int k = 0; k < SnailScene::kDeferSlots; k++) if(s->shade[k].hitT) (void)hipFree(s->shade[k].hitT);
	for(int k = 0; k < SnailScene::kDeferSlots; k++) {
		if(s->rayDefer[k].p) (void)hipFree(s->rayDefer[k].p);
		if(s->rayDefer[k].done) (void)hipEventDestroy(s->rayDefer[k].done);
		if(s->deferDone[k]) (void)hipEventDestroy(s->deferDone[k]);
		if(s->shade[k].done) (void)hipEventDestroy(s->shade[k].done);
	}
	delete s;
}

int snail_scene_info(const SnailScene *s, int *nNodes, int *nTris, int *depth, int *device) {
	if(!s) { snail_set_error("snail_scene_info: null scene"); return 1; }
	int cur[4] = {s->nNodes, s->depth, 0, 0};
	if(s->fast) { if(int rc = fastCurrent(s, cur)) return rc; }
	if(nNodes) *nNodes = cur[0];
	if(nTris) *nTris = s->nTris;
	if(depth) *depth = cur[1];
	if(device) *device = s->device;
	return 0;
}

int snail_scene_flags(const SnailScene *s, int *fastOK, int *nestedOK) {
	if(!s) { snail_set_error("snail_scene_flags: null scene"); return 1; }
	if(fastOK) *fastOK = s->fastOK;
	if(nestedOK) *nestedOK = s->nestedOK;
	return 0;
}

int snail_scene_set_arith(SnailScene *s, int arith) {
	if(int rc = checkScene(s, "snail_scene_set_arith")) return rc;
	if(arith != SNAIL_ARITH_IEEE && arith != SNAIL_ARITH_HOST_SSE) { snail_set_error("snail_scene_set_arith: unknown arithmetic %d", arith); return 1; }
	SNAIL_LOCK(s);
	if(arith == SNAIL_ARITH_HOST_SSE) {
		DeviceGuard guard(s->device);
		if(!guard.ok) { snail_set_error("snail_scene_set_arith: hipSetDevice(%d) failed", s->device); return 1; }
		if(int rc = hostSseFill("snail_scene_set_arith", &s->dTab, &s->tabGen)) return rc;
	}
	s->arith = arith;
	return 0;
}
int snail_scene_arith(const SnailScene *s, int *arith) {
	if(int rc = checkScene(s, "snail_scene_arith")) return rc;
	if(arith) *arith = s->arith;
	return 0;
}
int snail_arith_set_tables(const uint32_t *tables12288) {
	const char *why = "";
	if(hostSseSetTables(tables12288, &why)) { snail_set_error("snail_arith_set_tables: %s", why); return 1; }
	return 0;
}
int snail_arith_prepare_device(void) {
	const unsigned *tab = nullptr;
	return hostSseDeviceTables("snail_arith_prepare_device", &tab);
}
int snail_host_sse_tables(uint32_t *tables12288) {
	const char *why = "";
	if(hostSseSnapshot((unsigned *)tables12288, nullptr, &why)) { snail_set_error("snail_host_sse_tables: %s", why); return 2; }
	return 0;
}
int snail_host_sse_check(int fn, uint64_t first, uint64_t count, int threads, uint64_t *mismatches, uint32_t *firstBad) {
	if((fn != 0 && fn != 1) || first > (1ull << 32) || count > (1ull << 32) - first || !mismatches) { snail_set_error("snail_host_sse_check: bad arguments"); return 1; }
	const char *why = "";
	if(hostSseSnapshot(nullptr, nullptr, &why)) { snail_set_error("snail_host_sse_check: %s", why); return 2; }
	unsigned bad = 0;
	*mismatches = hostSseMismatches(fn, first, count, threads, &bad);
	if(firstBad) *firstBad = bad;
	return 0;
}

int snail_last_launch(const SnailScene *s, int *blocks, int *threads) {
	if(!s) { snail_set_error("snail_last_launch: null scene"); return 1; }
	std::lock_guard<std::mutex> lock(const_cast<SnailScene *>(s)->mu);
	if(blocks) *blocks = s->lastBlocks;
	if(threads) *threads = s->lastThreads;
	return 0;
}
// ... 597 lines not shown
	HIP_TRY(hipStreamCreateWithFlags(&st, hipStreamNonBlocking));
	int relWhich = -1;
	if(A.pack && !useDeep(s)) {
		if(int rc = relFor(s, cam, st, &A.rel[0], &relWhich)) return rc;
	}
	hipEvent_t e0, e1;
	HIP_TRY(hipEventCreate(&e0)); HIP_TRY(hipEventCreate(&e1));
	HIP_TRY(hipDeviceSynchronize());
	HIP_TRY(hipEventRecord(e0, st));
	for(int f = 0; f < frames; f++)
		hipExtLaunchKernelGGL(dev::k_primary<false>, dim3(blocks), dim3(64), 0, st, nullptr, nullptr, (unsigned)flags, A);
	HIP_TRY(hipGetLastError());
	HIP_TRY(hipEventRecord(e1, st));
	HIP_TRY(hipStreamSynchronize(st));
	HIP_TRY(hipEventElapsedTime(ms_total, e0, e1));
	(void)hipEventDestroy(e0); (void)hipEventDestroy(e1); (void)hipStreamDestroy(st);
	return 0;
}

int snail_debug_occupancy(int out[4]) {
	if(!out) { snail_set_error("snail_debug_occupancy: null output"); return 1; }
	int dev = 0;
	HIP_TRY(hipGetDevice(&dev));
	int perCU = 0, maxBlocks = 0, cus = 0;
	HIP_TRY(hipOccupancyMaxActiveBlocksPerMultiprocessor(&perCU, (const void *)dev::k_primary<false>, 64, 0));
	HIP_TRY(hipDeviceGetAttribute(&maxBlocks, hipDeviceAttributeMaxBlocksPerMultiProcessor, dev));
	HIP_TRY(hipDeviceGetAttribute(&cus, hipDeviceAttributeMultiprocessorCount, dev));
	out[0] = perCU; out[1] = maxBlocks; out[2] = cus; out[3] = 1;
	return 0;
}

int snail_debug_rel_flag_count(SnailScene *s, const float org[3], int *count) {
	if(int rc = checkScene(s, "snail_debug_rel_flag_count")) return rc;
	if(!org || !count) { snail_set_error("snail_debug_rel_flag_count: null argument"); return 1; }
	if(!stackPack(s)) { snail_set_error("snail_debug_rel_flag_count: this scene keeps no origin-relative node records"); return 1; }
	DeviceGuard guard(s->device);
	HostCallScope hc(s, "snail_debug_rel_flag_count");
	if(hc.rc) return hc.rc;
	if(int rc = hc.zeroStats()) return rc;
	{
		SNAIL_LOCK(s);
		SceneUse use(s, hc.stream());
		if(use.rc) return use.rc;
		const uint4 *rel = nullptr;
		int which = -1;
		if(int rc = relFor(s, org, hc.stream(), &rel, &which)) return rc;
		const int nSlots = s->nNodes + 1;
		hipLaunchKernelGGL(dev::k_rel_flag_count, dim3((unsigned)((nSlots + 255) / 256)), dim3(256), 0, hc.stream(), rel, nSlots, (unsigned long long *)hc.stats());
		HIP_TRY(hipGetLastError());
		if(int rc = relUsed(s, which, hc.stream())) return rc;
	}
	uint64_t st[4] = {0, 0, 0, 0};
	if(int rc = hc.finish(st)) return rc;
	*count = (int)st[0];
	return 0;
}

int snail_debug_rel_axis_flag_count(SnailScene *s, const float org[3], int out[6]) {
	if(int rc = checkScene(s, "snail_debug_rel_axis_flag_count")) return rc;
	if(!org || !out) { snail_set_error("snail_debug_rel_axis_flag_count: null argument"); return 1; }
	if(!stackPack(s)) { snail_set_error("snail_debug_rel_axis_flag_count: this scene keeps no origin-relative node records"); return 1; }
	DeviceGuard guard(s->device);
	HostCallScope hc(s, "snail_debug_rel_axis_flag_count");
	if(hc.rc) return hc.rc;
	if(int rc = hc.zeroStats()) return rc;
	{
		SNAIL_LOCK(s);
		SceneUse use(s, hc.stream());
		if(use.rc) return use.rc;
		const uint4 *rel = nullptr;
		int which = -1;
		if(int rc = relFor(s, org, hc.stream(), &rel, &which)) return rc;
		const int nSlots = s->nNodes + 1;
		hipLaunchKernelGGL(dev::k_rel_axis_flag_count, dim3((unsigned)((nSlots + 255) / 256)), dim3(256), 0, hc.stream(), rel, nSlots, (unsigned long long *)hc.stats());
		HIP_TRY(hipGetLastError());
		if(int rc = relUsed(s, which, hc.stream())) return rc;
	}
	uint64_t st[4] = {0, 0, 0, 0};
	if(int rc = hc.finish(st)) return rc;
	for(int k = 0; k < 3; k++) { out[2 * k] = (int)(st[k] & 0xffffffffu); out[2 * k + 1] = (int)(st[k] >> 32); }
	return 0;
}

#endif

int snail_account_packets(SnailScene *s, const float cam[13], int resx, int resy, uint32_t *out8) {
	if(int rc = checkScene(s, "snail_account_packets")) return rc;
	if(!out8 || resx <= 0 || resy <= 0) { snail_set_error("snail_account_packets: null output or bad resolution"); return 1; }
	DeviceGuard guard(s->device);
	HostCallScope hc(s, "snail_account_packets");
	if(hc.rc) return hc.rc;
	const size_t bytes = (size_t)((resx + 15) / 16) * ((resy + 15) / 16) * 32;
	if(int rc = hc.reserve(HostCallScope::pad(bytes))) return rc;
	void *c = hc.carve(bytes);
	HIP_TRY(hipMemsetAsync(c, 0, bytes, hc.stream()));
	{
		SNAIL_LOCK(s);
		if(int rc = launchPrimary(s, cam, resx, resy, 0, 0, resx, resy, nullptr, 0, nullptr, nullptr, nullptr, nullptr, nullptr, hc.stream(), (unsigned *)c)) return rc;
	}
	if(int rc = hc.get(out8, c, bytes)) return rc;
	return hc.finish(nullptr);
}

int snail_account_primary(SnailScene *s, const float cam[13], int resx, int resy, int x0, int y0, int w, int h, uint64_t out[4]) {
	if(int rc = checkScene(s, "snail_account_primary")) return rc;
	if((x0 & 15) || (y0 & 15) || w <= 0 || h <= 0 || !out) { snail_set_error("snail_account_primary: bad rect"); return 1; }
	DeviceGuard guard(s->device);
	HostCallScope hc(s, "snail_account_primary");
	if(hc.rc) return hc.rc;
	dev::AccountArgs A;
	A.nodes = s->dNodes; A.tris = s->dTris;
	A.g = makeGen(cam, resx, resy);
	A.x0 = x0; A.y0 = y0; A.pw = (w + 15) / 16; A.ph = (h + 15) / 16;
	A.out = (dev::u64 *)hc.stats();
	if(int rc = hc.zeroStats()) return rc;
	const int np = A.pw * A.ph;
	{
		SNAIL_LOCK(s);
		SceneUse use(s, hc.stream());
		if(use.rc) return use.rc;
		hipLaunchKernelGGL(dev::k_account, dim3((np + 3) / 4), dim3(256), 0, hc.stream(), A);
		HIP_TRY(hipGetLastError());
	}
	return hc.finish(out);
}

}

#include "bvh_fast.inc"
#include "render_host.inc"
#include "instances_host.inc"
#include "instances_tiles_host.inc"
#include "heatmap_host.inc"
#include "materials_host.inc"
#include "materials_tiles_host.inc"
#include "materials_transparency_host.inc"
#include "materials_tree_host.inc"
#include "materials_heat_host.inc"
#include "materials_dynamic_host.inc"
#include "instances_materials_host.inc"
#include "instances_materials_bounce_host.inc"
```

Measured before the change: 28030 Mrays/s.

## Cache per-camera-origin relative triangle records for primary packet leaf tests

Adds a kernel that precomputes, for each triangle, the origin-relative cross-product terms (c1, c2, tmul) for a given camera origin. These records are cached in two slots and reused by a new RELTRI primary traversal path. That path skips the per-leaf origin subtraction and cross products and replaces them with plain record loads. Records are built only when a camera origin repeats across recent launches, at the cost of an extra 64-byte-per-triangle buffer and a rebuild pass whenever the origin changes.

```diff
diff --git a/include/snail_hip_debug.h b/include/snail_hip_debug.h
--- a/include/snail_hip_debug.h
+++ b/include/snail_hip_debug.h
@@ -23,6 +23,10 @@
 
 int snail_debug_rel_axis_flag_count(SnailScene *, const float org[3], int out[6]);
 
+int snail_debug_rel_tris_counts(SnailScene *, int out[2]);
+
+int snail_debug_rel_tris_records(SnailScene *, const float org[3], uint32_t *out16);
+
 #ifdef __cplusplus
 }
 #endif
diff --git a/snail_amd/_lib.py b/snail_amd/_lib.py
--- a/snail_amd/_lib.py
+++ b/snail_amd/_lib.py
@@ -203,6 +203,8 @@
     "snail_debug_anyorder": (_I, [_VP, _F13, _I, _I, _I, _I, _VP]),
     "snail_debug_rel_flag_count": (_I, [_VP, _VP, _VP]),
     "snail_debug_rel_axis_flag_count": (_I, [_VP, _VP, _VP]),
+    "snail_debug_rel_tris_counts": (_I, [_VP, _VP]),
+    "snail_debug_rel_tris_records": (_I, [_VP, _VP, _VP]),
 }
 DEBUG_LIB_PATH = os.path.join(HERE, "libsnailhip_debug.so")
 _dbg = None
diff --git a/snail_amd/csrc/bvh_fast.inc b/snail_amd/csrc/bvh_fast.inc
--- a/snail_amd/csrc/bvh_fast.inc
+++ b/snail_amd/csrc/bvh_fast.inc
@@ -171,6 +171,7 @@
 int fastRebuildLocked(SnailScene *s, const float *dVerts, int32_t *dPerm, int32_t *dInfo, hipStream_t st) {
 	if(int rc = fastWaitUsers(s, st)) return rc;
 	for(auto &e : s->rel) e.valid = false;
+	for(auto &e : s->relTri) e.valid = false;
 	return fastEnqueue(s, dVerts, dPerm, dInfo, s->fastOK, st);
 }
 
diff --git a/snail_amd/csrc/snail_dev.inc b/snail_amd/csrc/snail_dev.inc
--- a/snail_amd/csrc/snail_dev.inc
+++ b/snail_amd/csrc/snail_dev.inc
@@ -363,6 +363,41 @@
 	}
 	return __builtin_amdgcn_ballot_w64(pass);
 }
+struct LaneDir {
+	float dmn, dmx;
+};
+template <int M>
+__device__ __forceinline__ u64 cullQuad(const uint4 *__restrict__ rtris, int count , int firstTri, int lane, const float (&)[3][4],
+										const LaneDir &ld, QuadTerms &T) {
+	const int c = lane & 3;
+	const bool active = lane < 4 * count;
+	T.n = T.t0v = T.t1v = T.tmul = 0.0f;
+	bool pass = false;
+	const float dmn = ld.dmn, dmx = ld.dmx;
+	if(active) {
+		const float *rec = (const float *)(rtris + (size_t)(firstTri + (lane >> 2)) * 4);
+		const float *rc = rec + (c == 3 ? 0 : c);
+		const float nc = rc[0], c1 = rc[3], c2 = rc[6];
+		const float t0 = rec[9], it0 = rec[10];
+		T.n = nc; T.t0v = c1 * it0; T.t1v = c2 * it0; T.tmul = rec[11];
+		float m;
+		if(M == M_EXACT) m = (nc < 0.0f ? dmn : dmx) * nc;
+		else m = vmax(dmn * nc, dmx * nc);
+		const float det = (m + quadRot<0xC9>(m)) + quadRot<0xD2>(m);
+		const float c1a = dmn * c1, c1b = dmx * c1, c2a = dmn * c2, c2b = dmx * c2;
+		const float u0p = Min<M>(c1a, c1b), u1p = Max<M>(c1a, c1b), v0p = Min<M>(c2a, c2b), v1p = Max<M>(c2a, c2b);
+		const float u0 = (u0p + quadRot<0xC9>(u0p)) + quadRot<0xD2>(u0p), u1 = (u1p + quadRot<0xC9>(u1p)) + quadRot<0xD2>(u1p);
+		const float v0 = (v0p + quadRot<0xC9>(v0p)) + quadRot<0xD2>(v0p), v1 = (v1p + quadRot<0xC9>(v1p)) + quadRot<0xD2>(v1p);
+		pass = (c == 0) & ((det < 0.0f) | ((Min<M>(u1, v1) >= 0.0f) & (u0 + v0 <= det * t0)));
+	}
+	return __builtin_amdgcn_ballot_w64(pass);
+}
+__device__ __forceinline__ LaneDir laneDir(const float (&minDir)[3], const float (&maxDir)[3]) {
+	LaneDir r;
+	r.dmn = selLanes(selLanes(minDir[0], minDir[1], 0x2222222222222222ull), minDir[2], 0x4444444444444444ull);
+	r.dmx = selLanes(selLanes(maxDir[0], maxDir[1], 0x2222222222222222ull), maxDir[2], 0x4444444444444444ull);
+	return r;
+}
 __device__ __forceinline__ void setId(int &d, int v) { d = v; }
 __device__ __forceinline__ void setId(float &d, int v) { d = __int_as_float(v); }
 template <int R> struct NarrowRays {
@@ -374,9 +409,9 @@
 	if(R == 1) out[0] = selLanes(selLanes(a0, a1, 0xaaaaaaaaaaaaaaaaull), selLanes(a2, a3, 0xaaaaaaaaaaaaaaaaull), 0xccccccccccccccccull);
 	else { out[0] = selLanes(a0, a2, 0xaaaaaaaaaaaaaaaaull); out[R - 1] = selLanes(a1, a3, 0xaaaaaaaaaaaaaaaaull); }
 }
-template <int R, int M, class TID>
+template <int R, int M, class TID, class IV >
 __device__ __forceinline__ void leafSharedNarrow(const uint4 *__restrict__ tris, int count, int firstTri, int lane, int first, int last,
-												 const float (&org)[3][4], Quad &Q, TID (&tid)[4], const Interval &iv, Counters &st) {
+												 const float (&org)[3][4], Quad &Q, TID (&tid)[4], const IV &iv, Counters &st) {
 	constexpr int LPQ = 4 / R;
 	const int width = last - first + 1;
 	const bool inRange = lane >= first && lane <= last;
@@ -454,9 +489,9 @@
 	}
 }
 
-template <int R, int M>
+template <int R, int M, class IV>
 __device__ __forceinline__ void leafSharedNarrowShadow(const uint4 *__restrict__ tris, int count, int firstTri, int lane, int first, int last,
-													   const float (&org)[3][4], Quad &Q, const Interval &iv, Counters &st) {
+													   const float (&org)[3][4], Quad &Q, const IV &iv, Counters &st) {
 	constexpr int LPQ = 4 / R;
 	const float inf = __builtin_inff();
 	const int width = last - first + 1;
@@ -498,10 +533,10 @@
 	}
 }
 
-template <bool MASK, bool SHADOW, int M, bool BARY, class TID>
+template <bool MASK, bool SHADOW, int M, bool BARY, class TID, class IV>
 __device__ __forceinline__ bool leafShared(const uint4 *__restrict__ tris, int count, int firstTri, int size, int lane, int first, int last,
 										   const float (&org)[3][4], Quad &Q, unsigned mask4, TID (&tid)[4], float (&bu)[4], float (&bv)[4],
-										   const Interval &iv, Counters &st) {
+										   const IV &iv, Counters &st) {
 	const float inf = __builtin_inff();
 	const bool inRange = lane >= first && lane <= last;
 	const int width = last - first + 1;
@@ -892,6 +927,7 @@
 	" v_sub_f32 %[pfx], " FX ", %[ox]\n v_sub_f32 %[pfy], " FY ", %[oy]\n v_sub_f32 %[pfz], " FZ ", %[oz]\n"
 #define SNAIL_PRE_NONE(NX, FX, NY, FY, NZ, FZ) ""
 #define SNAIL_ORG_SHARED() [ox] "v"(org[0][0]), [oy] "v"(org[1][0]), [oz] "v"(org[2][0])
+#define SNAIL_ORG_NONE() [onone] "i"(0)
 #define SNAIL_ORG_PERRAY()                                                                                                                 \
 	[ox0] "v"(org[0][0]), [ox1] "v"(org[0][1]), [ox2] "v"(org[0][2]), [ox3] "v"(org[0][3]), [oy0] "v"(org[1][0]), [oy1] "v"(org[1][1]),     \
 		[oy2] "v"(org[1][2]), [oy3] "v"(org[1][3]), [oz0] "v"(org[2][0]), [oz1] "v"(org[2][1]), [oz2] "v"(org[2][2]), [oz3] "v"(org[2][3])
@@ -1139,7 +1175,8 @@
 	default: SNAIL_DESCEND_ASM(PRE, ORGOPS, SLAB, TAIL, CNTPOP, CNTVISIT, "s87", "s84", "s88", "s85", "s89", "s86"); break;                             \
 	}
 
-template <bool SHADOW, bool COH, bool PACK, bool MASK, bool BARY, bool POSDIST, bool REL = true >
+template <bool SHADOW, bool COH, bool PACK, bool MASK, bool BARY, bool POSDIST, bool REL = true ,
+		  bool RELTRI = false>
 __device__ __forceinline__ void walkSharedAsm(const uint4 *__restrict__ nodes , const uint4 *__restrict__ tris, int size, int lane,
 											  const float (&org)[3][4], Quad &Q, unsigned mask4, int (&tid)[4], float (&bu)[4], float (&bv)[4], float *lds,
 											  Counters &st, const int oct) {
@@ -1154,8 +1191,11 @@
 		} else if(MASK) act4 = lane < size ? (mask4 & 15u) : 0u;
 		computeMinMax<false, (MASK || SHADOW)>(Q.d, act4, size, lane, lds, iv.minDir, iv.maxDir);
 	}
-#pragma unroll
-	for(int k = 0; k < 3; k++) { iv.minIDir[k] = iv.maxIDir[k] = 0.0f; iv.minOrg[k] = iv.maxOrg[k] = org[k][0]; }
+	static_assert(!RELTRI || (PACK && POSDIST && REL && !SHADOW && !MASK && !BARY), "relative triangle records: primary packets of the prefetching loop");
+	LaneDir ld = {0.0f, 0.0f};
+	if(RELTRI) ld = laneDir(iv.minDir, iv.maxDir);
+#pragma unroll
+	for(int k = 0; k < 3; k++) { iv.minIDir[k] = iv.maxIDir[k] = 0.0f; iv.minOrg[k] = iv.maxOrg[k] = RELTRI ? 0.0f : org[k][0]; }
 	const int signBits = __builtin_amdgcn_readfirstlane((Q.d[0][0] < 0.0f ? 1 : 0) | (Q.d[1][0] < 0.0f ? 2 : 0) | (Q.d[2][0] < 0.0f ? 4 : 0));
 	float tidBits[4];
 #pragma unroll
@@ -1173,11 +1213,13 @@
 			if(COH) {
 				if(SHADOW && REL) { SNAIL_DESCEND_PF2_OCT(SNAIL_PRE_NONE_X, SNAIL_ORG_SHARED, SNAIL_SLAB_COH_R, SNAIL_TAIL_ANY, "", SNAIL_COUNT, SNAIL_PF_LEAFREQ_SLOT0, oct) }
 				else if(SHADOW) { SNAIL_DESCEND_PF2_OCT(SNAIL_PRE_SHARED, SNAIL_ORG_SHARED, SNAIL_SLAB_COH, SNAIL_TAIL_ANY, "", SNAIL_COUNT, SNAIL_PF_LEAFREQ_TRI, oct) }
+				else if(POSDIST && RELTRI) { SNAIL_DESCEND_PF2_OCT(SNAIL_PRE_NONE_X, SNAIL_ORG_NONE, SNAIL_SLAB_COH_R, SNAIL_TAIL_POSF, SNAIL_COUNT, "", SNAIL_PF_LEAFREQ_SLOT0, oct) }
 				else if(POSDIST) { SNAIL_DESCEND_PF2_OCT(SNAIL_PRE_NONE_X, SNAIL_ORG_SHARED, SNAIL_SLAB_COH_R, SNAIL_TAIL_POSF, SNAIL_COUNT, "", SNAIL_PF_LEAFREQ_SLOT0, oct) }
 				else { SNAIL_DESCEND_PF2_OCT(SNAIL_PRE_SHARED, SNAIL_ORG_SHARED, SNAIL_SLAB_COH, SNAIL_TAIL_ANY, SNAIL_COUNT, "", SNAIL_PF_LEAFREQ_TRI, oct) }
 			} else {
 				if(SHADOW && REL) { SNAIL_DESCEND_PF2_PLAIN(SNAIL_PRE_NONE_X, SNAIL_ORG_SHARED, SNAIL_SLAB_FAST_R, SNAIL_TAIL_ANY, "", SNAIL_COUNT, SNAIL_PF_LEAFREQ_SLOT0); }
 				else if(SHADOW) { SNAIL_DESCEND_PF2_PLAIN(SNAIL_PRE_SHARED, SNAIL_ORG_SHARED, SNAIL_SLAB_FAST, SNAIL_TAIL_ANY, "", SNAIL_COUNT, SNAIL_PF_LEAFREQ_TRI); }
+				else if(POSDIST && RELTRI) { SNAIL_DESCEND_PF2_PLAIN(SNAIL_PRE_NONE_X, SNAIL_ORG_NONE, SNAIL_SLAB_FAST_R, SNAIL_TAIL_POS, SNAIL_COUNT, "", SNAIL_PF_LEAFREQ_SLOT0); }
 				else if(POSDIST) { SNAIL_DESCEND_PF2_PLAIN(SNAIL_PRE_NONE_X, SNAIL_ORG_SHARED, SNAIL_SLAB_FAST_R, SNAIL_TAIL_POS, SNAIL_COUNT, "", SNAIL_PF_LEAFREQ_SLOT0); }
 				else { SNAIL_DESCEND_PF2_PLAIN(SNAIL_PRE_SHARED, SNAIL_ORG_SHARED, SNAIL_SLAB_FAST, SNAIL_TAIL_ANY, SNAIL_COUNT, "", SNAIL_PF_LEAFREQ_TRI); }
 			}
@@ -1191,8 +1233,12 @@
 			else { SNAIL_DESCEND_ASM(SNAIL_PRE_SHARED, SNAIL_ORG_SHARED, SNAIL_SLAB_FAST, SNAIL_TAIL_ANY, SNAIL_COUNT, "", "s84", "s87", "s85", "s88", "s86", "s89"); }
 		}
 		if(leafSub == 0) break;
-		if(leafShared<MASK, SHADOW, COH ? M_COH : M_FAST, BARY>(tris, leafAux, (int)((unsigned)leafSub & 0x7fffffffu), size, lane, first, last, org, Q, mask4,
-																 tidBits, bu, bv, iv, st))
+		if constexpr(RELTRI) {
+			if(leafShared<MASK, SHADOW, COH ? M_COH : M_FAST, BARY>(tris, leafAux, (int)((unsigned)leafSub & 0x7fffffffu), size, lane, first, last, org, Q, mask4,
+																	 tidBits, bu, bv, ld, st))
+				break;
+		} else if(leafShared<MASK, SHADOW, COH ? M_COH : M_FAST, BARY>(tris, leafAux, (int)((unsigned)leafSub & 0x7fffffffu), size, lane, first, last, org, Q, mask4,
+																		tidBits, bu, bv, iv, st))
 			break;
 	}
 #pragma unroll
@@ -1253,6 +1299,54 @@
 			const Tri t = loadTriVector(tris, tid[l]);
 			const TriTerms tt = triTerms(t, org[0][0], org[1][0], org[2][0]);
 			const float det = Q.d[0][l] * t.n[0] + Q.d[1][l] * t.n[1] + Q.d[2][l] * t.n[2];
+			const float v = Q.d[0][l] * tt.t0v[0] + Q.d[1][l] * tt.t0v[1] + Q.d[2][l] * tt.t0v[2];
+			const float u = Q.d[0][l] * tt.t1v[0] + Q.d[1][l] * tt.t1v[1] + Q.d[2][l] * tt.t1v[2];
+			const float idet = Inv(det);
+			bu[l] = u * idet; bv[l] = v * idet;
+		}
+	}
+#endif
+}
+
+struct RelTriTerms {
+	float n[3], t0v[3], t1v[3];
+};
+__device__ __forceinline__ RelTriTerms loadRelTriTerms(const uint4 *rtris, int idx) {
+	const uint4 *p = rtris + (size_t)idx * 4;
+	const uint4 r0 = p[0], r1 = p[1], r2 = p[2];
+	const float it0 = asf(r2.z);
+	RelTriTerms r;
+	r.n[0] = asf(r0.x); r.n[1] = asf(r0.y); r.n[2] = asf(r0.z);
+	r.t0v[0] = asf(r0.w) * it0; r.t0v[1] = asf(r1.x) * it0; r.t0v[2] = asf(r1.y) * it0;
+	r.t1v[0] = asf(r1.z) * it0; r.t1v[1] = asf(r1.w) * it0; r.t1v[2] = asf(r2.x) * it0;
+	return r;
+}
+__device__ __forceinline__ void finalBarycentricsRel(const uint4 *__restrict__ rtris, const Quad &Q, const int (&tid)[4], float (&bu)[4], float (&bv)[4]) {
+#if SNAIL_ARITH_SSE
+	float det[4], uu[4], vv[4], idet[4];
+#pragma unroll
+	for(int l = 0; l < 4; l++) {
+		det[l] = 1.0f; uu[l] = 0.0f; vv[l] = 0.0f;
+		if(Q.dist[l] < __builtin_inff()) {
+			const RelTriTerms tt = loadRelTriTerms(rtris, tid[l]);
+			det[l] = Q.d[0][l] * tt.n[0] + Q.d[1][l] * tt.n[1] + Q.d[2][l] * tt.n[2];
+			vv[l] = Q.d[0][l] * tt.t0v[0] + Q.d[1][l] * tt.t0v[1] + Q.d[2][l] * tt.t0v[2];
+			uu[l] = Q.d[0][l] * tt.t1v[0] + Q.d[1][l] * tt.t1v[1] + Q.d[2][l] * tt.t1v[2];
+		}
+	}
+	InvN<4>(det, idet);
+#pragma unroll
+	for(int l = 0; l < 4; l++) {
+		const bool hit = Q.dist[l] < __builtin_inff();
+		bu[l] = hit ? uu[l] * idet[l] : 0.0f; bv[l] = hit ? vv[l] * idet[l] : 0.0f;
+	}
+#else
+#pragma unroll
+	for(int l = 0; l < 4; l++) {
+		bu[l] = 0.0f; bv[l] = 0.0f;
+		if(Q.dist[l] < __builtin_inff()) {
+			const RelTriTerms tt = loadRelTriTerms(rtris, tid[l]);
+			const float det = Q.d[0][l] * tt.n[0] + Q.d[1][l] * tt.n[1] + Q.d[2][l] * tt.n[2];
 			const float v = Q.d[0][l] * tt.t0v[0] + Q.d[1][l] * tt.t0v[1] + Q.d[2][l] * tt.t0v[2];
 			const float u = Q.d[0][l] * tt.t1v[0] + Q.d[1][l] * tt.t1v[1] + Q.d[2][l] * tt.t1v[2];
 			const float idet = Inv(det);
@@ -1359,6 +1453,7 @@
 	int *nextOrder;
 	int nextOrderFlags;
 	unsigned *pstats;
+	const uint4 *relTris[SNAIL_MAX_BATCH];
 };
 
 typedef const PrimaryArgs __attribute__((address_space(4))) *PrimaryArgsK;
@@ -1376,7 +1471,7 @@
 	return (((j >> 4) << 3) + xcd) * 16 + (j & 15);
 }
 
-template <bool DEEP, bool EXACTPASS, bool DIAG = false, bool PSTATS = false>
+template <bool DEEP, bool EXACTPASS, bool DIAG = false, bool PSTATS = false, bool RELTRI = false>
 __device__ __forceinline__ void primaryPacket(const PrimaryArgs &A, const int li, const int fi, float *lds) {
 	const int lane = threadIdx.x & 63;
 	const GenConst &G = A.g[fi];
@@ -1466,6 +1561,10 @@
 	} else if(DEEP) {
 		if(mode == M_COH) walk<true, false, false, M_COH, false, DEEP, true>(A.nodes, A.tris, 64, lane, org, Q, 15u, tid, bu, bv, lds, st, oct);
 		else walk<true, false, false, M_FAST, false, DEEP, true>(A.nodes, A.tris, 64, lane, org, Q, 15u, tid, bu, bv, lds, st);
+	} else if(RELTRI) {
+		const uint4 *pn = A.rel[fi], *pt = A.relTris[fi];
+		if(mode == M_COH) walkSharedAsm<false, true, true, false, false, true, true, RELTRI>(pn, pt, 64, lane, org, Q, 15u, tid, bu, bv, lds, st, oct);
+		else walkSharedAsm<false, false, true, false, false, true, true, RELTRI>(pn, pt, 64, lane, org, Q, 15u, tid, bu, bv, lds, st, 0);
 	} else if(A.pack && !DIAG) {
 		const uint4 *pn = A.rel[fi];
 		if(mode == M_COH) walkSharedAsm<false, true, true, false, false, true>(pn, A.tris, 64, lane, org, Q, 15u, tid, bu, bv, lds, st, oct);
@@ -1474,7 +1573,8 @@
 	else walkSharedAsm<false, false, false, false, false, true>(A.nodes, A.tris, 64, lane, org, Q, 15u, tid, bu, bv, lds, st, 0);
 	const PrimaryArgsK E = lateArgs();
 	const FrameOutK F = &E->out[fi];
-	if(F->u || F->v) finalBarycentrics(E->tris, org, Q, tid, bu, bv);
+	if(RELTRI) { if(F->u || F->v) finalBarycentricsRel(E->relTris[fi], Q, tid, bu, bv); }
+	else if(F->u || F->v) finalBarycentrics(E->tris, org, Q, tid, bu, bv);
 
 	flushStats(E->stats, st, 256u, lane);
 	if(PSTATS && fi == 0) bookPacket(E->pstats, (size_t)pidx, st, 256u, lane);
@@ -1530,7 +1630,7 @@
 #ifndef SNAIL_PRIMARY_WAVES
 #define SNAIL_PRIMARY_WAVES 6
 #endif
-template <bool DEEP, bool PSTATS = false>
+template <bool DEEP, bool PSTATS = false, bool RELTRI = false>
 __global__ __launch_bounds__(64) __attribute__((amdgpu_waves_per_eu(SNAIL_PRIMARY_WAVES))) void k_primary(PrimaryArgs A) {
 	__shared__ float lds[LDS_FLOATS_PER_WAVE];
 	int b = (int)blockIdx.x;
@@ -1546,7 +1646,7 @@
 		li = __builtin_amdgcn_readfirstlane(A.order[b]);
 		if((unsigned)li >= (unsigned)A.nSlots) return;
 	}
-	primaryPacket<DEEP, false, false, PSTATS>(A, li, fi, lds);
+	primaryPacket<DEEP, false, false, PSTATS, RELTRI>(A, li, fi, lds);
 }
 template <bool DEEP>
 __global__ __launch_bounds__(64) __attribute__((amdgpu_waves_per_eu(SNAIL_PRIMARY_WAVES))) void k_primary_diag(PrimaryArgs A) {
@@ -2690,6 +2790,25 @@
 		A.dst[f][(size_t)i * 2] = make_uint4(out[0], out[1], out[2], out[3]);
 		A.dst[f][(size_t)i * 2 + 1] = make_uint4(out[4], out[5], b.z, relAux(out, b.z, b.w));
 	}
+}
+__global__ __launch_bounds__(256) void k_rel_tris(const uint4 *__restrict__ tris, int nTris, float ox, float oy, float oz, uint4 *__restrict__ rel) {
+	const int i = (int)(blockIdx.x * 256 + threadIdx.x);
+	if(i >= nTris) return;
+	const Tri t = loadTriVector(tris, i);
+	const float tv[3] = {ox - t.a[0], oy - t.a[1], oz - t.a[2]};
+	float c1[3], c2[3], p[3];
+	for(int c = 0; c < 3; c++) {
+		const int c1n = (c + 1) % 3, c2n = (c + 2) % 3;
+		c1[c] = t.ba[c1n] * tv[c2n] - t.ba[c2n] * tv[c1n];
+		c2[c] = tv[c1n] * t.ca[c2n] - tv[c2n] * t.ca[c1n];
+		p[c] = tv[c] * t.n[c];
+	}
+	const float tmul = -((p[0] + p[1]) + p[2]);
+	uint4 *o = rel + (size_t)i * 4;
+	o[0] = make_uint4(__float_as_uint(t.n[0]), __float_as_uint(t.n[1]), __float_as_uint(t.n[2]), __float_as_uint(c1[0]));
+	o[1] = make_uint4(__float_as_uint(c1[1]), __float_as_uint(c1[2]), __float_as_uint(c2[0]), __float_as_uint(c2[1]));
+	o[2] = make_uint4(__float_as_uint(c2[2]), __float_as_uint(t.t0), __float_as_uint(t.it0), __float_as_uint(tmul));
+	o[3] = make_uint4(0u, 0u, 0u, 0u);
 }
 #ifdef SNAIL_DEBUG_API
 __global__ __launch_bounds__(256) void k_rel_flag_count(const uint4 *__restrict__ rel, int nSlots, unsigned long long *__restrict__ out) {
diff --git a/snail_amd/csrc/snail_hip.hip b/snail_amd/csrc/snail_hip.hip
--- a/snail_amd/csrc/snail_hip.hip
+++ b/snail_amd/csrc/snail_hip.hip
@@ -100,10 +100,16 @@
 		hipStream_t usedOn[kStreams] = {};
 		hipEvent_t used[kStreams] = {};
 		int nUsed = 0;
+		unsigned launches = 0;
+		unsigned long long lastPrimary = 0;
 	};
 	enum { kRelSlots = 40 };
 	RelNodes rel[kRelSlots];
 	unsigned long long relClock = 0;
+	enum { kRelTriSlots = 2, kRelTriRecent = 2 };
+	unsigned long long primarySeq = 0;
+	RelNodes relTri[kRelTriSlots];
+	unsigned relTriBuilt = 0;
 	int pfOK = 0;
 	int fastOK = 0;
 	int nestedOK = 1;
@@ -330,6 +336,7 @@
 		HIP_TRY(hipEventRecord(e.filled, stream));
 	}
 	memcpy(e.org, org, 12); e.valid = true; e.stamp = ++s->relClock;
+	e.launches = 0;
 	*out = e.d; *which = (int)(&e - s->rel);
 	return 0;
 }
@@ -351,8 +358,9 @@
 	pend.fill.n = 0;
 	return 0;
 }
-int relUsed(SnailScene *s, int which, hipStream_t stream) {
-	SnailScene::RelNodes &e = s->rel[which];
+int relUsed(SnailScene::RelNodes &e, hipStream_t stream);
+int relUsed(SnailScene *s, int which, hipStream_t stream) { return relUsed(s->rel[which], stream); }
+int relUsed(SnailScene::RelNodes &e, hipStream_t stream) {
 	int k = 0;
 	while(k < e.nUsed && e.usedOn[k] != stream) k++;
 	if(k == e.nUsed) {
@@ -364,6 +372,38 @@
 		if(!e.used[k]) HIP_TRY(hipEventCreateWithFlags(&e.used[k], hipEventDisableTiming));
 	}
 	HIP_TRY(hipEventRecord(e.used[k], stream));
+	return 0;
+}
+
+int relTrisFor(SnailScene *s, const float org[3], bool build, unsigned long long clock0, hipStream_t stream, const uint4 **out, int *which) {
+	*out = nullptr; *which = -1;
+	SnailScene::RelNodes *victim = nullptr;
+	for(auto &e : s->relTri) {
+		if(e.valid && memcmp(e.org, org, 12) == 0) {
+			HIP_TRY(hipStreamWaitEvent(stream, e.filled, 0));
+			e.stamp = ++s->relClock;
+			*out = e.d; *which = (int)(&e - s->relTri);
+			return 0;
+		}
+		if(e.valid && e.stamp > clock0) continue;
+		if(!victim || (!e.valid && victim->valid) || (e.valid == victim->valid && e.stamp < victim->stamp)) victim = &e;
+	}
+	if(!build || !victim) return 0;
+	hipStreamCaptureStatus cap = hipStreamCaptureStatusNone;
+	if(stream && (hipStreamIsCapturing(stream, &cap) != hipSuccess || cap != hipStreamCaptureStatusNone)) { (void)hipGetLastError(); return 0; }
+	SnailScene::RelNodes &e = *victim;
+	if(!e.d) HIP_TRY(hipMalloc((void **)&e.d, (size_t)s->nTris * 64));
+	if(!e.filled) HIP_TRY(hipEventCreateWithFlags(&e.filled, hipEventDisableTiming));
+	e.valid = false;
+	HIP_TRY(hipStreamWaitEvent(stream, e.filled, 0));
+	for(int k = 0; k < e.nUsed; k++) HIP_TRY(hipStreamWaitEvent(stream, e.used[k], 0));
+	e.nUsed = 0;
+	hipLaunchKernelGGL(dev::k_rel_tris, dim3((unsigned)((s->nTris + 255) / 256)), dim3(256), 0, stream, (const uint4 *)s->dTris, s->nTris, org[0], org[1], org[2], e.d);
+	HIP_TRY(hipGetLastError());
+	HIP_TRY(hipEventRecord(e.filled, stream));
+	memcpy(e.org, org, 12); e.valid = true; e.stamp = ++s->relClock;
+	s->relTriBuilt++;
+	*out = e.d; *which = (int)(&e - s->relTri);
 	return 0;
 }
 
@@ -434,8 +474,9 @@
 	A.pstats = dPacketStats;
 	A.packetMajor = packetMajor ? 1 : 0;
 	A.pack = stackPack(s);
-	int relWhich[SNAIL_MAX_BATCH];
-	for(int k = 0; k < FS.n; k++) { relWhich[k] = -1; A.rel[k] = nullptr; }
+	int relWhich[SNAIL_MAX_BATCH], triWhich[SNAIL_MAX_BATCH];
+	for(int k = 0; k < FS.n; k++) { relWhich[k] = triWhich[k] = -1; A.rel[k] = nullptr; A.relTris[k] = nullptr; }
+	bool relTri = false;
 	int blocks;
 	if(dPacketXY) {
 		if(nPackets <= 0) return 0;
@@ -457,11 +498,26 @@
 	A.nSlots = dPacketXY ? nPackets : blocks;
 	A.order = dOrder; A.slotCost = dSlotCost;
 	if(A.pack && !useDeep(s)) {
+		const unsigned long long clock0 = s->relClock;
 		RelPending pend;
 		pend.fill.n = 0;
 		for(int k = 0; k < FS.n; k++)
 			if(int rc = relFor(s, FS.cam[k], stream, &A.rel[k], &relWhich[k], &pend)) { relDrop(s, pend); return rc; }
 		if(int rc = relFlush(s, pend, stream)) return rc;
+		if(!dCost) {
+			relTri = true;
+			const unsigned long long seq = ++s->primarySeq;
+			for(int k = 0; k < FS.n; k++) {
+				const SnailScene::RelNodes &e = s->rel[relWhich[k]];
+				const bool repeats = e.launches > 0 && seq - e.lastPrimary <= (unsigned long long)SnailScene::kRelTriRecent;
+				if(int rc = relTrisFor(s, FS.cam[k], repeats, clock0, stream, &A.relTris[k], &triWhich[k])) return rc;
+				relTri = relTri && A.relTris[k];
+			}
+			for(int k = 0; k < FS.n; k++) {
+				SnailScene::RelNodes &e = s->rel[relWhich[k]];
+				if(e.lastPrimary != seq) { e.launches++; e.lastPrimary = seq; }
+			}
+		}
 	}
 	const int gridBlocks = blocks * FS.n;
 	s->lastBlocks = gridBlocks; s->lastThreads = 64;
@@ -491,8 +547,10 @@
 		else SNAIL_LAUNCH(sse, PrimaryArgs, dim3(blocks), dim3(64), 0, stream, A, k_primary_diag<false>);
 	} else if(A.pstats) {
 		if(useDeep(s)) SNAIL_LAUNCH(sse, PrimaryArgs, grid, block, dynLds, stream, A, k_primary<true, true>);
+		else if(relTri) SNAIL_LAUNCH(sse, PrimaryArgs, grid, block, dynLds, stream, A, k_primary<false, true, true>);
 		else SNAIL_LAUNCH(sse, PrimaryArgs, grid, block, dynLds, stream, A, k_primary<false, true>);
 	} else if(useDeep(s)) SNAIL_LAUNCH(sse, PrimaryArgs, grid, block, dynLds, stream, A, k_primary<true>);
+	else if(relTri) SNAIL_LAUNCH(sse, PrimaryArgs, grid, block, dynLds, stream, A, k_primary<false, false, true>);
 	else SNAIL_LAUNCH(sse, PrimaryArgs, grid, block, dynLds, stream, A, k_primary<false>);
 	static const bool noExact = debugEnvInt("SNAIL_DEBUG_NO_EXACT_PASS") != 0;
 	if(noExact && s->arith == SNAIL_ARITH_IEEE && !EP.nextOrder && !EP.sortAfter) { }
@@ -507,6 +565,8 @@
 	s->deferUsed[slot] = true;
 	for(int k = 0; k < FS.n; k++)
 		if(relWhich[k] >= 0) { if(int rc = relUsed(s, relWhich[k], stream)) return rc; }
+	for(int k = 0; k < FS.n; k++)
+		if(relTri && triWhich[k] >= 0) { if(int rc = relUsed(s->relTri[triWhich[k]], stream)) return rc; }
 	return 0;
 }
 
@@ -852,11 +912,13 @@
 	if(s->dPF) (void)hipFree(s->dPF);
 	if(s->dTab) (void)hipFree(s->dTab);
 	fastFree(s->fast);
-	for(auto &e : s->rel) {
-		if(e.d) (void)hipFree(e.d);
-		if(e.filled) (void)hipEventDestroy(e.filled);
-		for(hipEvent_t ev : e.used) if(ev) (void)hipEventDestroy(ev);
-	}
+	for(auto *arr : {&s->rel[0], &s->relTri[0]})
+		for(int k = 0; k < (arr == &s->rel[0] ? (int)SnailScene::kRelSlots : (int)SnailScene::kRelTriSlots); k++) {
+			SnailScene::RelNodes &e = arr[k];
+			if(e.d) (void)hipFree(e.d);
+			if(e.filled) (void)hipEventDestroy(e.filled);
+			for(hipEvent_t ev : e.used) if(ev) (void)hipEventDestroy(ev);
+		}
 	for(SnailScene::HostCall *c : s->hostFree) {
 		if(c->arena) (void)hipFree(c->arena);
 		if(c->dStats) (void)hipFree(c->dStats);
@@ -1620,6 +1682,35 @@
 	return 0;
 }
 
+int snail_debug_rel_tris_counts(SnailScene *s, int out[2]) {
+	if(int rc = checkScene(s, "snail_debug_rel_tris_counts")) return rc;
+	if(!out) { snail_set_error("snail_debug_rel_tris_counts: null argument"); return 1; }
+	SNAIL_LOCK(s);
+	out[0] = (int)s->relTriBuilt; out[1] = 0;
+	for(auto &e : s->relTri) out[1] += e.valid ? 1 : 0;
+	return 0;
+}
+
+int snail_debug_rel_tris_records(SnailScene *s, const float org[3], uint32_t *out16) {
+	if(int rc = checkScene(s, "snail_debug_rel_tris_records")) return rc;
+	if(!org || !out16) { snail_set_error("snail_debug_rel_tris_records: null argument"); return 1; }
+	DeviceGuard guard(s->device);
+	HostCallScope hc(s, "snail_debug_rel_tris_records");
+	if(hc.rc) return hc.rc;
+	const size_t bytes = (size_t)s->nTris * 64;
+	if(int rc = hc.reserve(HostCallScope::pad(bytes))) return rc;
+	void *d = hc.carve(bytes);
+	{
+		SNAIL_LOCK(s);
+		SceneUse use(s, hc.stream());
+		if(use.rc) return use.rc;
+		hipLaunchKernelGGL(dev::k_rel_tris, dim3((unsigned)((s->nTris + 255) / 256)), dim3(256), 0, hc.stream(), (const uint4 *)s->dTris, s->nTris, org[0], org[1], org[2], (uint4 *)d);
+		HIP_TRY(hipGetLastError());
+	}
+	if(int rc = hc.get(out16, d, bytes)) return rc;
+	return hc.finish(nullptr);
+}
+
 #endif
 
 int snail_account_packets(SnailScene *s, const float cam[13], int resx, int resy, uint32_t *out8) {
```

Result: no change. 28160 Mrays/s, median of 6 (+0.5%).
